# fnzhan/EMLight

Hardware: AMD Instinct MI355X
Metric: training images/sec (regression step: DenseNet-BC fwd + Sinkhorn loss + bwd + Adam) (higher is better)
Workload: dtype f32; 1 GPU; RegressionNetwork train step, BASELINE configs[1]; per_gpu_batch=64, global_batch=64, anchors=128, parallelism=single

## Files before the change

emlight_amd/RegressionNetwork/dense_engine.py:

```python

import os
import weakref

import numpy as np
import torch

from .. import _lib
from .._knobs import knob_int, knob_flag


def _r16(v):
    return (v + 15) // 16 * 16


def _capturing(x):
    return x.is_cuda and torch.cuda.is_current_stream_capturing()


def _row_floats(ctot):
    a = knob_int("EML_ROW_ALIGN", 32, 16, 64)
    if a not in (16, 32, 64):
        raise ValueError("EML_ROW_ALIGN must be 16, 32 or 64")
    return (ctot + a - 1) // a * a


class _Workspace:

    def __init__(self, enc, B, H, W, dev, keep_all):
        f32 = dict(dtype=torch.float32, device=dev)
        self.B, self.H, self.W = B, H, W
        self.blocks = []
        h, w = H, W
        for bi, (c0, nl) in enumerate(zip(enc.block_c0, enc.block_layers)):
            ctot = c0 + nl * enc.growth
            blk = {
                "H": h, "W": w, "P": B * h * w, "C0": c0, "Ctot": ctot, "ld": _row_floats(ctot),
                "X": torch.zeros(B * h * w, _row_floats(ctot), **f32),
                "Z": torch.empty(nl if keep_all else 1, B * h * w, enc.inter, **f32),
                "mean": torch.zeros(_r16(ctot), **f32), "var": torch.ones(_r16(ctot), **f32),
                "istd": torch.ones(_r16(ctot), **f32),
                "layers": [],
            }
            for l in range(nl):
                kp = _r16(c0 + l * enc.growth)
                blk["layers"].append({
                    "Cin": c0 + l * enc.growth, "Kp": kp,
                    "scale1": torch.zeros(kp, **f32), "shift1": torch.zeros(kp, **f32),
                    "scale2": torch.zeros(enc.inter, **f32), "shift2": torch.zeros(enc.inter, **f32),
                    "zmean": torch.zeros(enc.inter, **f32), "zvar": torch.ones(enc.inter, **f32),
                    "zistd": torch.ones(enc.inter, **f32),
                    "W1p": torch.empty(kp * 48, **f32), "W2p": torch.empty(9 * 3 * 4 * 16 * 4, **f32),
                    "W2t": torch.empty(7 * 3 * 64 * 4, **f32),
                    "mask": (torch.empty(((B * h * w + 255) // 256) * 16 * (kp // 16) * 4, dtype=torch.int64, device=dev)
                             if keep_all else None),
                })
            cout = enc.trans_cout[bi]
            kpt = _r16(ctot)
            blk["trans"] = {
                "Cout": cout, "Kp": kpt, "nchunks": (cout + 47) // 48,
                "scale": torch.zeros(kpt, **f32), "shift": torch.zeros(kpt, **f32),
                "Wp": torch.empty(((cout + 47) // 48) * kpt * 48, **f32),
                "Ko": _r16(cout),
                "T": torch.zeros(B * (h // 2) * (w // 2), _r16(cout), **f32),
                "A": torch.empty(B * (h // 2) * (w // 2), kpt, **f32),
                "mask16": (torch.empty(B * (h // 2) * (w // 2) * (kpt // 4), dtype=torch.int16, device=dev)
                           if keep_all else None),
                "one": torch.ones(kpt, **f32), "zero": torch.zeros(kpt, **f32),
                "tmean": torch.zeros(cout, **f32), "tvar": torch.ones(cout, **f32), "tistd": torch.ones(cout, **f32),
                "scaleL": torch.zeros(cout, **f32), "shiftL": torch.zeros(cout, **f32),
            }
            blk["tp"] = enc.tap_packed_plan(B, h, w, dev)
            self.blocks.append(blk)
            h, w = h // 2, w // 2
        self.hf, self.wf = h, w
        cf = enc.trans_cout[-1]
        self.F = torch.zeros(B * h * w, _r16(cf), **f32)
        self.Y0 = torch.empty(B * H * W, enc.c_init, **f32)
        self.mean0 = torch.zeros(enc.c_init, **f32)
        self.var0 = torch.ones(enc.c_init, **f32)
        self.istd0 = torch.ones(enc.c_init, **f32)
        self.scale0 = torch.zeros(enc.c_init, **f32)
        self.shift0 = torch.zeros(enc.c_init, **f32)
        self.partials = torch.zeros(enc.grid_max * max(96 * enc.chunks_max, 2 * enc.kp_max), dtype=torch.float64,
                                    device=dev)
        self.owner, self.done = None, True

    def in_use(self):
        return (not self.done) and self.owner is not None and self.owner() is not None


class _PermuteTable:
    _DT = np.dtype([("src", "<u8"), ("dst", "<u8"), ("kind", "<i4"), ("Cout", "<i4"), ("Cin", "<i4"), ("Kp", "<i4"),
                    ("Ko", "<i4"), ("reserved", "<i4")])

    def __init__(self):
        self.key, self.dev, self.n = None, None, 0

    def launch(self, L, st, items):
        key = tuple((w.data_ptr(), d.data_ptr(), cout, cin) for w, d, _, cout, cin, *_ in items)
        if key != self.key:
            host = np.zeros(len(items), dtype=self._DT)
            for i, (w, d, kind, cout, cin, kp, ko) in enumerate(items):
                host[i] = (w.data_ptr(), d.data_ptr(), kind, cout, cin, kp, ko, 0)
            self.dev = torch.from_numpy(host.view(np.uint8).copy()).to(items[0][1].device)
            self.key, self.n = key, len(items)
        _lib.check(L.eml_dense_permute_batch_f32(_lib.ptr(self.dev), self.n, st), "eml_dense_permute_batch_f32")


class _EncoderFn(torch.autograd.Function):

    @staticmethod
    def forward(ctx, enc, x, *params):
        ctx.enc = enc
        needs_grad = any(ctx.needs_input_grad[1:])
        ws, pooled = enc.run_forward(x, keep_all=needs_grad)
        ctx.ws = ws
        if needs_grad:
            ws.owner, ws.done = weakref.ref(ctx), False
        ctx.save_for_backward(x)
        return pooled

    @staticmethod
    def backward(ctx, gpooled):
        (x,) = ctx.saved_tensors
        ws = ctx.ws
        if ws.owner is None or ws.owner() is not ctx:
            raise RuntimeError("HIP DenseNet: the activations of this forward are gone -- backward() was already run on "
                               "this graph (the workspace is released after the first backward; retain_graph / double "
                               "backward are not supported)")
        need_x, need_params = ctx.needs_input_grad[1], ctx.needs_input_grad[2:]
        dx, grads = ctx.enc.run_backward(ws, x, gpooled.contiguous(), need_x, need_params)
        ws.done, ws.owner = True, None
        ctx.enc.trim_pool(ws)
        return (None, dx) + tuple(g if need else None for g, need in zip(grads, need_params))


class HipDenseEncoder:
    GRID_MAX = 1024

    @staticmethod
    def check_supported(model):
        f = model.features
        if model.bn_size * model.growth_rate != 48 or model.growth_rate != 12:
            raise NotImplementedError("the HIP engine is built for growth_rate=12, bn_size=4 (EMLight's DenseNet)")
        c = f.conv0.out_channels
        if c != 24:
            raise NotImplementedError("the HIP engine is built for num_init_features=24 (got %d)" % c)
        for bi, nl in enumerate(model.block_config):
            ctot = c + nl * model.growth_rate
            if nl < 1 or _r16(ctot) > 384:
                raise NotImplementedError("dense block %d would be %d channels wide; the HIP kernels hold per-channel "
                                          "vectors of at most 384 (EMLight: 216/300/342)" % (bi + 1, ctot))
            c = getattr(f, "transition%d" % (bi + 1)).conv.out_channels
            if _r16(c) == 48:
                raise NotImplementedError("transition %d has %d output channels: widths that pad to 48 collide with the "
                                          "dense layers' bottleneck in the 1x1 launchers (EMLight: 108/150/171)" % (bi + 1, c))
            if c % 2 and bi + 1 < len(model.block_config):
                raise NotImplementedError("transition %d feeds a dense block with an odd channel count (%d)" % (bi + 1, c))

    def __init__(self, model):
        f = model.features
        self.check_supported(model)
        self.model = model
        self.growth = model.growth_rate
        self.inter = model.bn_size * model.growth_rate
        self.c_init = f.conv0.out_channels
        self.block_layers = list(model.block_config)
        self.block_c0, self.trans_cout = [], []
        c = self.c_init
        for bi, nl in enumerate(self.block_layers):
            self.block_c0.append(c)
            c += nl * self.growth
            c = getattr(f, "transition%d" % (bi + 1)).conv.out_channels
            self.trans_cout.append(c)
        self.avgpool = model.avgpool_size
        self.grid_max = self.GRID_MAX
        self.kp_max = max(_r16(c0 + nl * self.growth) for c0, nl in zip(self.block_c0, self.block_layers))
        self.ko_max = max(_r16(c) for c in self.trans_cout)
        self.chunks_max = max((c + 47) // 48 for c in self.trans_cout)
        self._ws = {}
        self._cu = None
        self.last_dropout_key = None

    def param_list(self):
        f = self.model.features
        ps = [f.conv0.weight, f.norm0.weight, f.norm0.bias]
        for bi, nl in enumerate(self.block_layers):
            blk = getattr(f, "denseblock%d" % (bi + 1))
            for l in range(nl):
                L = getattr(blk, "denselayer%d" % (l + 1))
                ps += [L.norm1.weight, L.norm1.bias, L.conv1.weight, L.norm2.weight, L.norm2.bias, L.conv2.weight]
            T = getattr(f, "transition%d" % (bi + 1))
            ps += [T.norm.weight, T.norm.bias, T.conv.weight]
            LN = getattr(f, "last_norm%d" % (bi + 1))
            ps += [LN.weight, LN.bias]
        return ps

    def __call__(self, x):
        x = _lib.require_gpu_tensor(x, "x")
        B, C, H, W = x.shape
        if C != 3:
            raise ValueError("expected (B,3,H,W) input")
        div = 2 ** len(self.block_layers)
        if H % div or W % div or (H // div) < self.avgpool or (W // div) < self.avgpool:
            raise ValueError("crop %dx%d: each of the %d transitions halves the map and the HIP kernels need even maps "
                             "(H, W divisible by %d), then the head pools %dx%d.  Deviation from the reference: its "
                             "AvgPool2d(2) floors odd maps, so e.g. 100x132 trains there; crop to a multiple of %d "
                             "(EMLight's 192x256 and 240x320 are)." % (H, W, len(self.block_layers), div, self.avgpool,
                                                                       self.avgpool, div))
        return _EncoderFn.apply(self, x, *self.param_list())

    def _grid(self, dev):
        if self._cu is None:
            self._cu = torch.cuda.get_device_properties(dev).multi_processor_count
        return self._tuned("EML_GRID", 2 * self._cu)

    def _tuned(self, env, default):
        g = int(os.environ.get(env, 0))
        return min(self.grid_max, g if g > 0 else default)

    def overlap_wgrad(self, dev):
        return torch.device(dev).type == "cuda" and os.environ.get("EML_WGRAD_OVERLAP", "0") == "1"

    def _grid3(self, dev):
        self._grid(dev)
        return self._tuned("EML_GRID3", self._cu)

    def tap_packed_plan(self, B, H, W, dev):
        from .._knobs import knob_choice
        if knob_choice("EML_C3_TP", "auto", ("auto", "off")) == "off":
            return None
        if _lib.lib().eml_dense_conv3x3_fwd_tp_supported(B, H, W) != 4 or H < 8:
            return None
        self._grid(dev)
        bands = max(1, min(H // 4, -(-2 * self._cu // B)))
        band = -(-H // bands)
        return band, min(self.grid_max, B * (-(-H // band)))

    def workspace(self, B, H, W, dev, keep_all):
        key = (B, H, W, dev, keep_all)
        pool = self._ws.get(key)
        if pool is None:
            pool = []
            self._ws = {key: pool}
        for ws in pool:
            if not ws.in_use():
                return ws
        if pool:
            import warnings
            warnings.warn("HIP DenseNet: a %s grad-enabled forward of shape %s is alive before the previous one ran its "
                          "backward: allocating another full activation workspace (GBs at training sizes; idle extras are "
                          "freed after a backward)" % ("second" if len(pool) == 1 else "%d-th" % (len(pool) + 1),
                                                       (B, H, W)), stacklevel=3)
        ws = _Workspace(self, B, H, W, dev, keep_all)
        pool.append(ws)
        return ws

    POOL_KEEP = 2

    def trim_pool(self, ws):
        for key, pool in self._ws.items():
            if ws in pool:
                idle = [w for w in pool if not w.in_use()]
                for extra in idle[self.POOL_KEEP:]:
                    pool.remove(extra)
                return

    def _prepare(self, L, st, partials, G, pstride, n_new, c_new0, count, mean, var, istd, bn, C, Cpad, training,
                 scale, shift):
        p = _lib.ptr
        if bn is None:
            args = (None, None, None, None)
            eps, mom = 1e-5, 0.1
        else:
            args = (p(bn.weight), p(bn.bias), p(bn.running_mean), p(bn.running_var))
            eps, mom = bn.eps, (bn.momentum if bn.momentum is not None else 0.1)
        _lib.check(L.eml_dense_bn_prepare_f32(p(partials), G, pstride, n_new, c_new0, float(count), p(mean), p(var),
                                              p(istd), *args, C, Cpad, eps, mom, int(training), p(scale), p(shift),
                                              st), "eml_dense_bn_prepare_f32")

    def dropout_plan(self, x):
        from .DenseNet import check_drop_rate
        f = self.model.features
        plan, any_drop = [], False
        for bi, nl in enumerate(self.block_layers):
            mod = getattr(f, "denseblock%d" % (bi + 1))
            row = []
            for l in range(nl):
                Lm = getattr(mod, "denselayer%d" % (l + 1))
                q = check_drop_rate(Lm.drop_rate)
                row.append(q if (Lm.training and q > 0) else 0.0)
                any_drop = any_drop or row[-1] > 0
            plan.append(row)
        if not any_drop:
            return None, None
        if _capturing(x):
            raise RuntimeError("HIP DenseNet: drop_rate > 0 while the stream is being captured -- a captured graph would replay "
                               "one fixed dropout mask on every replay; capture with drop_rate = 0 or in eval mode")
        key = self.model.dropout_key
        if key is None:
            lo, hi = torch.randint(0, 2 ** 32, (2,), dtype=torch.int64).tolist()
            key = lo | (hi << 32)
        return key, plan

    def run_forward(self, x, keep_all):
        L, p, st = _lib.lib(), _lib.ptr, _lib.current_stream()
        m = self.model
        f = m.features
        B, _, H, W = x.shape
        dev = x.device
        drop_key, drop_plan = self.dropout_plan(x)
        ws = self.workspace(B, H, W, dev, keep_all)
        ws.drop_key, ws.drop_plan = drop_key, drop_plan
        self.last_dropout_key = drop_key
        G = self._grid(dev)
        G3 = self._grid3(dev)
        Gf = self._tuned("EML_GRID_FWD1", G)
        Gb = min(self.grid_max, 4 * (self._cu or 256))
        training = m.training
        part = ws.partials
        b0 = ws.blocks[0]
        if getattr(ws, "fwd_permutes", None) is None:
            ws.fwd_permutes = _PermuteTable()
        items = []
        for bi, blk in enumerate(ws.blocks):
            mod = getattr(f, "denseblock%d" % (bi + 1))
            for l, lay in enumerate(blk["layers"]):
                Lm = getattr(mod, "denselayer%d" % (l + 1))
                items.append((Lm.conv1.weight, lay["W1p"], 0, 48, lay["Cin"], lay["Kp"], 0))
                if blk["tp"] is None or not training:
                    items.append((Lm.conv2.weight, lay["W2p"], 1, 12, 48, 48, 0))
                else:
                    items.append((Lm.conv2.weight, lay["W2t"], 3, 12, 48, 48, 0))
            T, tr = getattr(f, "transition%d" % (bi + 1)), blk["trans"]
            items.append((T.conv.weight, tr["Wp"], 0, tr["Cout"], blk["Ctot"], tr["Kp"], 0))
        ws.fwd_permutes.launch(L, st, items)
        conv0 = ("eml_dense_conv0_fwd_mfma_f32" if knob_flag("EML_CONV0_MFMA", True) and 3 * B * H * W < 2 ** 31
                 else "eml_dense_conv0_fwd_f32")
        _lib.check(getattr(L, conv0)(p(x), p(f.conv0.weight), p(ws.Y0), self.c_init, B, H, W, self.c_init,
                                     p(part), G, st), conv0)
        self._prepare(L, st, part, G, 2 * self.c_init, self.c_init, 0, b0["P"], ws.mean0, ws.var0, ws.istd0, f.norm0,
                      self.c_init, self.c_init, training, ws.scale0, ws.shift0)
        _lib.check(L.eml_dense_bn_apply_f32(p(ws.Y0), self.c_init, p(b0["X"]), b0["ld"], self.c_init, b0["P"],
                                            p(ws.scale0), p(ws.shift0), 1, p(part), Gb, st), "eml_dense_bn_apply_f32")
        self._prepare(L, st, part, Gb, 2 * self.c_init, self.c_init, 0, b0["P"], b0["mean"], b0["var"], b0["istd"],
                      None, 0, 0, training, None, None)
        nb = len(ws.blocks)
        for bi, blk in enumerate(ws.blocks):
            mod = getattr(f, "denseblock%d" % (bi + 1))
            gl0 = sum(self.block_layers[:bi])
            P, Hb, Wb, ld = blk["P"], blk["H"], blk["W"], blk["ld"]
            pending = False
            Gc = G3
            for l, lay in enumerate(blk["layers"]):
                Lm = getattr(mod, "denselayer%d" % (l + 1))
                cin, kp = lay["Cin"], lay["Kp"]
                z = blk["Z"][l if keep_all else 0]
                self._prepare(L, st, part if pending else None, Gc, 32, 12, cin - 12, P, blk["mean"], blk["var"],
                              blk["istd"], Lm.norm1, cin, kp, training, lay["scale1"], lay["shift1"])
                _lib.check(L.eml_dense_conv1x1_fwd_f32(p(blk["X"]), ld, P, Hb, Wb, 0, kp, p(lay["scale1"]),
                                                       p(lay["shift1"]), p(lay["W1p"]), 48, p(z), 48, p(part), Gf,
                                                       p(lay["mask"]) if (keep_all and training) else None, st),
                           "eml_dense_conv1x1_fwd_f32")
                self._prepare(L, st, part, Gf, 96, 48, 0, P, lay["zmean"], lay["zvar"], lay["zistd"], Lm.norm2, 48, 48,
                              training, lay["scale2"], lay["shift2"])
                q = drop_plan[bi][l] if drop_plan is not None else 0.0
                drop = (drop_key, gl0 + l, q) if q > 0 else ()
                if blk["tp"] is None or not training:
                    Gc = G3
                    fn = "eml_dense_conv3x3_fwd_drop_f32" if drop else "eml_dense_conv3x3_fwd_f32"
                    _lib.check(getattr(L, fn)(p(z), p(lay["scale2"]), p(lay["shift2"]), p(lay["W2p"]), p(blk["X"]), ld, cin,
                                              B, Hb, Wb, p(part), G3, *drop, st), fn)
                else:
                    band, Gc = blk["tp"]
                    fn = "eml_dense_conv3x3_fwd_tp_drop_f32" if drop else "eml_dense_conv3x3_fwd_tp_f32"
                    _lib.check(getattr(L, fn)(p(z), p(lay["scale2"]), p(lay["shift2"]), p(lay["W2t"]), p(blk["X"]), ld, cin,
                                              B, Hb, Wb, band, p(part), Gc, *drop, st), fn)
                pending = True
            tr, T = blk["trans"], getattr(f, "transition%d" % (bi + 1))
            LN = getattr(f, "last_norm%d" % (bi + 1))
            ctot, cout, kpt = blk["Ctot"], tr["Cout"], tr["Kp"]
            self._prepare(L, st, part if pending else None, Gc, 32, 12, ctot - 12, P, blk["mean"], blk["var"],
                          blk["istd"], T.norm, ctot, kpt, training, tr["scale"], tr["shift"])
            Pn = B * (Hb // 2) * (Wb // 2)
            _lib.check(L.eml_dense_pool_act_f32(p(blk["X"]), ld, B, Hb, Wb, kpt, p(tr["scale"]), p(tr["shift"]),
                                                p(tr["A"]), kpt, p(tr["mask16"]) if (keep_all and training) else None,
                                                st), "eml_dense_pool_act_f32")
            _lib.check(L.eml_dense_conv1x1_fwd_f32(p(tr["A"]), kpt, Pn, Hb // 2, Wb // 2, 0, kpt, p(tr["one"]),
                                                   p(tr["zero"]), p(tr["Wp"]), cout, p(tr["T"]), tr["Ko"], p(part), G,
                                                   None, st), "eml_dense_conv1x1_fwd_f32(transition)")
            for ch in range(tr["nchunks"]):
                nv = min(48, cout - 48 * ch)
                last = ch == tr["nchunks"] - 1
                pv = part[ch * G * 96:]
                self._prepare(L, st, pv, G, 96, nv, 48 * ch, Pn, tr["tmean"], tr["tvar"], tr["tistd"],
                              LN if last else None, cout if last else 0, cout if last else 0, training,
                              tr["scaleL"] if last else None, tr["shiftL"] if last else None)
            if bi + 1 < nb:
                nxt = ws.blocks[bi + 1]
                dst, ldd = nxt["X"], nxt["ld"]
            else:
                dst, ldd = ws.F, ws.F.shape[1]
            _lib.check(L.eml_dense_bn_apply_f32(p(tr["T"]), tr["Ko"], p(dst), ldd, cout, Pn, p(tr["scaleL"]),
                                                p(tr["shiftL"]), 0, p(part), Gb, st), "eml_dense_bn_apply_f32")
            if bi + 1 < nb:
                self._prepare(L, st, part, Gb, 2 * cout, cout, 0, Pn, nxt["mean"], nxt["var"], nxt["istd"], None, 0, 0,
                              training, None, None)
        cf = self.trans_cout[-1]
        k = self.avgpool
        pooled = torch.empty(B, cf * (ws.hf // k) * (ws.wf // k), dtype=torch.float32, device=dev)
        _lib.check(L.eml_dense_head_pool_fwd_f32(p(ws.F), ws.F.shape[1], cf, B, ws.hf, ws.wf, k, p(pooled), st),
                   "eml_dense_head_pool_fwd_f32")
        if training:
            bns = [mm for mm in f.modules() if isinstance(mm, torch.nn.BatchNorm2d)]
            torch._foreach_add_([mm.num_batches_tracked for mm in bns], 1)
        return ws, pooled

    def run_backward(self, ws, x, gpooled, need_x=False, need_params=None):
        from .dense_engine_bwd import run_backward
        return run_backward(self, ws, x, gpooled, need_x, need_params)
```

emlight_amd/RegressionNetwork/dense_engine_bwd.py:

```python
import ctypes
import os

import torch

from .. import _lib
from .._knobs import knob_choice, knob_flag


def _r16(v):
    return (v + 15) // 16 * 16


class _BwdBuffers:
    def gf12(self, r):
        if self.GF12[r] is None:
            self.GF12[r] = self._gf12_new()
        return self.GF12[r]

    def __init__(self, enc, ws, dev):
        f32 = dict(dtype=torch.float32, device=dev)
        self.G = [torch.zeros(blk["P"], blk["ld"], **f32) for blk in ws.blocks]
        self.GF = torch.zeros(ws.F.shape[0], ws.F.shape[1], **f32)
        maxP = ws.blocks[0]["P"]
        self.DZ = torch.empty(2, maxP, 48, **f32)
        self.ring = max(1, int(os.environ.get("EML_WGRAD_RING", 4))) if enc.overlap_wgrad(dev) else 1
        self.GF12 = [None] * self.ring
        self._gf12_new = lambda: torch.empty(maxP, 12, **f32)
        self.N12 = torch.empty(maxP, 12, **f32)
        self.TOP = torch.empty(2 * maxP * 12, **f32)
        kp, ko, g = enc.kp_max, max(enc.ko_max, 48), enc.grid_max
        self.Wd = [[torch.empty(lay["Kp"] * 48, **f32) for lay in blk["layers"]] for blk in ws.blocks]
        self.WdT = [torch.empty(blk["trans"]["Kp"] * blk["trans"]["Ko"], **f32) for blk in ws.blocks]
        self.permutes = None
        self.coef = torch.zeros(8, max(kp, ko), **f32)
        self.part2 = torch.zeros(2, g * kp * 2, dtype=torch.float64, device=dev)
        self.partW = torch.empty(g * max(kp * 48, 2 * 27 * 256, 4 * 1024), **f32)
        i32 = dict(dtype=torch.int32, device=dev)
        self.cond = [[torch.zeros(lay["Kp"], **i32) for lay in blk["layers"]] for blk in ws.blocks]
        self.condT = [torch.zeros(blk["trans"]["Kp"], **i32) for blk in ws.blocks]
        self.any_ill = torch.zeros(1, **i32)
        self.dg_grid = 128
        self.dg_scratch = torch.empty(self.dg_grid * kp, dtype=torch.float64, device=dev)
        self.side = None
        if enc.overlap_wgrad(dev):
            self.side = torch.cuda.Stream(device=dev)
            self.partW3 = [torch.empty(g * 2 * 27 * 256, **f32) for _ in range(self.ring)]
            self.ev_ready = [torch.cuda.Event() for _ in range(self.ring)]
            self.ev_done = [None] * self.ring


def run_backward(enc, ws, x, gpooled, need_x=False, need_params=None):
    if getattr(ws, "bwd", None) is None:
        ws.bwd = _BwdBuffers(enc, ws, x.device)
    L, p, st = _lib.lib(), _lib.ptr, _lib.current_stream()
    m = enc.model
    f = m.features
    if not m.training:
        raise NotImplementedError("HIP DenseNet backward is implemented for train-mode BatchNorm "
                                  "(EMLight trains and tests in train mode, train.py:42 / test.py:36-37)")
    dev = x.device
    B, _, H, W = x.shape
    G = enc._grid(dev)
    G3 = enc._grid3(dev)
    G3d = enc._tuned("EML_GRID3_DGRAD", G3)
    Gw = enc._tuned("EML_GRID_WGRAD1", G)
    Gd = enc._tuned("EML_GRID_DGRAD", G)
    Gb = min(enc.grid_max, 4 * enc._cu)
    bw = ws.bwd
    part = ws.partials
    ring = [0]
    if bw.side is not None:
        main = torch.cuda.current_stream(dev)
        st_side = ctypes.c_void_p(bw.side.cuda_stream)
        G3s = enc._tuned("EML_GRID3_SIDE", G3)
        bw.side.wait_stream(main)
    if bw.permutes is None:
        from .dense_engine import _PermuteTable
        bw.permutes = _PermuteTable()
    items = []
    for bi_, blk_ in enumerate(ws.blocks):
        mod_ = getattr(f, "denseblock%d" % (bi_ + 1))
        for l_, lay_ in enumerate(blk_["layers"]):
            items.append((getattr(mod_, "denselayer%d" % (l_ + 1)).conv1.weight, bw.Wd[bi_][l_], 2, 48, lay_["Cin"],
                          lay_["Kp"], 48))
        tr_ = blk_["trans"]
        items.append((getattr(f, "transition%d" % (bi_ + 1)).conv.weight, bw.WdT[bi_], 2, tr_["Cout"], blk_["Ctot"],
                      tr_["Kp"], tr_["Ko"]))
    bw.permutes.launch(L, st, items)
    params = enc.param_list()
    if need_params is None:
        need_params = [True] * len(params)
    from .._dist import grad_slot
    grads = {}
    for q, need in zip(params, need_params):
        slot = grad_slot(q) if need else None
        grads[id(q)] = slot if slot is not None else torch.empty_like(q)
    gr = lambda q: p(grads[id(q)])
    coefs = [tuple(bw.coef[3 * k + i] for i in range(3)) for k in range(2)]
    cA, cB, cC = coefs[0]
    sB, sC = bw.coef[6], bw.coef[7]

    direct = knob_choice("EML_DGAMMA_DIRECT", "always", ("always", "never")) != "never"
    c3_fold = knob_flag("EML_C3_FOLD", True)
    c3_gf = knob_flag("EML_C3_GF", False)
    bw.any_ill.zero_()

    def dgamma_direct(blk, X_ld, Pin, Hin, Win, pool, DY, ld_dy, Zr, ld_z, co, Cout, conv, Cin, scale1, shift1, cond, bn):
        if not direct:
            return
        a, b, c = co if co is not None else (None, None, None)
        _lib.check(L.eml_dense_bn_dgamma_direct_f32(
            p(blk["X"]), X_ld, Pin, Hin, Win, pool, p(DY), ld_dy, p(Zr), ld_z, p(a), p(b), p(c), Cout, p(conv.weight), Cin,
            p(scale1), p(shift1), p(blk["mean"]), p(blk["istd"]), p(cond), p(bw.dg_scratch), gr(bn.weight), bw.dg_grid, st),
            "eml_dense_bn_dgamma_direct_f32")

    def finalize(R, pstride, count, bn, mean, istd, C, Cpad, coef=0, s_acc=None, src=None, c_lo=0, c_hi=None, conv=None,
                 cond=None):
        a, b, c = coefs[coef] if coef is not None else (None, None, None)
        wargs = (p(bn.bias), p(conv.weight), gr(conv.weight), conv.weight.shape[0]) if conv is not None else (None, None, None, 0)
        _lib.check(L.eml_dense_bn_bwd_finalize_f32(
            p(part if src is None else src), R, pstride, float(count), p(bn.weight), p(mean), p(istd), C, Cpad, 1,
            gr(bn.weight), gr(bn.bias), p(a), p(b), p(c),
            p(sB) if s_acc is not None else None, p(sC) if s_acc is not None else None, int(bool(s_acc)),
            c_lo, Cpad if c_hi is None else c_hi, *wargs, p(cond), p(bw.any_ill) if cond is not None else None, st),
            "eml_dense_bn_bwd_finalize_f32")

    def parr(tensors):
        return (ctypes.c_void_p * len(tensors))(*[t.data_ptr() for t in tensors])

    def materialize(Gbuf, blk, c0, n):
        _lib.check(L.eml_dense_grad_materialize_f32(p(Gbuf), blk["ld"], p(blk["X"]), blk["ld"], p(sB), p(sC), c0, n,
                                                    blk["P"], st), "eml_dense_grad_materialize_f32")

    cf, k = enc.trans_cout[-1], enc.avgpool
    ldF = ws.F.shape[1]
    _lib.check(L.eml_dense_head_pool_bwd_f32(p(gpooled), p(ws.F), ldF, cf, B, ws.hf, ws.wf, k, p(bw.GF), ldF, st),
               "eml_dense_head_pool_bwd_f32")
    dY, ld_dy = bw.GF, ldF
    nb = len(ws.blocks)
    for bi in reversed(range(nb)):
        blk, tr = ws.blocks[bi], ws.blocks[bi]["trans"]
        mod = getattr(f, "denseblock%d" % (bi + 1))
        T, LN = getattr(f, "transition%d" % (bi + 1)), getattr(f, "last_norm%d" % (bi + 1))
        P, Hb, Wb, ld, ctot = blk["P"], blk["H"], blk["W"], blk["ld"], blk["Ctot"]
        cout, Ko, kpt = tr["Cout"], tr["Ko"], tr["Kp"]
        Pn = B * (Hb // 2) * (Wb // 2)
        Gbuf = bw.G[bi]
        gl0 = sum(enc.block_layers[:bi])
        top2 = bw.TOP[:2 * P * 12].view(2, P, 12)
        _lib.check(L.eml_dense_bn_bwd_stats_f32(p(dY), ld_dy, p(tr["T"]), Ko, None, 0, 0, cout, Pn, p(tr["tmean"]),
                                                p(tr["tistd"]), p(part), Gb, st), "eml_dense_bn_bwd_stats_f32")
        finalize(Gb, 2 * cout, Pn, LN, tr["tmean"], tr["tistd"], cout, Ko, coef=0)
        _lib.check(L.eml_dense_conv1x1_bwd_weight_f32(
            p(tr["A"]), kpt, Pn, Hb // 2, Wb // 2, 0, kpt, ctot, p(tr["one"]), p(tr["zero"]), p(dY), ld_dy, p(tr["T"]),
            Ko, p(cA), p(cB), p(cC), cout, p(bw.partW), gr(T.conv.weight), G, None, None, 0, None, 0, None, None, st),
            "eml_dense_conv1x1_bwd_weight_f32")
        _lib.check(L.eml_dense_conv1x1_bwd_data_f32(
            p(dY), ld_dy, p(tr["T"]), Ko, p(cA), p(cB), p(cC), Ko, p(bw.WdT[bi]), None, ld, p(tr["scale"]),
            p(tr["shift"]), None, None, Pn, Hb, Wb, 1, kpt, p(Gbuf), ld, 0, p(part), G, p(tr["mask16"]), st),
            "eml_dense_conv1x1_bwd_data_f32")
        finalize(G, 2 * kpt, P, T.norm, blk["mean"], blk["istd"], ctot, kpt, coef=None, s_acc=False, conv=T.conv,
                 cond=bw.condT[bi])
        dgamma_direct(blk, ld, P, Hb, Wb, 1, dY, ld_dy, tr["T"], Ko, coefs[0], cout, T.conv, ctot, tr["scale"], tr["shift"],
                      bw.condT[bi], T.norm)
        def conv2_backward(l, slot, n12=False, narrow_lo=None, top=False):
            lay = blk["layers"][l]
            Lm = getattr(mod, "denselayer%d" % (l + 1))
            cin, kp, z, dz = lay["Cin"], lay["Kp"], blk["Z"][l], bw.DZ[slot]
            gsrc = (p(bw.N12), 12, 0) if n12 else (p(top2[1]), 12, 0) if top else (p(Gbuf), ld, cin)
            r = ring[0] = (ring[0] + 1) % bw.ring
            if bw.side is not None and bw.ev_done[r] is not None:
                main.wait_event(bw.ev_done[r])
            fold = (bw.side is None and c3_fold
                    and L.eml_dense_conv3x3_bwd_fused_supported(gsrc[1], gsrc[2], ld, cin) == 1)
            q = ws.drop_plan[bi][l] if ws.drop_plan is not None else 0.0
            drop = (ws.drop_key, gl0 + l, q) if q > 0 else ()
            if fold:
                fn = "eml_dense_conv3x3_bwd_fused_drop_f32" if drop else "eml_dense_conv3x3_bwd_fused_f32"
                _lib.check(getattr(L, fn)(*gsrc, p(Lm.conv2.weight), p(z), p(lay["zmean"]), p(lay["zistd"]), p(dz), B, Hb, Wb,
                                          p(part), G3d, p(blk["X"]), ld, cin, p(sB), p(sC), p(bw.gf12(r)) if c3_gf else None,
                                          p(lay["scale2"]), p(lay["shift2"]), p(bw.partW), gr(Lm.conv2.weight), *drop, st), fn)
            else:
                fn = "eml_dense_conv3x3_bwd_data_drop_f32" if drop else "eml_dense_conv3x3_bwd_data_f32"
                _lib.check(getattr(L, fn)(*gsrc, p(Lm.conv2.weight), p(z), p(lay["zmean"]), p(lay["zistd"]), p(dz), B, Hb, Wb,
                                          p(part), G3d, p(blk["X"]), ld, cin, p(sB), p(sC), p(bw.gf12(r)), *drop, st), fn)
            if fold:
                pass
            elif bw.side is None:
                _lib.check(L.eml_dense_conv3x3_bwd_weight_f32(p(bw.gf12(r)), 12, 0, p(z), p(lay["scale2"]),
                                                              p(lay["shift2"]), B, Hb, Wb, p(bw.partW),
                                                              gr(Lm.conv2.weight), G3, st),
                           "eml_dense_conv3x3_bwd_weight_f32")
            else:
                bw.ev_ready[r].record(main)
                bw.side.wait_event(bw.ev_ready[r])
                _lib.check(L.eml_dense_conv3x3_bwd_weight_f32(p(bw.gf12(r)), 12, 0, p(z), p(lay["scale2"]),
                                                              p(lay["shift2"]), B, Hb, Wb, p(bw.partW3[r]),
                                                              gr(Lm.conv2.weight), G3s, st_side),
                           "eml_dense_conv3x3_bwd_weight_f32")
                if bw.ev_done[r] is None:
                    bw.ev_done[r] = torch.cuda.Event()
                bw.ev_done[r].record(bw.side)
            finalize(G3d, 96, P, Lm.norm2, lay["zmean"], lay["zistd"], 48, 48, coef=slot)
            a, b, c = coefs[slot]
            _lib.check(L.eml_dense_conv1x1_bwd_weight_f32(
                p(blk["X"]), ld, P, Hb, Wb, 0, kp, cin, p(lay["scale1"]), p(lay["shift1"]), p(dz), 48, p(z), 48,
                p(a), p(b), p(c), 48, p(bw.partW), gr(Lm.conv1.weight), Gw, p(dz),
                *((p(Lm.conv1.weight), narrow_lo, *((p(top2[0]), 12) if top else (p(Gbuf), ld)), p(bw.N12),
                   p(bw.part2[slot])) if narrow_lo is not None
                  else (None, 0, None, 0, None, None)), st), "eml_dense_conv1x1_bwd_weight_f32")
            return Lm

        def dgrad(layers, slots, k_lo, k_hi, top=False):
            lays = [blk["layers"][l] for l in layers]
            if top:
                _lib.check(L.eml_dense_conv1x1_bwd_data_multi_top_f32(
                    parr([bw.DZ[s_] for s_ in slots]), parr([bw.Wd[bi][l_] for l_ in layers]),
                    parr([y["scale1"] for y in lays]), parr([y["shift1"] for y in lays]),
                    parr([bw.part2[s_] for s_ in slots]), (ctypes.c_int * len(layers))(*[y["Kp"] for y in lays]),
                    P, k_hi, p(Gbuf), ld, Gd, parr([y["mask"] for y in lays]), p(top2), st),
                    "eml_dense_conv1x1_bwd_data_multi_top_f32")
                return
            _lib.check(L.eml_dense_conv1x1_bwd_data_multi_f32(
                len(layers), parr([bw.DZ[s_] for s_ in slots]), None, None, None, None,
                parr([bw.Wd[bi][l_] for l_ in layers]),
                parr([y["scale1"] for y in lays]), parr([y["shift1"] for y in lays]),
                parr([bw.part2[s_] for s_ in slots]), (ctypes.c_int * len(layers))(*[y["Kp"] for y in lays]),
                None, ld, None, None, P, k_lo, k_hi, p(Gbuf), ld, Gd,
                parr([y["mask"] for y in lays]), st),
                "eml_dense_conv1x1_bwd_data_multi_f32")

        def bn1_finalize(l, Lm, slot, c_lo, c_hi, rows=None):
            lay = blk["layers"][l]
            finalize(Gd if rows is None else rows, 2 * lay["Kp"], P, Lm.norm1, blk["mean"], blk["istd"], lay["Cin"], lay["Kp"], coef=None,
                     s_acc=True, src=bw.part2[slot], c_lo=c_lo, c_hi=c_hi, conv=Lm.conv1, cond=bw.cond[bi][l])

        def bn1_direct(l, Lm, slot):
            lay = blk["layers"][l]
            dgamma_direct(blk, ld, P, Hb, Wb, 0, bw.DZ[slot], 48, None, 0, None, 48, Lm.conv1, lay["Cin"], lay["scale1"],
                          lay["shift1"], bw.cond[bi][l], Lm.norm1)

        l = len(blk["layers"]) - 1
        have_top = False
        while l >= 0:
            if l >= 1:
                la, lb = l, l - 1
                cin_a, cin_b = blk["layers"][la]["Cin"], blk["layers"][lb]["Cin"]
                Lma = conv2_backward(la, 0, narrow_lo=cin_b, top=have_top)
                bn1_finalize(la, Lma, 0, cin_b, cin_a, rows=Gw)
                Lmb = conv2_backward(lb, 1, n12=True)
                to_top = (lb >= 2 and blk["layers"][la]["mask"] is not None and bw.side is None
                          and cin_b >= 24 and cin_b % 4 == 0)
                dgrad([la, lb], [0, 1], 0, cin_b, top=to_top)
                have_top = to_top
                bn1_finalize(la, Lma, 0, 0, cin_b)
                bn1_finalize(lb, Lmb, 1, 0, blk["layers"][lb]["Kp"])
                bn1_direct(la, Lma, 0)
                bn1_direct(lb, Lmb, 1)
                l -= 2
            else:
                Lm0 = conv2_backward(l, 0)
                dgrad([l], [0], 0, blk["layers"][l]["Cin"])
                bn1_finalize(l, Lm0, 0, 0, blk["layers"][l]["Kp"])
                bn1_direct(l, Lm0, 0)
                l -= 1
        c0b = blk["C0"]
        norm0_fused = bi == 0 and knob_flag("EML_NORM0_FUSED", True) and c0b % 4 == 0 and c0b <= 32
        if not norm0_fused:
            materialize(Gbuf, blk, 0, c0b)
        dY, ld_dy = Gbuf, ld
    b0 = ws.blocks[0]
    c0 = enc.c_init
    if norm0_fused:
        _lib.check(L.eml_dense_norm0_bwd_stats_f32(p(dY), ld_dy, p(ws.Y0), c0, p(ws.scale0), p(ws.shift0), p(sB), p(sC), c0,
                                                   b0["P"], p(ws.mean0), p(ws.istd0), p(part), Gb, st),
                   "eml_dense_norm0_bwd_stats_f32")
    else:
        _lib.check(L.eml_dense_bn_bwd_stats_f32(p(dY), ld_dy, p(ws.Y0), c0, p(b0["X"]), b0["ld"], 1, c0, b0["P"],
                                                p(ws.mean0), p(ws.istd0), p(part), Gb, st), "eml_dense_bn_bwd_stats_f32")
    finalize(Gb, 2 * c0, b0["P"], f.norm0, ws.mean0, ws.istd0, c0, _r16(c0), coef=0)
    if norm0_fused:
        _lib.check(L.eml_dense_conv0_bwd_weight_fused_f32(p(x), p(dY), ld_dy, p(ws.Y0), c0, p(ws.scale0), p(ws.shift0), p(sB),
                                                          p(sC), p(cA), p(cB), p(cC), B, H, W, p(bw.partW),
                                                          gr(f.conv0.weight), G, st), "eml_dense_conv0_bwd_weight_fused_f32")
    else:
        _lib.check(L.eml_dense_conv0_bwd_weight_f32(p(x), p(dY), ld_dy, p(b0["X"]), b0["ld"], p(ws.Y0), c0, p(cA), p(cB),
                                                    p(cC), B, H, W, p(bw.partW), gr(f.conv0.weight), G, st),
                   "eml_dense_conv0_bwd_weight_f32")
    dx = None
    if need_x:
        dx = torch.empty(B, 3, H, W, dtype=torch.float32, device=dev)
        X1 = (None, 0) if norm0_fused else (p(b0["X"]), b0["ld"])
        _lib.check(L.eml_dense_conv0_bwd_data_f32(p(dY), ld_dy, *X1, p(ws.Y0), c0, p(ws.scale0), p(ws.shift0), p(sB), p(sC),
                                                  p(cA), p(cB), p(cC), p(f.conv0.weight), B, H, W, p(dx), st),
                   "eml_dense_conv0_bwd_data_f32")
    if bw.side is not None:
        main.wait_stream(bw.side)
    return dx, [grads[id(q)] for q in params]
```

emlight_amd/_lib.py:

```python
import ctypes
import os
import threading

_HERE = os.path.dirname(os.path.abspath(__file__))
LIB_PATH = os.environ.get("EML_LIB_PATH") or os.path.join(_HERE, "libemlight_hip.so")

_f32p = ctypes.c_void_p
_i32p = ctypes.c_void_p
_f64p = ctypes.c_void_p
_stream = ctypes.c_void_p
_int = ctypes.c_int
_u64 = ctypes.c_ulonglong

ABI_VERSION = 31

SIGNATURES = {
    "eml_abi_version": (_int, []),
    "eml_last_error": (ctypes.c_char_p, []),
    "eml_sg_rasterise_f32": (_int, [_f32p, _f32p, _f32p, _f32p, _int, _int, _int, _int, _stream]),
    "eml_sg_rasterise_ex_f32": (_int, [_f32p, _f32p, _f32p, _f32p, _int, _int, _int, _int, _int, ctypes.c_void_p, _stream]),
    "eml_sg_rasterise_bwd_colors_f32": (_int, [_f32p, _f32p, _f32p, _f32p, _int, _int, _int, _int, _stream]),
    "eml_emd_anchor_cost_f32": (_int, [_f32p, _f32p, _int, _stream]),
    "eml_sinkhorn_schedule_f32": (_int, [_f32p, _f32p, ctypes.c_long, ctypes.c_double, ctypes.c_double, _int,
                                         ctypes.c_double, _f32p, _f32p, _i32p, _f32p, _stream]),
    "eml_sinkhorn_work_floats": (ctypes.c_size_t, [_int, _int]),
    "eml_sinkhorn_fwd_f32": (_int, [_f32p, _f32p, _f32p, _f32p, _f32p, _f32p, ctypes.c_double, ctypes.c_double, _int,
                                    ctypes.c_double, _f32p, _f32p, _i32p, _f32p, _f32p, _f32p, _f32p, _f32p, _int, _int,
                                    _stream]),
    "eml_sinkhorn_fwd_ex_f32": (_int, [_f32p, _f32p, _f32p, _f32p, _f32p, _f32p, ctypes.c_double, ctypes.c_double, _int,
                                       ctypes.c_double, _f32p, _f32p, _i32p, _f32p, _f32p, _f32p, _f32p, _f32p, _int, _int,
                                       _int, _stream]),
    "eml_sinkhorn_fwd_rho_f32": (_int, [_f32p, _f32p, _f32p, _f32p, _f32p, _f32p, ctypes.c_double, ctypes.c_double, _int,
                                        ctypes.c_double, _f32p, _f32p, _i32p, _f32p, _f32p, _f32p, _f32p, _f32p, _int, _int,
                                        _int, ctypes.c_double, _f32p, _stream]),
    "eml_sinkhorn_bwd_f32": (_int, [_f32p, _f32p, _f32p, _int, _int, _stream]),
    "eml_sinkhorn_dim_work_floats": (ctypes.c_size_t, [_int, _int, _int]),
    "eml_sinkhorn_fwd_dim_f32": (_int, [_f32p, _f32p, _f32p, _f32p, _f32p, _f32p, ctypes.c_double, ctypes.c_double, _int,
                                        ctypes.c_double, _f32p, _f32p, _i32p, _f32p, _f32p, _f32p, _f32p, _f32p, _int, _int,
                                        _int, _int, ctypes.c_double, _f32p, _stream]),
    "eml_sinkhorn_schedule_dim_f32": (_int, [_f32p, _f32p, ctypes.c_long, _int, ctypes.c_double, ctypes.c_double, _int,
                                             ctypes.c_double, _f32p, _f32p, _i32p, _f32p, _stream]),
    "eml_sinkhorn_bwd_weights_f32": (_int, [_f32p, _f32p, _f32p, _f32p, _int, _int, _stream]),
    "eml_l1_pairs_partial_doubles": (ctypes.c_size_t, [_int]),
    "eml_l1_pairs_fwd_f32": (_int, [_int, ctypes.c_void_p, ctypes.c_void_p, ctypes.c_void_p, ctypes.c_void_p, ctypes.c_void_p,
                                    ctypes.c_void_p, _f64p, _f32p, _stream]),
    "eml_l1_pairs_bwd_f32": (_int, [_int, ctypes.c_void_p, ctypes.c_void_p, ctypes.c_void_p, ctypes.c_void_p, ctypes.c_void_p,
                                    ctypes.c_void_p, _f32p, ctypes.c_void_p, ctypes.c_void_p, ctypes.c_void_p, _stream]),
    "eml_colsum_partial_doubles": (ctypes.c_size_t, [_int]),
    "eml_colsum_f32": (_int, [_f32p, ctypes.c_long, _int, _f64p, _f32p, _stream]),
    "eml_gt_anchor_index_i32": (_int, [_f32p, _int, _int, _int, _i32p, _stream]),
    "eml_gt_parametrise_f64": (_int, [_f32p, _i32p, _i32p, _int, _int, _int, _int, _f32p, _f32p, _f32p, _stream]),
    "eml_pano_crop_f32": (_int, [ctypes.c_void_p, _int, _int, _int, _int, _int, _int, ctypes.c_double, ctypes.c_double, _f64p,
                                 ctypes.c_double, _f64p, _f32p, _stream]),
    "eml_pano_resize_area_f32": (_int, [_f32p, _int, _int, _int, _int, _int, ctypes.c_double, _f64p, _f32p, _stream]),
    "eml_tonemap_work_floats": (ctypes.c_size_t, [_int]),
    "eml_tonemap_f32": (_int, [_f32p, _int, ctypes.c_long, _int, ctypes.c_double, ctypes.c_double, ctypes.c_double, _f32p,
                               _int, _f32p, _f32p, _i32p, _f32p, ctypes.c_void_p, _stream]),
    "eml_projector_targets_work_floats": (ctypes.c_size_t, [_int, _int, _int]),
    "eml_projector_targets_f32": (_int, [_f32p, _f32p, _int, _int, _int, _f32p, _f32p, _f32p, _stream]),
    "eml_resize_bilinear_f32": (_int, [_f32p, _f32p, _int, _int, _int, _int, _int, _int, _int, _f32p, _stream]),
    "eml_sphere_render_work_floats": (ctypes.c_size_t, [_int, _int, _int, _int]),
    "eml_sphere_render_f32": (_int, [_f32p, _int, _int, _int, _int, ctypes.c_double, _int, ctypes.c_double, _f32p, _f32p,
                                     _stream]),
    "eml_sphere_render_metrics_f64": (_int, [_f32p, _f32p, _int, _int, _int, _f64p, _stream]),
    "eml_needlet_basis_f32": (_int, [_f32p, _int, _f32p, _f32p, _int, _f32p, _stream]),
    "eml_needlet_work_floats": (ctypes.c_size_t, [_int, _int, _int]),
    "eml_needlet_analysis_f32": (_int, [_f32p, _f32p, _f32p, _int, _int, _f32p, _f32p, _int, _f32p, _f32p, _stream]),
    "eml_needlet_synthesis_f32": (_int, [_f32p, _f32p, _f32p, _int, _int, _f32p, _f32p, _int, _f32p, _stream]),
    "eml_needlet_sparsify_f32": (_int, [_f32p, _int, _int, _int, ctypes.c_double, _f32p, _i32p, _stream]),
    "eml_sh_basis_f32": (_int, [_f32p, _int, _f32p, _int, _f32p, _stream]),
    "eml_sh_work_floats": (ctypes.c_size_t, [_int, _int, _int, _int]),
    "eml_sh_analysis_f32": (_int, [_f32p, _f32p, _f32p, _f32p, _f32p, _int, _int, _int, _int, _f32p, _f32p, _stream]),
    "eml_sh_synthesis_f32": (_int, [_f32p, _f32p, _f32p, _f32p, _f32p, _int, _int, _int, _int, _f32p, _stream]),
    "eml_sphere_tap_table_f32": (_int, [_f32p, _int, _int, _int, _int, _i32p, _f32p, _stream]),
    "eml_sphere_im2col_f32": (_int, [_f32p, _i32p, _f32p, _f32p, _int, _int, _int, _int, _stream]),
    "eml_sphere_col2im_f32": (_int, [_f32p, _i32p, _i32p, _f32p, _f32p, _int, _int, _int, _int, _stream]),
    "eml_sphere_conv_fwd_fused_f32": (_int, [_f32p, _i32p, _f32p, _f32p, _f32p, _f32p, _int, _int, _int, _int, _int, _int,
                                             _stream]),
    "eml_sphere_conv_fwd_fused_ex_f32": (_int, [_f32p, _i32p, _f32p, _f32p, _f32p, _f32p, _int, _int, _int, _int, _int, _int,
                                                _f32p, ctypes.c_float, _int, _stream]),
    "eml_sphere_conv_small_supported": (_int, [_int, _int]),
    "eml_sphere_conv_small_fwd_f32": (_int, [_f32p, _i32p, _f32p, _f32p, _f32p, _f32p, _int, _int, _int, _int, _int,
                                             ctypes.c_float, _stream]),
    "eml_sphere_conv_small_wgrad_partial_floats": (ctypes.c_size_t, [_int, _int, _int, _int]),
    "eml_sphere_conv_small_wgrad_f32": (_int, [_f32p, _i32p, _f32p, _f32p, _f32p, ctypes.c_float, _f32p, _f32p, _f32p, _int,
                                               _int, _int, _int, _int, _stream]),
    "eml_sphere_conv_small_da9_f32": (_int, [_f32p, _f32p, ctypes.c_float, _f32p, _f32p, ctypes.c_long, _int, _int, _stream]),
    "eml_spade_norm_modulate_up2_fwd_f32": (_int, [_f32p, _f32p, _f32p, _int, _int, _int, _int, ctypes.c_float, _f32p, _f32p,
                                                   _stream]),
    "eml_spade_norm_modulate_bwd_cols_f32": (_int, [_f32p, _f32p, _f32p, _f32p, _f32p, _int, _int, _int, _int, _int,
                                                    ctypes.c_float, _f32p, _f32p, _f32p, _int, _stream]),
    "eml_sg_rasterise_bwd_work_floats": (ctypes.c_size_t, [_int, _int, _int, _int]),
    "eml_sg_rasterise_bwd_colors_ex_f32": (_int, [_f32p, _f32p, _f32p, _f32p, _f32p, _int, _int, _int, _int, _int, _stream]),
    "eml_sg_rasterise_bwd_full_work_floats": (ctypes.c_size_t, [_int, _int, _int, _int]),
    "eml_sg_rasterise_bwd_f32": (_int, [_f32p, _f32p, _f32p, _f32p, _f32p, _f32p, _f32p, _f32p, _int, _int, _int, _int, _int,
                                        _stream]),
    "eml_sphere_conv_narrow_supported": (_int, [_int, _int]),
    "eml_sphere_conv_narrow_fwd_f32": (_int, [_f32p, _i32p, _f32p, _f32p, _f32p, _f32p, _int, _int, _int, _int, _int, _stream]),
    "eml_sphere_conv_narrow_dgrad_f32": (_int, [_f32p, _i32p, _f32p, _int, _f32p, _f32p, _int, _int, _int, _int, _int, _stream]),
    "eml_sphere_conv_narrow_wgrad_partial_floats": (ctypes.c_size_t, [_int, _int, _int, _int]),
    "eml_sphere_conv_narrow_wgrad_f32": (_int, [_f32p, _i32p, _f32p, _f32p, _f32p, _f32p, _int, _int, _int, _int, _int, _stream]),
    "eml_sphere_conv_narrow_scratch_floats": (ctypes.c_size_t, [_int, _int]),
    "eml_sphere_conv_narrow_fwd2_f32": (_int, [_f32p, _i32p, _f32p, _f32p, _f32p, _f32p, _f32p, _int, _int, _int, _int, _int, _stream]),
    "eml_sphere_conv_narrow_wgrad2_partial_floats": (ctypes.c_size_t, [_int, _int, _int]),
    "eml_sphere_conv_narrow_dgrad2_f32": (_int, [_f32p, _i32p, _f32p, _int, ctypes.c_void_p, _f32p, _f32p, _f32p, _int, _int, _int,
                                                 _int, _int, _int, _stream]),
    "eml_sphere_conv_narrow_wgrad2_f32": (_int, [_f32p, _i32p, _f32p, _int, ctypes.c_void_p, _f32p, _f32p, _f32p, _f32p, _int, _int,
                                                 _int, _int, _int, _stream]),
    "eml_sphere_conv_spade_supported": (_int, [_int, _int, ctypes.c_long]),
    "eml_sphere_conv_spade_fwd_f32": (_int, [_f32p, _i32p, _f32p, _f32p, _f32p, _f32p, _f32p, _f32p, _f32p, _f32p, _int, _int,
                                             _int, _int, _int, _int, ctypes.c_float, _int, _stream]),
    "eml_spade_norm_modulate_bwd_y_f32": (_int, [_f32p, _f32p, _f32p, _f32p, _f32p, _f32p, _int, _int, _int, _int, _int,
                                                 ctypes.c_float, _f32p, _f32p, _f32p, _int, _stream]),
    "eml_bn_bwd_apply_up2_f32": (_int, [_f32p, _f32p, _int, _int, _int, _int, _f32p, _f32p, _f32p, _f32p, _stream]),
    "eml_spectral_norm_scratch_floats": (ctypes.c_size_t, [_int, _int]),
    "eml_spectral_norm_w2_f32": (_int, [_f32p, _f32p, _f32p, _int, ctypes.c_float, _f32p, _f32p, _f32p, _f32p, _int, _int,
                                        _stream]),
    "eml_spectral_norm_w2_bwd_f32": (_int, [_f32p, _f32p, _f32p, _f32p, _f32p, _f32p, _f32p, _int, _int, _stream]),
    "eml_spectral_norm_w2_batch_f32": (_int, [_int, ctypes.c_void_p, ctypes.c_void_p, ctypes.c_void_p, _int, ctypes.c_float,
                                              ctypes.c_void_p, ctypes.c_void_p, ctypes.c_void_p, ctypes.c_void_p, ctypes.c_void_p,
                                              ctypes.c_void_p, _stream]),
    "eml_spade_heads_w2_f32": (_int, [_f32p, _f32p, _f32p, _f32p, _f32p, _f32p, _int, _int, _int, _stream]),
    "eml_instance_norm_act_fwd_f32": (_int, [_f32p, _f32p, _f32p, _int, _int, _int, _int, ctypes.c_float, ctypes.c_float,
                                             _stream]),
    "eml_instance_norm_act_bwd_f32": (_int, [_f32p, _f32p, _f32p, _f32p, _int, _int, _int, _int, ctypes.c_float, _stream]),
    "eml_sphere_conv_dgrad_fused_f32": (_int, [_f32p, _i32p, _f32p, _i32p, _int, _f32p, _f32p, _int, _int, _int, _int, _int,
                                               _int, _stream]),
    "eml_sphere_conv_lowres_variant": (_int, [_int, _int, _int, _int]),
    "eml_sphere_conv_lowres_table_i32": (_int, [_i32p, _i32p, _i32p, _int, _int, _stream]),
    "eml_sphere_conv_lowres_partial_floats": (ctypes.c_size_t, [ctypes.c_long, _int, _int]),
    "eml_sphere_conv_lowres_f32": (_int, [_f32p, _i32p, _f32p, _i32p, _int, _i32p, _int, _f32p, _f32p, _f32p, _f32p, _int, _int,
                                          _int, _int, _int, _int, _f32p, ctypes.c_float, _stream]),
    "eml_sphere_conv_wgrad_partial_floats": (ctypes.c_size_t, [_int, _int, _int]),
    "eml_sphere_conv_wgrad_fused_f32": (_int, [_f32p, _i32p, _f32p, _f32p, _f32p, _f32p, _int, _int, _int, _int, _int, _int,
                                               _stream]),
    "eml_spade_modulate_fwd_f32": (_int, [_f32p, _int, _f32p, _int, _f32p, _int, ctypes.c_long, _int, ctypes.c_float,
                                          _stream]),
    "eml_spade_modulate_bwd_f32": (_int, [_f32p, _int, _f32p, _int, _f32p, _int, _f32p, _int, _f32p, _int, ctypes.c_long,
                                          _int, ctypes.c_float, _stream]),
    "eml_bn_stats_f32": (_int, [_f32p, _int, ctypes.c_long, _int, _f32p, _int, _stream]),
    "eml_bn_fold_f64": (_int, [_f32p, _int, _int, _f32p, _stream]),
    "eml_bn_finalize_f32": (_int, [_f32p, _int, ctypes.c_float, ctypes.c_float, _f32p, _f32p, _f32p, _f32p, _stream]),
    "eml_spade_norm_modulate_fwd_f32": (_int, [_f32p, _int, _f32p, _int, _f32p, _int, ctypes.c_long, _int, ctypes.c_float,
                                               _f32p, _f32p, _stream]),
    "eml_bn_bwd_apply_f32": (_int, [_f32p, _int, _f32p, _int, ctypes.c_long, _int, _f32p, _f32p, _f32p, _f32p, _int,
                                    _stream]),
    "eml_dense_conv0_fwd_f32": (_int, [_f32p, _f32p, _f32p, _int, _int, _int, _int, _int, _f32p, _int, _stream]),
    "eml_dense_conv0_fwd_mfma_f32": (_int, [_f32p, _f32p, _f32p, _int, _int, _int, _int, _int, _f32p, _int, _stream]),
    "eml_dense_bn_apply_f32": (_int, [_f32p, _int, _f32p, _int, _int, ctypes.c_long, _f32p, _f32p, _int, _f32p,
                                      _int, _stream]),
    "eml_dense_bn_prepare_f32": (_int, [_f32p, _int, _int, _int, _int, ctypes.c_double, _f32p, _f32p, _f32p, _f32p,
                                        _f32p, _f32p, _f32p, _int, _int, ctypes.c_float, ctypes.c_float, _int,
                                        _f32p, _f32p, _stream]),
    "eml_dense_permute_w1_f32": (_int, [_f32p, _int, _int, _int, _f32p, _stream]),
    "eml_dense_permute_w2_f32": (_int, [_f32p, _int, _f32p, _stream]),
    "eml_dense_permute_batch_f32": (_int, [ctypes.c_void_p, _int, _stream]),
    "eml_dense_conv1x1_fwd_f32": (_int, [_f32p, _int, ctypes.c_long, _int, _int, _int, _int, _f32p, _f32p, _f32p,
                                         _int, _f32p, _int, _f32p, _int, ctypes.c_void_p, _stream]),
    "eml_dense_conv3x3_fwd_f32": (_int, [_f32p, _f32p, _f32p, _f32p, _f32p, _int, _int, _int, _int, _int, _f32p,
                                         _int, _stream]),
    "eml_dense_permute_w2_tp_f32": (_int, [_f32p, _f32p, _stream]),
    "eml_dense_conv3x3_fwd_tp_supported": (_int, [_int, _int, _int]),
    "eml_dense_conv3x3_fwd_tp_f32": (_int, [_f32p, _f32p, _f32p, _f32p, _f32p, _int, _int, _int, _int, _int, _int, _f32p,
                                            _int, _stream]),
    "eml_dense_conv3x3_fwd_drop_f32": (_int, [_f32p, _f32p, _f32p, _f32p, _f32p, _int, _int, _int, _int, _int, _f32p,
                                              _int, _u64, _int, ctypes.c_double, _stream]),
    "eml_dense_conv3x3_fwd_tp_drop_f32": (_int, [_f32p, _f32p, _f32p, _f32p, _f32p, _int, _int, _int, _int, _int, _int, _f32p,
                                                 _int, _u64, _int, ctypes.c_double, _stream]),
    "eml_dense_dropout_mask_u16": (_int, [_u64, _int, ctypes.c_double, ctypes.c_long, ctypes.c_void_p, _stream]),
    "eml_dense_pool_act_f32": (_int, [_f32p, _int, _int, _int, _int, _int, _f32p, _f32p, _f32p, _int, ctypes.c_void_p,
                                      _stream]),
    "eml_dense_head_pool_fwd_f32": (_int, [_f32p, _int, _int, _int, _int, _int, _int, _f32p, _stream]),
    "eml_dense_conv3x3_bwd_data_f32": (_int, [_f32p, _int, _int, _f32p, _f32p, _f32p, _f32p, _f32p, _int, _int, _int,
                                              _f32p, _int, _f32p, _int, _int, _f32p, _f32p, _f32p, _stream]),
    "eml_dense_conv3x3_bwd_fused_supported": (_int, [_int, _int, _int, _int]),
    "eml_dense_conv3x3_bwd_fused_f32": (_int, [_f32p, _int, _int, _f32p, _f32p, _f32p, _f32p, _f32p, _int, _int, _int, _f64p, _int,
                                               _f32p, _int, _int, _f32p, _f32p, _f32p, _f32p, _f32p, _f32p, _f32p, _stream]),
    "eml_dense_conv3x3_bwd_data_drop_f32": (_int, [_f32p, _int, _int, _f32p, _f32p, _f32p, _f32p, _f32p, _int, _int, _int,
                                                   _f32p, _int, _f32p, _int, _int, _f32p, _f32p, _f32p, _u64, _int,
                                                   ctypes.c_double, _stream]),
    "eml_dense_conv3x3_bwd_fused_drop_f32": (_int, [_f32p, _int, _int, _f32p, _f32p, _f32p, _f32p, _f32p, _int, _int, _int,
                                                    _f64p, _int, _f32p, _int, _int, _f32p, _f32p, _f32p, _f32p, _f32p, _f32p,
                                                    _f32p, _u64, _int, ctypes.c_double, _stream]),
    "eml_dense_conv3x3_bwd_weight_f32": (_int, [_f32p, _int, _int, _f32p, _f32p, _f32p, _int, _int, _int, _f32p,
                                                _f32p, _int, _stream]),
    "eml_dense_bn_bwd_finalize_f32": (_int, [_f32p, _int, _int, ctypes.c_double, _f32p, _f32p, _f32p, _int, _int,
                                             _int, _f32p, _f32p, _f32p, _f32p, _f32p, _f32p, _f32p, _int, _int, _int,
                                             _f32p, _f32p, _f32p, _int, _i32p, _i32p, _stream]),
    "eml_dense_bn_dgamma_direct_f32": (_int, [_f32p, _int, ctypes.c_long, _int, _int, _int, _f32p, _int, _f32p, _int,
                                              _f32p, _f32p, _f32p, _int, _f32p, _int, _f32p, _f32p, _f32p, _f32p, _i32p,
                                              _f32p, _f32p, _int, _stream]),
    "eml_dense_conv1x1_bwd_weight_f32": (_int, [_f32p, _int, ctypes.c_long, _int, _int, _int, _int, _int, _f32p,
                                                _f32p, _f32p, _int, _f32p, _int, _f32p, _f32p, _f32p, _int, _f32p,
                                                _f32p, _int, _f32p, _f32p, _int, _f32p, _int, _f32p, _f32p, _stream]),
    "eml_dense_conv1x1_bwd_narrow_f32": (_int, [_f32p, _f32p, _int, _int, _f32p, _int, _f32p, _f32p, _f32p, _f32p,
                                                ctypes.c_long, _f32p, _int, _f32p, _f32p, _int, _int, _stream]),
    "eml_dense_permute_w1_bwd_f32": (_int, [_f32p, _int, _int, _int, _int, _f32p, _stream]),
    "eml_dense_conv1x1_bwd_data_f32": (_int, [_f32p, _int, _f32p, _int, _f32p, _f32p, _f32p, _int, _f32p, _f32p,
                                              _int, _f32p, _f32p, _f32p, _f32p, ctypes.c_long, _int, _int, _int,
                                              _int, _f32p, _int, _int, _f32p, _int, ctypes.c_void_p, _stream]),
    "eml_dense_conv1x1_bwd_data_multi_f32": (_int, [_int] + [ctypes.c_void_p] * 10 + [_f32p, _int, _f32p, _f32p,
                                                    ctypes.c_long, _int, _int, _f32p, _int, _int, ctypes.c_void_p,
                                                    _stream]),
    "eml_dense_conv1x1_bwd_data_multi_top_f32": (_int, [ctypes.c_void_p] * 6 + [ctypes.c_long, _int, _f32p, _int, _int,
                                                        ctypes.c_void_p, _f32p, _stream]),
    "eml_dense_grad_materialize_f32": (_int, [_f32p, _int, _f32p, _int, _f32p, _f32p, _int, _int, ctypes.c_long,
                                              _stream]),
    "eml_dense_bn_bwd_stats_f32": (_int, [_f32p, _int, _f32p, _int, _f32p, _int, _int, _int, ctypes.c_long, _f32p,
                                          _f32p, _f32p, _int, _stream]),
    "eml_dense_norm0_bwd_stats_f32": (_int, [_f32p, _int, _f32p, _int, _f32p, _f32p, _f32p, _f32p, _int, ctypes.c_long, _f32p, _f32p,
                                             ctypes.c_void_p, _int, _stream]),
    "eml_dense_conv0_bwd_weight_fused_f32": (_int, [_f32p, _f32p, _int, _f32p, _int, _f32p, _f32p, _f32p, _f32p, _f32p, _f32p, _f32p,
                                                    _int, _int, _int, _f32p, _f32p, _int, _stream]),
    "eml_dense_conv0_bwd_weight_f32": (_int, [_f32p, _f32p, _int, _f32p, _int, _f32p, _int, _f32p, _f32p, _f32p,
                                              _int, _int, _int, _f32p, _f32p, _int, _stream]),
    "eml_dense_conv0_bwd_data_f32": (_int, [_f32p, _int, _f32p, _int, _f32p, _int, _f32p, _f32p, _f32p, _f32p, _f32p, _f32p,
                                            _f32p, _f32p, _int, _int, _int, _f32p, _stream]),
    "eml_dense_head_pool_bwd_f32": (_int, [_f32p, _f32p, _int, _int, _int, _int, _int, _int, _f32p, _int, _stream]),
}

EXT_SIGNATURES = {
    "eml_pano_warp_f32": (_int, [_f32p, _int, _int, _int, _int, _int, ctypes.c_double, ctypes.c_double, ctypes.c_double, _f64p,
                                 _f32p, _f64p, _stream]),
    "eml_pano_warp_bwd_work_floats": (ctypes.c_size_t, [_int, _int, _int, _int, _int, _int, _int]),
    "eml_pano_warp_bwd_f32": (_int, [_f32p, _f32p, _int, _int, _int, _int, _int, ctypes.c_double, ctypes.c_double,
                                     ctypes.c_double, _f64p, _f32p, _f64p, _f32p, _stream]),
    "eml_sphere_render_bwd_work_floats": (ctypes.c_size_t, [_int, _int, _int, _int]),
    "eml_sphere_render_bwd_f32": (_int, [_f32p, _int, _int, _int, _int, ctypes.c_double, _int, ctypes.c_double, _i32p, _i32p,
                                         _f32p, _f32p, _f32p, _stream]),
    "eml_sphere_mirror_taps_f32": (_int, [_int, _int, _int, ctypes.c_double, _i32p, _f32p, _stream]),
    "eml_gm_anchor_cost_f32": (_int, [ctypes.c_void_p, _int, _int, _int, _f32p, _f32p, _stream]),
    "eml_sinkhorn_fwd_cost_f32": (_int, [_f32p, _f32p, _f32p, _f32p, _f32p, _f32p, ctypes.c_double, ctypes.c_double, _int,
                                         ctypes.c_double, _f32p, _f32p, _i32p, _f32p, _f32p, _f32p, _f32p, _f32p, _int, _int,
                                         _int, _int, ctypes.c_double, _f32p, ctypes.c_long, _stream]),
    "eml_sphere_max_pool_fwd_f32": (_int, [_f32p, _i32p, _f32p, _f32p, ctypes.c_void_p, _int, _int, _int, _int, _stream]),
    "eml_sphere_max_pool_bwd_f32": (_int, [_f32p, ctypes.c_void_p, _i32p, _i32p, _f32p, _f32p, _int, _int, _int, _int, _stream]),
    "eml_sphere_conv_small_dbias_f32": (_int, [_f32p, _f32p, ctypes.c_float, _f32p, _f32p, _int, _int, _int, _int, _stream]),
    "eml_env_prefilter_work_floats": (ctypes.c_size_t, [_int, _int, _int, _int, _int]),
    "eml_env_prefilter_f32": (_int, [_f32p, _int, _int, _int, _int, _int, ctypes.c_void_p, _f32p, _f32p, _stream]),
    "eml_gbuffer_shade_f32": (_int, [_f32p, _int, _f32p, _int, ctypes.c_long, _f32p, _int, ctypes.c_long, _f32p, _f32p, _f32p,
                                     _f32p, _f32p, _int, _int, _int, ctypes.c_double, ctypes.c_double, _f32p, _f32p, _f32p,
                                     ctypes.c_double, _f32p, _stream]),
    "eml_env_prefilter_bwd_work_floats": (ctypes.c_size_t, [_int, _int, _int, _int, _int]),
    "eml_env_prefilter_bwd_f32": (_int, [_f32p, _int, _int, _int, _int, _int, ctypes.c_void_p, _f32p, _f32p, _stream]),
    "eml_gbuffer_shade_bwd_work_floats": (ctypes.c_size_t, [_int, _int, _int, _int, _int, _int, _int, _int, _int]),
    "eml_gbuffer_shade_bwd_f32": (_int, [_f32p, _f32p, _int, _f32p, _int, ctypes.c_long, _f32p, _int, ctypes.c_long, _f32p,
                                         _f32p, _f32p, _f32p, _f32p, _int, _int, _int, ctypes.c_double, ctypes.c_double,
                                         _f32p, _f32p, ctypes.c_double, _f32p, _f32p, _f32p, _f32p, _f32p, _f32p, _f32p,
                                         _f32p, _stream]),
    "eml_pano_warp_depth_work_floats": (ctypes.c_size_t, [_int, _int, _int]),
    "eml_pano_warp_depth_f32": (_int, [_f32p, _f32p, _int, _int, _int, _int, _int, ctypes.c_double, ctypes.c_double,
                                       ctypes.c_double, _f64p, _int, _int, _f32p, _f32p, _f64p, _f32p, _stream]),
    "eml_gt_anchor_depth_f64": (_int, [_f32p, _i32p, _i32p, _int, _int, _int, _int, _f64p, _stream]),
    "eml_ground_shadow_work_floats": (ctypes.c_size_t, [_int, _int, _int, _int, _int]),
    "eml_ground_shadow_f32": (_int, [_f32p, _int, _int, _int, _f32p, _int, _f32p, _int, _int, _int, ctypes.c_double,
                                     ctypes.c_double, _f32p, _f32p, _f32p, _f32p, _stream]),
}

_lock = threading.Lock()
_lib = None


class EmlightHipError(RuntimeError):
    pass


def lib():
    global _lib
    if _lib is not None:
        return _lib
    with _lock:
        if _lib is not None:
            return _lib
        if not os.path.exists(LIB_PATH):
            raise EmlightHipError(
                "libemlight_hip.so not found at %s -- build it with "
                "`python -c 'import __graft_entry__ as g; g.build()'` or `make -C emlight_amd/csrc`. "
                "There is no CPU fallback." % LIB_PATH)
        handle = ctypes.CDLL(LIB_PATH)
        for name, (res, args) in list(SIGNATURES.items()) + list(EXT_SIGNATURES.items()):
            try:
                fn = getattr(handle, name)
            except AttributeError as e:
                raise EmlightHipError("libemlight_hip.so lacks symbol %s" % name) from e
            fn.restype, fn.argtypes = res, args
        got = handle.eml_abi_version()
        if got != ABI_VERSION:
            raise EmlightHipError("libemlight_hip.so has ABI version %d, this binding expects %d -- rebuild it "
                                  "(make -C emlight_amd/csrc)" % (got, ABI_VERSION))
        _lib = handle
    from . import _gemm_selection
    _gemm_selection.ensure_if_requested()
    return _lib


_DEBUG_SYNC = bool(os.environ.get("EML_DEBUG_SYNC"))


def check(rc, what):
    if rc != 0:
        msg = lib().eml_last_error()
        raise EmlightHipError("%s failed (rc=%d): %s" % (what, rc, msg.decode() if msg else "?"))
    if _DEBUG_SYNC:
        import sys
        import torch
        sys.stderr.write("[eml] %s ... " % what)
        sys.stderr.flush()
        torch.cuda.synchronize()
        sys.stderr.write("ok\n")


def ptr(t):
    if t is None:
        return None
    return ctypes.c_void_p(t.data_ptr())


def current_stream():
    import torch
    return ctypes.c_void_p(torch.cuda.current_stream().cuda_stream)


def require_gpu_tensor(t, name, dtype=None):
    import torch
    if not isinstance(t, torch.Tensor) or not t.is_cuda:
        raise EmlightHipError("%s must be a tensor on the MI355X (got %s); there is no CPU path"
                              % (name, getattr(t, "device", type(t))))
    if t.dtype != (dtype or torch.float32):
        raise EmlightHipError("%s must be %s (got %s)" % (name, dtype or torch.float32, t.dtype))
    return t.contiguous()
```

emlight_amd/csrc/dense_bwd.hip:

```cpp
#include "eml_common.h"
#include "eml_dropout.h"

#include <cstdint>
#include <cstdlib>
#include <type_traits>

namespace {

using eml::f32x4;
using eml::f4c;
using eml::mfma16;
using eml::shfl_xor_d;

constexpr int kTH = 8, kTW = 32, kHH = kTH + 2, kHW = kTW + 2;

constexpr int kPSG = 14;
constexpr int kBD = 512;
constexpr int kGRows = 2;
constexpr int kGPass = kHH / kGRows;

template <bool FUSE, bool WIDE, bool DROP = false>
__global__ __launch_bounds__(kBD, 2) void conv3x3_bwd_data_kernel(
    const float* __restrict__ G, int ldg, int c0, const float* __restrict__ W2, const float* __restrict__ Z,
    const float* __restrict__ zmean, const float* __restrict__ zistd, float* __restrict__ DZ, int B, int H, int W,
// ... 444 lines not shown

  for (int e = tid; e < 27 * 3 * 64; e += 512) {
    const int l = e & 63, g3 = e >> 6, n = g3 % 3, ts = g3 / 3, s3 = ts % 3, tap = ts / 3;
    w_l[e] = W2[((size_t)(4 * s3 + (l >> 4)) * 48 + 16 * n + (l & 15)) * 9 + tap];
  }
  if (tid < 24) coef_l[tid] = tid < 12 ? sB[cx + tid] : sC[cx + tid - 12];

  const int role = __builtin_amdgcn_readfirstlane(wave >> 2), pairj = wave & 3;
  f32x4 accw[4][3];
  int goff[4];
#pragma unroll
  for (int i = 0; i < 4; ++i) {
#pragma unroll
    for (int n = 0; n < 3; ++n) accw[i][n] = f32x4{0.f, 0.f, 0.f, 0.f};
    const int t = min(3 * role + i, 6);
    const int row = min(16 * t + r, 107), tap = row / 12, o = row - 12 * tap;
    goff[i] = (-(tap / 3 - 1) * kHW - (tap % 3 - 1)) * kPSG + o;
  }
  float scb[3], shb[3];
#pragma unroll
  for (int n = 0; n < 3; ++n) {
    scb[n] = scale2[16 * n + r];
    shb[n] = shift2[16 * n + r];
  }
  const int tx_n = (W + kTW - 1) / kTW, ty_n = (H + kTH - 1) / kTH;
  const int ntiles = B * ty_n * tx_n;
  for (int e = tid; e < 8 * 48 * 2; e += 512) red[e] = 0.0;

  constexpr int kWideItems = kHH * kHW * 3;
  int w_hy[2], w_hx[2], w_q[2], w_pix[2];
  bool w_ok[2], w_own[2];
#pragma unroll
  for (int it = 0; it < 2; ++it) {
    const int t = min(tid + 512 * it, kWideItems - 1), hp = t / 3;
    w_q[it] = t - 3 * hp;
    w_hy[it] = hp / kHW;
    w_hx[it] = hp - w_hy[it] * kHW;
  }
  f32x4 gt4[2], xt4[2];
  constexpr int kZI = kTH * kTW * 12 / 512;
  int z_pq[kZI];
#pragma unroll
  for (int it = 0; it < kZI; ++it) {
    const int t = tid + 512 * it;
    z_pq[it] = ((t / 12) << 4) | (t % 12);
  }
  auto stage_begin = [&](int tile) {
    const int b = tile / (ty_n * tx_n), rem = tile - b * (ty_n * tx_n);
    const int ty = rem / tx_n, tx = rem - ty * tx_n;
#pragma unroll
    for (int it = 0; it < 2; ++it) {
      const int gy = ty * kTH - 1 + w_hy[it], gx = tx * kTW - 1 + w_hx[it];
      w_ok[it] = gy >= 0 && gy < H && gx >= 0 && gx < W;
      w_pix[it] = (b * H + min(max(gy, 0), H - 1)) * W + min(max(gx, 0), W - 1);
      if constexpr (STORE_GF) w_own[it] = w_ok[it] && w_hy[it] >= 1 && w_hy[it] <= kTH && w_hx[it] >= 1 && w_hx[it] <= kTW;
    }
  };
  auto g_load = [&](int it) {
    const float* gp = G + (size_t)w_pix[it] * ldg + c0 + 4 * w_q[it];
    const float* xp = Xb + (size_t)w_pix[it] * ldx + cx + 4 * w_q[it];
    if constexpr (A16) {
      asm volatile("global_load_dwordx4 %0, %1, off" : "=&v"(gt4[it]) : "v"(gp) : "memory");
      asm volatile("global_load_dwordx4 %0, %1, off" : "=&v"(xt4[it]) : "v"(xp) : "memory");
    } else {
      const float2 g0 = *reinterpret_cast<const float2*>(gp), g1 = *reinterpret_cast<const float2*>(gp + 2);
      const float2 x0 = *reinterpret_cast<const float2*>(xp), x1 = *reinterpret_cast<const float2*>(xp + 2);
      gt4[it] = f32x4{g0.x, g0.y, g1.x, g1.y};
      xt4[it] = f32x4{x0.x, x0.y, x1.x, x1.y};
    }
  };
  auto g_wait = [&]() {
    if constexpr (A16)
      asm volatile("s_waitcnt vmcnt(0)" : "+v"(gt4[0]), "+v"(xt4[0]), "+v"(gt4[1]), "+v"(xt4[1]) :: "memory");
  };
  auto g_commit = [&](int it, float* dst) {
    const float4 fb4 = *reinterpret_cast<const float4*>(coef_l + 4 * w_q[it]);
    const float4 fc4 = *reinterpret_cast<const float4*>(coef_l + 12 + 4 * w_q[it]);
    float4 v;
    v.x = fmaf(fb4.x, xt4[it][0], gt4[it][0]) + fc4.x;
    v.y = fmaf(fb4.y, xt4[it][1], gt4[it][1]) + fc4.y;
    v.z = fmaf(fb4.z, xt4[it][2], gt4[it][2]) + fc4.z;
    v.w = fmaf(fb4.w, xt4[it][3], gt4[it][3]) + fc4.w;
    if constexpr (DROP) v = eml::drop4(dk, (unsigned)w_pix[it], (unsigned)w_q[it], v);
    if (!w_ok[it]) v = make_float4(0.f, 0.f, 0.f, 0.f);
    float* d = dst + (w_hy[it] * kHW + w_hx[it]) * kPSG + 4 * w_q[it];
    *reinterpret_cast<float2*>(d) = make_float2(v.x, v.y);
    *reinterpret_cast<float2*>(d + 2) = make_float2(v.z, v.w);
    if constexpr (STORE_GF) gt4[it] = f32x4{v.x, v.y, v.z, v.w};
  };
  auto g_store = [&](int it) {
    if constexpr (!STORE_GF) return;
    if (w_own[it]) *reinterpret_cast<float4*>(GF + ((unsigned)w_pix[it] * 12u + 4u * (unsigned)w_q[it])) = make_float4(gt4[it][0], gt4[it][1], gt4[it][2], gt4[it][3]);
  };
  auto z_dma = [&](int it, int b, int y0, int x0, int buf) {
    const int pix = z_pq[it] >> 4, q = z_pq[it] & 15;
    const int gy = min(y0 + (pix >> 5), H - 1), gx = min(x0 + (pix & 31), W - 1);
    const float* src = Z + ((size_t)(b * H + gy) * W + gx) * 48 + 4 * q;
    unsigned keep;
    const unsigned dst = __builtin_amdgcn_readfirstlane(
        (unsigned)(size_t)(const __attribute__((address_space(3))) char*)(z_l + buf * (kTH * kTW * kZS) + 4 * (64 * wave + 512 * it)));
    asm volatile("s_mov_b32 %0, m0\n\ts_mov_b32 m0, %2\n\ts_nop 0\n\tglobal_load_lds_dwordx4 %1, off\n\ts_mov_b32 m0, %0"
                 : "=&s"(keep) : "v"(src), "s"(dst) : "memory");
  };

  int tile = blockIdx.x, cur = 0;
  __syncthreads();
  if (tile < ntiles) {
    stage_begin(tile);
    g_load(0);
    g_load(1);
    {
      const int b = tile / (ty_n * tx_n), rem = tile - b * (ty_n * tx_n);
#pragma unroll
      for (int it = 0; it < kZI; ++it) z_dma(it, b, (rem / tx_n) * kTH, (rem % tx_n) * kTW, 0);
    }
    g_wait();
    g_commit(0, g_l);
    g_commit(1, g_l);
    g_store(0);
    g_store(1);
  }
  __syncthreads();
#ifdef EML_STAMPS
  unsigned long long st_acc[5] = {0, 0, 0, 0, 0}, st_last = __builtin_readcyclecounter();
#endif
  for (; tile < ntiles; tile += gridDim.x) {
    const int nxt = tile + gridDim.x;
    const float* gc = g_l + cur * kGT;
    float* gn = g_l + (cur ^ 1) * kGT;
    const int b = tile / (ty_n * tx_n), rem = tile - b * (ty_n * tx_n);
    const int ty = rem / tx_n, tx = rem - ty * tx_n;
    const int gy = ty * kTH + wave;
    size_t prow[2];
    bool pv[2];
#pragma unroll
    for (int m = 0; m < 2; ++m) {
      const int gx = tx * kTW + 16 * m + r;
      pv[m] = gy < H && gx < W;
      prow[m] = ((size_t)(b * H + min(gy, H - 1)) * W + min(gx, W - 1)) * 48;
    }
    stage_begin(nxt < ntiles ? nxt : tile);
    f32x4 acc[2][3];
#pragma unroll
    for (int m = 0; m < 2; ++m)
#pragma unroll
      for (int n = 0; n < 3; ++n) acc[m][n] = f32x4{0.f, 0.f, 0.f, 0.f};
    float aq[2][2], wq[2][3];
#pragma unroll
    for (int n = 0; n < 3; ++n) wq[0][n] = w_l[n * 64 + lane];
#pragma unroll
    for (int m = 0; m < 2; ++m) aq[0][m] = gc[((wave + 2) * kHW + 16 * m + r + 2) * kPSG + kk];
#pragma unroll
    for (int tap = 0; tap < 9; ++tap) {
#pragma unroll
      for (int s3 = 0; s3 < 3; ++s3) {
        const int gi = tap * 3 + s3;
        if (gi < 2) {
          g_load(gi);
          asm volatile("" ::: "memory");
          __builtin_amdgcn_sched_barrier(0);
        }
        if (gi + 1 < 27) {
          const int tn = (gi + 1) / 3, sn = (gi + 1) - 3 * tn, dyn = tn / 3, dxn = tn - 3 * dyn;
#pragma unroll
          for (int n = 0; n < 3; ++n) wq[(gi + 1) & 1][n] = w_l[((gi + 1) * 3 + n) * 64 + lane];
#pragma unroll
          for (int m = 0; m < 2; ++m)
            aq[(gi + 1) & 1][m] = gc[((wave + 2 - dyn) * kHW + 16 * m + r + 2 - dxn) * kPSG + 4 * sn + kk];
        }
        __builtin_amdgcn_sched_barrier(0);
#pragma unroll
        for (int m = 0; m < 2; ++m)
#pragma unroll
          for (int n = 0; n < 3; ++n) acc[m][n] = mfma16(wq[gi & 1][n], aq[gi & 1][m], acc[m][n]);
        if (gi >= 25) {
          __builtin_amdgcn_sched_barrier(0);
          if (gi == 25) g_wait();
          g_commit(gi - 25, gn);
        }
      }
    }
    g_store(0);
    g_store(1);
    EML_C3_STAMP(0);
    asm volatile("s_waitcnt vmcnt(0)" ::: "memory");
    eml::lds_barrier();
    EML_C3_STAMP(1);
    const float* ga = gc + ((2 * pairj + 1) * kHW + kk + 1) * kPSG;
    const float* zc = z_l + cur * (kTH * kTW * kZS);
    const float* zb = zc + (kTW * 2 * pairj + kk) * kZS + r;
    const int xl0 = ty * kTH + 2 * pairj < H ? W - tx * kTW - kk : 0, xl1 = ty * kTH + 2 * pairj + 1 < H ? W - tx * kTW - kk : 0;
    auto phase_b = [&](auto nt_tag) {
      constexpr int NT = decltype(nt_tag)::value;
      float av[2][NT], bz[2][3];
#pragma unroll
      for (int i = 0; i < NT; ++i) av[0][i] = ga[goff[i]];
#pragma unroll
      for (int n = 0; n < 3; ++n) bz[0][n] = zb[16 * n];
#pragma unroll
      for (int ks = 0; ks < 16; ++ks) {
        if (ks + 1 < 16) {
          const int k1 = ks + 1, go = ((k1 >> 3) * kHW + 4 * (k1 & 7)) * kPSG, zo = ((k1 >> 3) * kTW + 4 * (k1 & 7)) * kZS;
#pragma unroll
          for (int i = 0; i < NT; ++i) av[k1 & 1][i] = ga[go + goff[i]];
#pragma unroll
          for (int n = 0; n < 3; ++n) bz[k1 & 1][n] = zb[zo + 16 * n];
        }
        __builtin_amdgcn_sched_barrier(0);
        if (ks == 1) {
          const int t2 = nxt < ntiles ? nxt : tile;
          const int b2 = t2 / (ty_n * tx_n), rem2 = t2 - b2 * (ty_n * tx_n);
#pragma unroll
          for (int it = 0; it < kZI; ++it) z_dma(it, b2, (rem2 / tx_n) * kTH, (rem2 % tx_n) * kTW, cur ^ 1);
          __builtin_amdgcn_sched_barrier(0);
        }
        const bool pin = 4 * (ks & 7) < (ks < 8 ? xl0 : xl1);
        float bv[3];
#pragma unroll
        for (int n = 0; n < 3; ++n) bv[n] = pin ? fmaf(bz[ks & 1][n], scb[n], shb[n]) : 0.f;
#pragma unroll
        for (int i = 0; i < NT; ++i) {
          const float a = (i < 3 || r < 12) ? av[ks & 1][i] : 0.f;
#pragma unroll
          for (int n = 0; n < 3; ++n) accw[i][n] = mfma16(a, bv[n], accw[i][n]);
        }
        if (ks == 2 || ks == 4 || ks == 6) {
          const int n = (ks - 2) >> 1;
          float l1[4] = {0.f, 0.f, 0.f, 0.f}, l2[4] = {0.f, 0.f, 0.f, 0.f};
#pragma unroll
          for (int m = 0; m < 2; ++m) {
            const float4 z = *reinterpret_cast<const float4*>(zc + (kTW * wave + 16 * m + r) * kZS + 16 * n + 4 * kk);
#pragma unroll
            for (int g = 0; g < 4; ++g) {
              const float v = pv[m] ? acc[m][n][g] : 0.f;
              l1[g] += v;
              l2[g] = fmaf(v, f4c(z, g), l2[g]);
            }
          }
#pragma unroll
          for (int g = 0; g < 4; ++g) {
            const float t1 = eml::row16_sum(l1[g]), t2 = eml::row16_sum(l2[g]);
            if (r == 0) {
              double* d = red + (wave * 48 + 16 * n + 4 * kk + g) * 2;
              d[0] += (double)t1;
              d[1] += (double)t2;
            }
          }
        } else if (ks >= 8 && ks < 14) {
          const int si = ks - 8, m = si / 3, n = si - 3 * m;
          if (pv[m])
            *reinterpret_cast<float4*>(DZ + prow[m] + 16 * n + 4 * kk) =
                make_float4(acc[m][n][0], acc[m][n][1], acc[m][n][2], acc[m][n][3]);
        }
        __builtin_amdgcn_sched_barrier(0);
      }
    };
    if (role == 0) phase_b(std::integral_constant<int, 3>{});
    else phase_b(std::integral_constant<int, 4>{});
    EML_C3_STAMP(2);
    eml::lds_barrier();
    EML_C3_STAMP(3);
#ifdef EML_STAMPS
    st_acc[4] += 1;
#endif
    cur ^= 1;
  }
#ifdef EML_STAMPS
  if (tid == 0)
    for (int i = 0; i < 5; ++i) atomicAdd(&eml_c3_stamps[i], st_acc[i]);
#endif
  asm volatile("s_waitcnt vmcnt(0)" ::: "memory");
  __syncthreads();
  float* wsum = smem;
  for (int w8 = 0; w8 < 8; ++w8) {
    if (wave == w8) {
#pragma unroll
      for (int i = 0; i < 4; ++i)
        if (i < 3 + role) {
#pragma unroll
          for (int n = 0; n < 3; ++n)
#pragma unroll
            for (int g = 0; g < 4; ++g) {
              float* q = wsum + ((((3 * role + i) * 3 + n) * 16 + 4 * kk + g) * 16 + r);
              *q = ((w8 & 3) == 0 ? 0.f : *q) + accw[i][n][g];
            }
        }
    }
    __syncthreads();
  }
  for (int e = tid; e < 21 * 256; e += 512) partialW[(size_t)blockIdx.x * (21 * 256) + e] = wsum[e];
  if (tid < 48) {
    double t1 = 0.0, t2 = 0.0;
#pragma unroll
    for (int w8 = 0; w8 < 8; ++w8) {
      t1 += red[(w8 * 48 + tid) * 2 + 0];
      t2 += red[(w8 * 48 + tid) * 2 + 1];
    }
    partials[(size_t)blockIdx.x * 96 + 2 * tid + 0] = t1;
    partials[(size_t)blockIdx.x * 96 + 2 * tid + 1] = (double)zistd[tid] * (t2 - (double)zmean[tid] * t1);
  }
}


__global__ __launch_bounds__(256) void bn_bwd_finalize_kernel(
    const double* __restrict__ partials, int R, int pstride, double count, const float* __restrict__ gamma,
    const float* __restrict__ mean, const float* __restrict__ istd, int C, int Cpad, int training,
    float* __restrict__ dgamma, float* __restrict__ dbeta, float* __restrict__ cA, float* __restrict__ cB,
    float* __restrict__ cC, float* __restrict__ sB, float* __restrict__ sC, int s_accumulate, int c_lo, int c_hi,
    const float* __restrict__ beta, const float* __restrict__ Wc, const float* __restrict__ dWc, int w_rows,
    int* __restrict__ cond , int* __restrict__ any_cond ) {
  const int lane = threadIdx.x & 63, wave = threadIdx.x >> 6;
  const int c = c_lo + blockIdx.x * 4 + wave;
  if (c >= Cpad || c >= c_hi) return;
  float a = 0.f, b = 0.f, d = 0.f;
  if (c < C) {
    double S1 = 0.0, S2 = 0.0;
    for (int g = lane; g < R; g += 64) {
      S1 += partials[(size_t)g * pstride + 2 * c];
      S2 += partials[(size_t)g * pstride + 2 * c + 1];
    }
    double Q = 0.0;
    if (Wc)
      for (int o = lane; o < w_rows; o += 64) Q += (double)Wc[(size_t)o * C + c] * (double)dWc[(size_t)o * C + c];
#pragma unroll
    for (int o = 32; o > 0; o >>= 1) {
      S1 += __shfl_xor(S1, o, 64);
      S2 += __shfl_xor(S2, o, 64);
      Q += __shfl_xor(Q, o, 64);
    }
    if (Wc) {
      const double ga0 = gamma[c], bs = (double)beta[c] * S1, num = Q - bs;
      S2 = fabs(ga0) >= 1e-12 ? num / ga0 : 0.0;
      if (cond && lane == 0) {
        const int ill = fabs(ga0) < 1e-3 * fabs((double)beta[c]) || ga0 == 0.0;
        cond[c] = ill;
        if (ill && any_cond) *any_cond = 1;
      }
    }
    if (lane == 0) {
      dgamma[c] = (float)S2;
      dbeta[c] = (float)S1;
    }
    const double ga = gamma[c], is = istd[c], mu = mean[c];
    a = (float)(ga * is);
    if (training) {
      b = (float)(-ga * is * is * S2 / count);
      d = (float)(-ga * is * S1 / count + ga * is * is * S2 / count * mu);
    }
  }
  if (lane != 0) return;
  if (cA) {
    cA[c] = a;
    cB[c] = b;
    cC[c] = d;
  }
  if (sB) {
    sB[c] = (s_accumulate ? sB[c] : 0.f) + b;
    sC[c] = (s_accumulate ? sC[c] : 0.f) + d;
  }
}

__global__ __launch_bounds__(256) void reduce_rows_kernel(const float* __restrict__ partial, int R, size_t row_stride,
                                                          int mode, int dim0, int dim1, int n0,
                                                          float* __restrict__ out) {
  __shared__ double red[4][64];
  const int tid = threadIdx.x, e = blockIdx.x * 64 + (tid & 63), slice = tid >> 6;
  size_t src = 0, dst = 0;
  bool valid = false;
  if (mode == 0) {
    const int k = e / 48, o = e - 48 * k;
    valid = k < dim0 && o < dim1;
    src = (size_t)e;
    dst = (size_t)(n0 + o) * dim0 + k;
  } else if (mode == 1) {
    const int o = e & 15, ci = (e >> 4) & 15, pair = e >> 8, tap = pair / 3, mc = pair - 3 * tap;
    valid = pair < 27 && o < 12;
    src = (size_t)e;
    dst = (size_t)(o * 48 + 16 * mc + ci) * 9 + tap;
  } else if (mode == 3) {
    const int j = e & 15, i = (e >> 4) & 15, tn = e >> 8, t = tn / 3, n = tn - 3 * t, row = 16 * t + i;
    valid = tn < 21 && row < 108;
    src = (size_t)e;
    dst = (size_t)((row % 12) * 48 + 16 * n + j) * 9 + row / 12;
  } else {
    const int t = e >> 5, o = e & 31;
    valid = t < 27 && o < dim1;
    src = (size_t)e;
    dst = (size_t)o * 27 + t;
  }
  double s = 0.0;
  if (valid) {
#pragma unroll 8
    for (int r = slice; r < R; r += 4) s += (double)partial[(size_t)r * row_stride + src];
  }
  red[slice][tid & 63] = s;
  __syncthreads();
  if (slice == 0 && valid) out[dst] = (float)((red[0][tid] + red[1][tid]) + (red[2][tid] + red[3][tid]));
}

struct NarrowArgs {
  const float* W1;
  const float* G;
  float* N12;
  double* partials;
  int Cin, k_lo, ldg;
};
template <bool POOL, bool NARROW = false>
__global__ __launch_bounds__(256, NARROW ? 2 : 1) void conv1x1_bwd_weight_kernel(
    const float* __restrict__ X, int ldx, int P, int Hin, int Win, int Kp, const float* __restrict__ scale1,
    const float* __restrict__ shift1, const float* __restrict__ DY, int ld_dy, const float* __restrict__ Zr,
    int ld_z, const float* __restrict__ cA, const float* __restrict__ cB, const float* __restrict__ cC, int n_valid,
    int n_load ,
    float* __restrict__ partial ,
    float* __restrict__ dz_out ,
    NarrowArgs na) {
  __shared__ __attribute__((aligned(16))) float dz_l[2][64 * 48];
  const int tid = threadIdx.x, lane = tid & 63, wave = tid >> 6;
  const int r = lane & 15, kk = lane >> 4;
  constexpr int GW = 32;
  constexpr int MAXG = 3;
  const int ngroups = (Kp + GW - 1) / GW;
  float nsk[4] = {0.f, 0.f, 0.f, 0.f}, ntk[4] = {0.f, 0.f, 0.f, 0.f};
  double ns1[4] = {0.0, 0.0, 0.0, 0.0};
  const int kq = min(kk, 2);
  if constexpr (NARROW) {
#pragma unroll
    for (int g = 0; g < 4; ++g) {
      nsk[g] = kk < 3 ? scale1[na.k_lo + 4 * kq + g] : 0.f;
      ntk[g] = kk < 3 ? shift1[na.k_lo + 4 * kq + g] : 0.f;
    }
  }

  float sv[MAXG][2], tv[MAXG][2];
  int coff[MAXG];
  bool gv[MAXG];
#pragma unroll
  for (int i = 0; i < MAXG; ++i) {
    const int cg = wave + 4 * i;
    const int ch = GW * cg + 2 * r;
    gv[i] = cg < ngroups && ch < Kp;
    coff[i] = gv[i] ? ch : 0;
#pragma unroll
    for (int t = 0; t < 2; ++t) {
      sv[i][t] = gv[i] ? scale1[ch + t] : 0.f;
      tv[i][t] = gv[i] ? shift1[ch + t] : 0.f;
    }
  }
  const int spix = tid >> 2, sq = tid & 3;
  __shared__ __attribute__((aligned(16))) float co_l[3 * 48];
  __shared__ float wn_l[NARROW ? 12 * 64 : 1];
  float4 sa_r[NARROW ? 1 : 3], sb_r[NARROW ? 1 : 3], sc_r[NARROW ? 1 : 3];
  if constexpr (NARROW) {
    if (tid < 48) {
      const bool v = tid < n_valid;
      co_l[tid] = v ? cA[tid] : 0.f;
      co_l[48 + tid] = v ? cB[tid] : 0.f;
      co_l[96 + tid] = v ? cC[tid] : 0.f;
    }
  } else {
#pragma unroll
    for (int j = 0; j < 3; ++j) {
      const int col = 4 * (sq + 4 * j);
      float a[4], b[4], c[4];
#pragma unroll
      for (int e = 0; e < 4; ++e) {
        const bool v = col + e < n_valid;
        a[e] = v ? cA[col + e] : 0.f;
        b[e] = v ? cB[col + e] : 0.f;
        c[e] = v ? cC[col + e] : 0.f;
      }
      sa_r[j] = make_float4(a[0], a[1], a[2], a[3]);
      sb_r[j] = make_float4(b[0], b[1], b[2], b[3]);
      sc_r[j] = make_float4(c[0], c[1], c[2], c[3]);
    }
  }
  if constexpr (NARROW) {
    for (int e = tid; e < 12 * 64; e += 256) {
      const int st = e >> 6, l = e & 63, rr = l & 15, k4 = l >> 4;
      wn_l[e] = rr < 12 ? na.W1[(size_t)(4 * st + k4) * na.Cin + na.k_lo + rr] : 0.f;
    }
  }
  __syncthreads();
  f32x4 acc[MAXG][2][3];
#pragma unroll
  for (int i = 0; i < MAXG; ++i)
#pragma unroll
    for (int t = 0; t < 2; ++t)
#pragma unroll
      for (int n = 0; n < 3; ++n) acc[i][t][n] = f32x4{0.f, 0.f, 0.f, 0.f};

  const int Wo = Win >> 1, Ho = Hin >> 1;
  const int nchunks = (P + 63) >> 6;
  const int ngw = (ngroups > wave) ? (ngroups - wave + 3) >> 2 : 0;

  float4 rdy[3], rzr[3];
  bool rpv = false;
  int rp = 0;
  auto stage_load = [&](int chunk) {
    const int p = chunk * 64 + spix;
    rpv = chunk < nchunks && p < P;
    const size_t pc = rpv ? p : 0;
    rp = (int)pc;
#pragma unroll
    for (int j = 0; j < 3; ++j) {
      const int col = 4 * (sq + 4 * j);
      const bool cv = col < n_load;
      rdy[j] = cv ? *reinterpret_cast<const float4*>(DY + pc * ld_dy + col) : make_float4(0.f, 0.f, 0.f, 0.f);
      rzr[j] = cv ? *reinterpret_cast<const float4*>(Zr + pc * ld_z + col) : make_float4(0.f, 0.f, 0.f, 0.f);
    }
  };
  auto stage_write = [&](float* dzb) {
#pragma unroll
    for (int j = 0; j < 3; ++j) {
      const int col = 4 * (sq + 4 * j);
      float4 sa, sb, sc;
      if constexpr (NARROW) {
        sa = *reinterpret_cast<const float4*>(co_l + col);
        sb = *reinterpret_cast<const float4*>(co_l + 48 + col);
        sc = *reinterpret_cast<const float4*>(co_l + 96 + col);
      } else {
        sa = sa_r[j];
        sb = sb_r[j];
        sc = sc_r[j];
      }
      float4 v;
      v.x = rpv ? fmaf(sa.x, rdy[j].x, fmaf(sb.x, rzr[j].x, sc.x)) : 0.f;
      v.y = rpv ? fmaf(sa.y, rdy[j].y, fmaf(sb.y, rzr[j].y, sc.y)) : 0.f;
      v.z = rpv ? fmaf(sa.z, rdy[j].z, fmaf(sb.z, rzr[j].z, sc.z)) : 0.f;
      v.w = rpv ? fmaf(sa.w, rdy[j].w, fmaf(sb.w, rzr[j].w, sc.w)) : 0.f;
      *reinterpret_cast<float4*>(dzb + spix * 48 + col) = v;
      if (dz_out && rpv) *reinterpret_cast<float4*>(dz_out + (size_t)rp * 48 + col) = v;
    }
  };
  auto chunk_loop = [&](auto ngw_c) {
    constexpr int NGW = decltype(ngw_c)::value;
    constexpr int UQ = POOL ? 1 : 4;
    constexpr int NBUF = 2;
    constexpr int NS = POOL ? 4 : 1;
    constexpr int NB = 16 / UQ;
    constexpr int AHEAD = NBUF - 1;
    float2 xr[NBUF][UQ][NGW > 0 ? NGW : 1][NS];
    auto load_batch = [&](int chunk, int q0, float2 (&dst)[UQ][NGW > 0 ? NGW : 1][NS]) {
#pragma unroll
      for (int u = 0; u < UQ; ++u) {
        const int pc = min(chunk * 64 + 4 * (q0 + u) + kk, P - 1);
        const float* xp;
        if constexpr (POOL) {
          const int b = pc / (Ho * Wo), rem = pc - b * (Ho * Wo);
          const int oy = rem / Wo, ox = rem - oy * Wo;
          xp = X + ((size_t)(b * Hin + 2 * oy) * Win + 2 * ox) * ldx;
        } else {
          xp = X + (size_t)pc * ldx;
        }
#pragma unroll
        for (int i = 0; i < NGW; ++i)
#pragma unroll
          for (int sub = 0; sub < NS; ++sub)
            dst[u][i][sub] = *reinterpret_cast<const float2*>(xp + ((sub >> 1) * (size_t)Win + (sub & 1)) * ldx + coff[i]);
      }
    };
    stage_load(blockIdx.x);
    stage_write(dz_l[0]);
    if constexpr (NGW > 0) {
#pragma unroll
      for (int a = 0; a < AHEAD; ++a) load_batch(min((int)blockIdx.x, nchunks - 1), a * UQ, xr[a]);
    }
    __syncthreads();
    int it = 0;
    for (int chunk = blockIdx.x; chunk < nchunks; chunk += gridDim.x, ++it) {
      const float* dzb = dz_l[it & 1];
      stage_load(chunk + gridDim.x);
      float2 nx[2], ng[2];
      const int pn = chunk * 64 + 16 * wave + r;
      if constexpr (NARROW) {
        const size_t pc = (size_t)min(pn, P - 1);
        const float* xs = X + pc * ldx + na.k_lo + 4 * kq;
        const float* gs = na.G + pc * na.ldg + (na.ldg == 12 ? 0 : na.k_lo) + 4 * kq;
        nx[0] = *reinterpret_cast<const float2*>(xs);
        nx[1] = *reinterpret_cast<const float2*>(xs + 2);
        ng[0] = *reinterpret_cast<const float2*>(gs);
        ng[1] = *reinterpret_cast<const float2*>(gs + 2);
      }
      if constexpr (NGW > 0) {
        float bzq[2][3];
#pragma unroll
        for (int n = 0; n < 3; ++n) bzq[0][n] = dzb[kk * 48 + 16 * n + r];
#pragma unroll
        for (int bi = 0; bi < NB; ++bi) {
          const int q0 = bi * UQ;
          if (bi + AHEAD < NB)
            load_batch(chunk, q0 + AHEAD * UQ, xr[(bi + AHEAD) % NBUF]);
          else
            load_batch(min(chunk + (int)gridDim.x, nchunks - 1), (bi + AHEAD - NB) * UQ, xr[(bi + AHEAD) % NBUF]);
          __builtin_amdgcn_sched_barrier(0);
#pragma unroll
          for (int u = 0; u < UQ; ++u) {
            const int pl = 4 * (q0 + u) + kk;
            const bool pvu = chunk * 64 + pl < P;
            float bz[3];
#pragma unroll
            for (int n = 0; n < 3; ++n) bz[n] = bzq[(q0 + u) & 1][n];
            if (q0 + u + 1 < 16) {
#pragma unroll
              for (int n = 0; n < 3; ++n) bzq[(q0 + u + 1) & 1][n] = dzb[(pl + 4) * 48 + 16 * n + r];
            }
#pragma unroll
            for (int i = 0; i < NGW; ++i) {
              float av[2];
#pragma unroll
              for (int t = 0; t < 2; ++t) av[t] = 0.f;
#pragma unroll
              for (int sub = 0; sub < NS; ++sub) {
                const float2 xv = xr[bi % NBUF][u][i][sub];
                av[0] += fmaxf(fmaf(xv.x, sv[i][0], tv[i][0]), 0.f);
                av[1] += fmaxf(fmaf(xv.y, sv[i][1], tv[i][1]), 0.f);
              }
#pragma unroll
              for (int t = 0; t < 2; ++t) {
                if constexpr (POOL) av[t] *= 0.25f;
                if (!pvu) av[t] = 0.f;
              }
#pragma unroll
              for (int n = 0; n < 3; ++n)
#pragma unroll
                for (int t = 0; t < 2; ++t) acc[i][t][n] = mfma16(av[t], bz[n], acc[i][t][n]);
            }
          }
          __builtin_amdgcn_sched_barrier(0);
        }
      }
      if constexpr (NARROW) {
        asm volatile("" ::"v"(ng[0].x), "v"(ng[0].y), "v"(ng[1].x), "v"(ng[1].y), "v"(nx[0].x), "v"(nx[0].y), "v"(nx[1].x), "v"(nx[1].y));
        f32x4 an = f32x4{0.f, 0.f, 0.f, 0.f};
#pragma unroll
        for (int st = 0; st < 12; ++st) an = mfma16(wn_l[st * 64 + lane], dzb[(16 * wave + r) * 48 + 4 * st + kk], an);
        const bool nv = pn < P && kk < 3;
        const float xg[4] = {nx[0].x, nx[0].y, nx[1].x, nx[1].y}, gg[4] = {ng[0].x, ng[0].y, ng[1].x, ng[1].y};
        float o4[4];
#pragma unroll
        for (int g = 0; g < 4; ++g) {
          const float dam = (nv && fmaf(xg[g], nsk[g], ntk[g]) > 0.f) ? an[g] : 0.f;
          o4[g] = fmaf(nsk[g], dam, gg[g]);
          ns1[g] += (double)dam;
        }
        if (nv) *reinterpret_cast<float4*>(na.N12 + ((unsigned)pn * 12u + 4u * (unsigned)kk)) = make_float4(o4[0], o4[1], o4[2], o4[3]);
      }
      stage_write(dz_l[(it + 1) & 1]);
      eml::lds_barrier();
    }
  };
  switch (ngw) {
    case 0: chunk_loop(std::integral_constant<int, 0>{}); break;
    case 1: chunk_loop(std::integral_constant<int, 1>{}); break;
    case 2: chunk_loop(std::integral_constant<int, 2>{}); break;
    default: chunk_loop(std::integral_constant<int, MAXG>{}); break;
  }
  float* out = partial + (size_t)blockIdx.x * Kp * 48;
#pragma unroll
  for (int i = 0; i < MAXG; ++i) {
    const int cg = wave + 4 * i;
#pragma unroll
    for (int t = 0; t < 2; ++t)
#pragma unroll
      for (int g = 0; g < 4; ++g) {
        const int ch = GW * cg + 2 * (4 * kk + g) + t;
        if (cg < ngroups && ch < Kp) {
#pragma unroll
          for (int n = 0; n < 3; ++n) out[(size_t)ch * 48 + 16 * n + r] = acc[i][t][n][g];
        }
      }
  }
  if constexpr (NARROW) {
    __syncthreads();
    double* red = reinterpret_cast<double*>(&dz_l[0][0]);
#pragma unroll
    for (int g = 0; g < 4; ++g) {
#pragma unroll
      for (int o = 1; o < 16; o <<= 1) ns1[g] += shfl_xor_d(ns1[g], o);
      if (r == 0 && kk < 3) red[wave * 12 + 4 * kk + g] = ns1[g];
    }
    __syncthreads();
    if (tid < 12) {
      double* dst = na.partials + ((size_t)blockIdx.x * Kp + na.k_lo + tid) * 2;
      dst[0] = (red[tid] + red[12 + tid]) + (red[24 + tid] + red[36 + tid]);
      dst[1] = 0.0;
    }
  }
}

template <bool POOL, bool RES , int NCH = 4>
__global__ __launch_bounds__(256) void conv1x1_bwd_data_kernel(
    const float* __restrict__ DY, int ld_dy, const float* __restrict__ Zr, int ld_z, const float* __restrict__ cA,
    const float* __restrict__ cB, const float* __restrict__ cC, int Ko, const float* __restrict__ Wd,
    const float* __restrict__ X, int ldx, const float* __restrict__ scale1, const float* __restrict__ shift1,
    const float* __restrict__ mean, const float* __restrict__ istd, int P, int Hin, int Win, int Kp,
    float* __restrict__ Gd, int ldg, int accumulate, double* __restrict__ partials ) {
  extern __shared__ __attribute__((aligned(16))) float smem[];
  double* sacc = reinterpret_cast<double*>(smem);
  const int tid = threadIdx.x, lane = tid & 63, wave = tid >> 6;
  const int r = lane & 15, kk = lane >> 4;
// ... 846 lines not shown
    for (int u = 0; u < kUN; ++u) {
      const bool ok = live && p0 + (size_t)u * PW + slot < P;
      const float d[4] = {(ok && ou[u].x > 0.f) ? dy[u].x : 0.f, (ok && ou[u].y > 0.f) ? dy[u].y : 0.f,
                          (ok && ou[u].z > 0.f) ? dy[u].z : 0.f, (ok && ou[u].w > 0.f) ? dy[u].w : 0.f};
      const float xh[4] = {(rw[u].x - mu.x) * is.x, (rw[u].y - mu.y) * is.y, (rw[u].z - mu.z) * is.z, (rw[u].w - mu.w) * is.w};
#pragma unroll
      for (int g = 0; g < 4; ++g) {
        a1[g] += (double)d[g];
        a2[g] += (double)(d[g] * xh[g]);
      }
    }
  }
#pragma unroll
  for (int g = 0; g < 4; ++g) {
    red[wave][lane][2 * g] = live ? a1[g] : 0.0;
    red[wave][lane][2 * g + 1] = live ? a2[g] : 0.0;
  }
  __syncthreads();
  for (int e = tid; e < C * 2; e += 256) {
    const int c = e >> 1, k = e & 1, q = c >> 2, g = c & 3;
    double t = 0.0;
    for (int w = 0; w < 4; ++w)
      for (int sl = 0; sl < PW; ++sl) t += red[w][sl * CQ + q][2 * g + k];
    partials[(size_t)blockIdx.x * C * 2 + e] = t;
  }
}

__global__ __launch_bounds__(256) void norm0_bwd_stats_kernel(const float* __restrict__ Gd, int ldg, const float* __restrict__ Y0,
                                                              int ld_y0, const float* __restrict__ scale0,
                                                              const float* __restrict__ shift0, const float* __restrict__ sB,
                                                              const float* __restrict__ sC, int C, size_t P,
                                                              const float* __restrict__ mean, const float* __restrict__ istd,
                                                              double* __restrict__ partials ) {
  __shared__ double red[4][64][8];
  const int tid = threadIdx.x, lane = tid & 63, wave = tid >> 6;
  const int CQ = C >> 2, PW = 64 / CQ;
  const int slot = lane / CQ, quad = lane - slot * CQ;
  const bool live = slot < PW;
  auto ld4 = [&](const float* q) { return *reinterpret_cast<const float4*>(q + 4 * quad); };
  const float4 mu = ld4(mean), is = ld4(istd), s0 = ld4(scale0), t0 = ld4(shift0), b4 = ld4(sB), c4 = ld4(sC);
  double a1[4] = {0.0, 0.0, 0.0, 0.0}, a2[4] = {0.0, 0.0, 0.0, 0.0};
  constexpr int kUN = 4;
  const size_t step = (size_t)gridDim.x * 4 * kUN * PW;
  for (size_t p0 = ((size_t)blockIdx.x * 4 + wave) * kUN * PW; p0 < P; p0 += step) {
    float4 gv[kUN], yv[kUN];
#pragma unroll
    for (int u = 0; u < kUN; ++u) {
      const size_t p = p0 + (size_t)u * PW + slot;
      const size_t pc = p < P ? p : P - 1;
      gv[u] = *reinterpret_cast<const float4*>(Gd + pc * ldg + 4 * quad);
      yv[u] = *reinterpret_cast<const float4*>(Y0 + pc * ld_y0 + 4 * quad);
    }
#pragma unroll
    for (int u = 0; u < kUN; ++u) {
      const bool ok = live && p0 + (size_t)u * PW + slot < P;
      const float y[4] = {yv[u].x, yv[u].y, yv[u].z, yv[u].w}, g[4] = {gv[u].x, gv[u].y, gv[u].z, gv[u].w};
      const float sc[4] = {s0.x, s0.y, s0.z, s0.w}, sh[4] = {t0.x, t0.y, t0.z, t0.w};
      const float bb[4] = {b4.x, b4.y, b4.z, b4.w}, cc[4] = {c4.x, c4.y, c4.z, c4.w};
      const float mm[4] = {mu.x, mu.y, mu.z, mu.w}, ii[4] = {is.x, is.y, is.z, is.w};
#pragma unroll
      for (int e = 0; e < 4; ++e) {
        const float x = fmaxf(fmaf(y[e], sc[e], sh[e]), 0.f);
        const float dy = g[e] + fmaf(bb[e], x, cc[e]);
        const float d = (ok && x > 0.f) ? dy : 0.f;
        a1[e] += (double)d;
        a2[e] += (double)(d * ((y[e] - mm[e]) * ii[e]));
      }
    }
  }
#pragma unroll
  for (int g = 0; g < 4; ++g) {
    red[wave][lane][2 * g] = live ? a1[g] : 0.0;
    red[wave][lane][2 * g + 1] = live ? a2[g] : 0.0;
  }
  __syncthreads();
  for (int e = tid; e < C * 2; e += 256) {
    const int c = e >> 1, k = e & 1, q = c >> 2, g = c & 3;
    double t = 0.0;
    for (int w = 0; w < 4; ++w)
      for (int sl = 0; sl < PW; ++sl) t += red[w][sl * CQ + q][2 * g + k];
    partials[(size_t)blockIdx.x * C * 2 + e] = t;
  }
}

template <bool FUSED>
__global__ __launch_bounds__(256) void conv0_bwd_weight_kernel(
    const float* __restrict__ x, const float* __restrict__ Gd, int ldg, const float* __restrict__ X1, int ldx,
    const float* __restrict__ Y0, int C0, const float* __restrict__ cA, const float* __restrict__ cB,
    const float* __restrict__ cC, int B, int H, int W, float* __restrict__ partial ,
    const float* __restrict__ scale0, const float* __restrict__ shift0, const float* __restrict__ sB,
    const float* __restrict__ sC) {
  const int tid = threadIdx.x, lane = tid & 63, wave = tid >> 6;
  const int r = lane & 15, kk = lane >> 4;
  f32x4 acc[2][2];
#pragma unroll
  for (int i = 0; i < 2; ++i)
#pragma unroll
    for (int n = 0; n < 2; ++n) acc[i][n] = f32x4{0.f, 0.f, 0.f, 0.f};
  float ca[2], cb[2], cc[2], fs0[2] = {0.f, 0.f}, ft0[2] = {0.f, 0.f}, fb[2] = {0.f, 0.f}, fc[2] = {0.f, 0.f};
  bool ov[2];
#pragma unroll
  for (int n = 0; n < 2; ++n) {
    ov[n] = 16 * n + r < C0;
    ca[n] = ov[n] ? cA[16 * n + r] : 0.f;
    cb[n] = ov[n] ? cB[16 * n + r] : 0.f;
    cc[n] = ov[n] ? cC[16 * n + r] : 0.f;
    if constexpr (FUSED) {
      fs0[n] = ov[n] ? scale0[16 * n + r] : 0.f;
      ft0[n] = ov[n] ? shift0[16 * n + r] : 0.f;
      fb[n] = ov[n] ? sB[16 * n + r] : 0.f;
      fc[n] = ov[n] ? sC[16 * n + r] : 0.f;
    }
  }
  int ci[2], dyi[2], dxi[2];
  bool iv[2];
#pragma unroll
  for (int i = 0; i < 2; ++i) {
    const int t = 16 * i + r;
    iv[i] = t < 27;
    ci[i] = iv[i] ? t / 9 : 0;
    dyi[i] = iv[i] ? (t % 9) / 3 - 1 : 0;
    dxi[i] = iv[i] ? (t % 3) - 1 : 0;
  }
  const size_t P = (size_t)B * H * W, plane = (size_t)H * W;
  const size_t nq = (P + 3) >> 2;
  constexpr int kU = 4;
  for (size_t q0 = ((size_t)blockIdx.x * 4 + wave) * kU; q0 < nq; q0 += (size_t)gridDim.x * 4 * kU) {
    float av[kU][2], gv[kU][2], xv[kU][2], yv[kU][2];
    bool pvu[kU], inb[kU][2];
#pragma unroll
    for (int u = 0; u < kU; ++u) {
      const size_t p = 4 * (q0 + u) + kk;
      pvu[u] = p < P;
      const size_t pc = pvu[u] ? p : P - 1;
      const int b = (int)(pc / plane), rem = (int)(pc - (size_t)b * plane);
      const int yy = rem / W, xx = rem - yy * W;
#pragma unroll
      for (int i = 0; i < 2; ++i) {
        const int gy = yy + dyi[i], gx = xx + dxi[i];
        inb[u][i] = pvu[u] && iv[i] && gy >= 0 && gy < H && gx >= 0 && gx < W;
        const int gyc = min(max(gy, 0), H - 1), gxc = min(max(gx, 0), W - 1);
        av[u][i] = x[((size_t)(b * 3 + ci[i]) * H + gyc) * W + gxc];
      }
#pragma unroll
      for (int n = 0; n < 2; ++n) {
        const int o = ov[n] ? 16 * n + r : 0;
        gv[u][n] = Gd[pc * ldg + o];
        if constexpr (!FUSED) xv[u][n] = X1[pc * ldx + o];
        yv[u][n] = Y0[pc * C0 + o];
      }
    }
#pragma unroll
    for (int u = 0; u < kU; ++u) {
      float a[2], d[2];
#pragma unroll
      for (int i = 0; i < 2; ++i) a[i] = inb[u][i] ? av[u][i] : 0.f;
#pragma unroll
      for (int n = 0; n < 2; ++n) {
        float g;
        if constexpr (FUSED) {
          const float xx = fmaxf(fmaf(yv[u][n], fs0[n], ft0[n]), 0.f);
          g = xx > 0.f ? gv[u][n] + fmaf(fb[n], xx, fc[n]) : 0.f;
        } else {
          g = xv[u][n] > 0.f ? gv[u][n] : 0.f;
        }
        const float v = fmaf(ca[n], g, fmaf(cb[n], yv[u][n], cc[n]));
        d[n] = (pvu[u] && ov[n]) ? v : 0.f;
      }
#pragma unroll
      for (int i = 0; i < 2; ++i)
#pragma unroll
        for (int n = 0; n < 2; ++n) acc[i][n] = mfma16(a[i], d[n], acc[i][n]);
    }
  }
  float* out = partial + ((size_t)blockIdx.x * 4 + wave) * 1024;
#pragma unroll
  for (int i = 0; i < 2; ++i)
#pragma unroll
    for (int n = 0; n < 2; ++n)
#pragma unroll
      for (int g = 0; g < 4; ++g) out[(16 * i + 4 * kk + g) * 32 + 16 * n + r] = acc[i][n][g];
}

constexpr int kC0dTH = 8, kC0dTW = 32, kC0dC = 24;
constexpr int kC0dHW = kC0dTW + 2, kC0dNP = (kC0dTH + 2) * kC0dHW;
constexpr int kC0dLd = 28;
constexpr int kC0dPP = 256 / (kC0dC / 4);
constexpr int kC0dPasses = (kC0dNP + kC0dPP - 1) / kC0dPP;

template <bool FUSED>
__global__ __launch_bounds__(256) void conv0_bwd_data_kernel(
    const float* __restrict__ Gd, int ldg, const float* __restrict__ X1, int ldx, const float* __restrict__ Y0,
    const float* __restrict__ scale0, const float* __restrict__ shift0, const float* __restrict__ sB,
    const float* __restrict__ sC, const float* __restrict__ cA, const float* __restrict__ cB, const float* __restrict__ cC,
    const float* __restrict__ W0, int B, int H, int W, float* __restrict__ dX) {
  __shared__ __attribute__((aligned(16))) float dz[kC0dNP * kC0dLd];
  __shared__ __attribute__((aligned(16))) float wl[9 * 3 * kC0dC];
  const int tid = threadIdx.x;
  for (int e = tid; e < kC0dC * 27; e += 256) wl[((e % 9) * 3 + (e % 27) / 9) * kC0dC + e / 27] = W0[e];
  const int q = tid % (kC0dC / 4), s0 = tid / (kC0dC / 4);
  const bool stager = s0 < kC0dPP;
  const int o4 = 4 * q;
  const float4 ca = *reinterpret_cast<const float4*>(cA + o4), cb = *reinterpret_cast<const float4*>(cB + o4),
               cc = *reinterpret_cast<const float4*>(cC + o4);
  float4 fs0 = {0.f, 0.f, 0.f, 0.f}, ft0 = fs0, fb = fs0, fc = fs0;
  if constexpr (FUSED) {
    fs0 = *reinterpret_cast<const float4*>(scale0 + o4);
    ft0 = *reinterpret_cast<const float4*>(shift0 + o4);
    fb = *reinterpret_cast<const float4*>(sB + o4);
    fc = *reinterpret_cast<const float4*>(sC + o4);
  }
  const float cav[4] = {ca.x, ca.y, ca.z, ca.w}, cbv[4] = {cb.x, cb.y, cb.z, cb.w}, ccv[4] = {cc.x, cc.y, cc.z, cc.w};
  const float fsv[4] = {fs0.x, fs0.y, fs0.z, fs0.w}, ftv[4] = {ft0.x, ft0.y, ft0.z, ft0.w};
  const float fbv[4] = {fb.x, fb.y, fb.z, fb.w}, fcv[4] = {fc.x, fc.y, fc.z, fc.w};
  const int ty = tid / kC0dTW, tx = tid % kC0dTW;
  const int tiles_x = (W + kC0dTW - 1) / kC0dTW, tiles_y = (H + kC0dTH - 1) / kC0dTH;
  const size_t plane = (size_t)H * W;
  {
    const int b = (int)(blockIdx.x / (tiles_y * tiles_x));
    const int r = (int)(blockIdx.x - b * tiles_y * tiles_x);
    const int h0 = (r / tiles_x) * kC0dTH, w0 = (r % tiles_x) * kC0dTW;
    float4 gv[kC0dPasses], yv[kC0dPasses], xv[kC0dPasses];
    bool in[kC0dPasses];
#pragma unroll
    for (int k = 0; k < kC0dPasses; ++k) {
      const int s = s0 + k * kC0dPP;
      const int hy = h0 - 1 + s / kC0dHW, hx = w0 - 1 + s % kC0dHW;
      in[k] = stager && s < kC0dNP && hy >= 0 && hy < H && hx >= 0 && hx < W;
      const size_t p = (size_t)b * plane + (size_t)(in[k] ? hy : 0) * W + (in[k] ? hx : 0);
      gv[k] = in[k] ? *reinterpret_cast<const float4*>(Gd + p * ldg + o4) : float4{0.f, 0.f, 0.f, 0.f};
      yv[k] = in[k] ? *reinterpret_cast<const float4*>(Y0 + p * kC0dC + o4) : float4{0.f, 0.f, 0.f, 0.f};
      if constexpr (!FUSED) xv[k] = in[k] ? *reinterpret_cast<const float4*>(X1 + p * ldx + o4) : float4{0.f, 0.f, 0.f, 0.f};
    }
#pragma unroll
    for (int k = 0; k < kC0dPasses; ++k) {
      const int s = s0 + k * kC0dPP;
      if (!stager || s >= kC0dNP) continue;
      const float g4[4] = {gv[k].x, gv[k].y, gv[k].z, gv[k].w}, y4[4] = {yv[k].x, yv[k].y, yv[k].z, yv[k].w};
      float d[4];
#pragma unroll
      for (int e = 0; e < 4; ++e) {
        float g;
        if constexpr (FUSED) {
          const float xx = fmaxf(fmaf(y4[e], fsv[e], ftv[e]), 0.f);
          g = xx > 0.f ? g4[e] + fmaf(fbv[e], xx, fcv[e]) : 0.f;
        } else {
          const float x4[4] = {xv[k].x, xv[k].y, xv[k].z, xv[k].w};
          g = x4[e] > 0.f ? g4[e] : 0.f;
        }
        d[e] = in[k] ? fmaf(cav[e], g, fmaf(cbv[e], y4[e], ccv[e])) : 0.f;
      }
      *reinterpret_cast<float4*>(&dz[s * kC0dLd + o4]) = float4{d[0], d[1], d[2], d[3]};
    }
    __syncthreads();
    float acc[3] = {0.f, 0.f, 0.f};
#pragma unroll
    for (int ky = 0; ky < 3; ++ky)
#pragma unroll
      for (int kx = 0; kx < 3; ++kx) {
        const float* src = &dz[((ty + 2 - ky) * kC0dHW + (tx + 2 - kx)) * kC0dLd];
        const float* wt = &wl[(ky * 3 + kx) * 3 * kC0dC];
#pragma unroll
        for (int o4i = 0; o4i < kC0dC / 4; ++o4i) {
          const float4 v = *reinterpret_cast<const float4*>(src + 4 * o4i);
          const float vv[4] = {v.x, v.y, v.z, v.w};
#pragma unroll
          for (int c = 0; c < 3; ++c) {
            const float4 wq = *reinterpret_cast<const float4*>(wt + c * kC0dC + 4 * o4i);
            const float ww[4] = {wq.x, wq.y, wq.z, wq.w};
#pragma unroll
            for (int e = 0; e < 4; ++e) acc[c] = fmaf(ww[e], vv[e], acc[c]);
          }
        }
      }
    const int h = h0 + ty, w = w0 + tx;
    if (h < H && w < W) {
#pragma unroll
      for (int c = 0; c < 3; ++c) dX[((size_t)b * 3 + c) * plane + (size_t)h * W + w] = acc[c];
    }
  }
}

__global__ __launch_bounds__(256) void head_pool_bwd_kernel(const float* __restrict__ gp, const float* __restrict__ F,
                                                            int ldf, int C, int B, int H, int W, int k,
                                                            float* __restrict__ dF, int ldd) {
  const int Ho = H / k, Wo = W / k;
  const size_t total = (size_t)B * H * W * C;
  const float inv = 1.0f / (float)(k * k);
  for (size_t e = (size_t)blockIdx.x * 256 + threadIdx.x; e < total; e += (size_t)gridDim.x * 256) {
    const int c = (int)(e % C);
    const size_t p = e / C;
    const int xx = (int)(p % W);
    const size_t rest = p / W;
    const int yy = (int)(rest % H), b = (int)(rest / H);
    const int oy = yy / k, ox = xx / k;
    float v = 0.f;
    if (oy < Ho && ox < Wo && F[p * ldf + c] > 0.f) v = gp[(((size_t)b * C + c) * Ho + oy) * Wo + ox] * inv;
    dF[p * ldd + c] = v;
  }
}

}

__global__ __launch_bounds__(256) void bn_dgamma_direct_partial_kernel(
    const float* __restrict__ X, int ldx, long P, int Hin, int Win, int pool, const float* __restrict__ DY, int ld_dy,
    const float* __restrict__ Zr, int ld_z, const float* __restrict__ cA, const float* __restrict__ cB,
    const float* __restrict__ cC, int Cout, const float* __restrict__ W, int Cin, const float* __restrict__ scale1,
    const float* __restrict__ shift1, const float* __restrict__ mean, const float* __restrict__ istd,
    const int* __restrict__ cond, double* __restrict__ partial) {
  __shared__ int list[384];
  __shared__ int cnt;
  __shared__ float wcol[192], co[3][192];
  __shared__ double red[4];
  const int tid = threadIdx.x;
  if (tid == 0) cnt = 0;
  __syncthreads();
  for (int c = tid; c < Cin; c += 256)
    if (cond[c]) list[atomicAdd(&cnt, 1)] = c;
  __syncthreads();
  const int n = cnt;
  if (n == 0) return;
  for (int o = tid; o < Cout; o += 256) {
    co[0][o] = Zr ? cA[o] : 1.f;
    co[1][o] = Zr ? cB[o] : 0.f;
    co[2][o] = Zr ? cC[o] : 0.f;
  }
  const long per = (P + gridDim.x - 1) / gridDim.x, p_lo = (long)blockIdx.x * per, p_hi = min(P, p_lo + per);
  const int Ho = Hin >> 1, Wo = Win >> 1;
  for (int li = 0; li < n; ++li) {
    const int c = list[li];
    __syncthreads();
    for (int o = tid; o < Cout; o += 256) wcol[o] = W[(size_t)o * Cin + c];
    __syncthreads();
    const float s1 = scale1[c], t1 = shift1[c];
    const double mu = mean[c], is = istd[c];
    double acc = 0.0;
    for (long p = p_lo + tid; p < p_hi; p += 256) {
      const float x = X[(size_t)p * ldx + c];
      if (fmaf(x, s1, t1) > 0.f) {
        long pp = p;
        if (pool) {
          const long b = p / ((long)Hin * Win), rem = p - b * (long)Hin * Win;
          const int y = (int)(rem / Win), xx = (int)(rem - (long)y * Win);
          pp = (b * Ho + (y >> 1)) * Wo + (xx >> 1);
        }
        const float* dy = DY + (size_t)pp * ld_dy;
        const float* zr = Zr ? Zr + (size_t)pp * ld_z : dy;
        double d = 0.0;
        for (int o = 0; o < Cout; ++o) d += (double)wcol[o] * (double)fmaf(co[0][o], dy[o], fmaf(co[1][o], zr[o], co[2][o]));
        if (pool) d *= 0.25;
        acc += d * (((double)x - mu) * is);
      }
    }
#pragma unroll
    for (int o = 32; o > 0; o >>= 1) acc += shfl_xor_d(acc, o);
    if ((tid & 63) == 0) red[tid >> 6] = acc;
    __syncthreads();
    if (tid == 0) partial[(size_t)blockIdx.x * Cin + c] = (red[0] + red[1]) + (red[2] + red[3]);
  }
}

__global__ __launch_bounds__(256) void bn_dgamma_direct_reduce_kernel(const double* __restrict__ partial, int R, int Cin,
                                                                      const int* __restrict__ cond,
                                                                      float* __restrict__ dgamma) {
  const int c = blockIdx.x * 256 + threadIdx.x;
  if (c >= Cin || !cond[c]) return;
  double s = 0.0;
  for (int g = 0; g < R; ++g) s += partial[(size_t)g * Cin + c];
  dgamma[c] = (float)s;
}

template <bool DROP>
static int conv3x3_bwd_data_launch(const char* name, const float* G, int ldg, int c0, const float* W2, const float* Z,
                                   const float* zmean, const float* zistd, float* DZ, int B, int H, int W, double* partials,
                                   int grid, const float* X, int ldx, int cx, const float* sB, const float* sC, float* GF,
                                   unsigned long long seed, int layer, double p, eml_stream_t stream) {
  if (!G || !W2 || !Z || !zmean || !zistd || !DZ || !partials || B < 1 || H < 1 || W < 1 || grid < 1 || (c0 & 1) ||
      (ldg & 1))
    return eml::fail(EML_EINVAL, "%s: bad arguments", name);
  if (DROP || X) {
    if (!X || !sB || !sC || !GF || (ldx & 1)) return eml::fail(EML_EINVAL, "%s: fused affine needs X, sB, sC, GF", name);
    if (cx < 0 || (cx & 1)) return eml::fail(EML_EINVAL, "%s: cx must be even", name);
  }
  eml::DropKey dk{};
  if constexpr (DROP) {
    if (!(p >= 0.0 && p <= 1.0) || layer < 0)
      return eml::fail(EML_EINVAL, "%s: p must be in [0, 1] and layer >= 0 (p = %g, layer = %d)", name, p, layer);
    if ((long long)B * H * W > 0x7FFFFFFFll) return eml::fail(EML_EINVAL, "%s: B*H*W must fit the 32-bit pixel counter", name);
    dk = eml_drop_key(seed, layer, p);
  }
  const auto al16 = [](const void* q) { return (reinterpret_cast<uintptr_t>(q) & 15) == 0; };
  const bool wide = (ldg & 3) == 0 && (c0 & 3) == 0 && al16(G) &&
                    (!X || ((ldx & 3) == 0 && (cx & 3) == 0 && al16(X) && al16(sB) && al16(sC) && al16(GF)));
#define EML_LAUNCH_D3(FUSEV, WIDEV)                                                                                      \
  hipLaunchKernelGGL((conv3x3_bwd_data_kernel<FUSEV, WIDEV, DROP>), dim3(grid), dim3(kBD), 0, (hipStream_t)stream, G, ldg, c0, \
                     W2, Z, zmean, zistd, DZ, B, H, W, partials, X, ldx, cx, sB, sC, GF, dk)
  if (DROP || X) {
    if (wide) EML_LAUNCH_D3(true, true); else EML_LAUNCH_D3(true, false);
  } else if constexpr (!DROP) {
    if (wide) EML_LAUNCH_D3(false, true); else EML_LAUNCH_D3(false, false);
  }
#undef EML_LAUNCH_D3
  return eml::check_launch(name);
}

extern "C" int eml_dense_conv3x3_bwd_data_f32(const float* G, int ldg, int c0, const float* W2, const float* Z,
                                              const float* zmean, const float* zistd, float* DZ, int B, int H, int W,
                                              double* partials, int grid, const float* X, int ldx, int cx,
                                              const float* sB, const float* sC, float* GF, eml_stream_t stream) {
  return conv3x3_bwd_data_launch<false>("eml_dense_conv3x3_bwd_data_f32", G, ldg, c0, W2, Z, zmean, zistd, DZ, B, H, W, partials,
                                        grid, X, ldx, cx, sB, sC, GF, 0, 0, 0.0, stream);
}

extern "C" int eml_dense_conv3x3_bwd_data_drop_f32(const float* G, int ldg, int c0, const float* W2, const float* Z,
                                                   const float* zmean, const float* zistd, float* DZ, int B, int H, int W,
                                                   double* partials, int grid, const float* X, int ldx, int cx,
                                                   const float* sB, const float* sC, float* GF, unsigned long long seed,
                                                   int layer, double p, eml_stream_t stream) {
  return conv3x3_bwd_data_launch<true>("eml_dense_conv3x3_bwd_data_drop_f32", G, ldg, c0, W2, Z, zmean, zistd, DZ, B, H, W,
                                       partials, grid, X, ldx, cx, sB, sC, GF, seed, layer, p, stream);
}

extern "C" int eml_dense_conv3x3_bwd_weight_f32(const float* G, int ldg, int c0, const float* Z, const float* scale2,
                                                const float* shift2, int B, int H, int W, float* partial, float* dW2,
                                                int grid, eml_stream_t stream) {
  if (!G || !Z || !scale2 || !shift2 || !partial || !dW2 || B < 1 || H < 1 || W < 1 || grid < 1)
    return eml::fail(EML_EINVAL, "eml_dense_conv3x3_bwd_weight_f32: bad arguments");
  if ((ldg & 3) == 0 && (c0 & 3) == 0 && (reinterpret_cast<uintptr_t>(G) & 15) == 0) {
    const size_t lds = (size_t)(2 * kHH * kHW * kPSW + 2 * kGL) * sizeof(float);
    EML_ENSURE_LDS((&conv3x3_bwd_weight_kernel<true>), lds);
    hipLaunchKernelGGL(conv3x3_bwd_weight_kernel<true>, dim3(grid), dim3(kBW), lds, (hipStream_t)stream, G, ldg, c0, Z,
                       scale2, shift2, B, H, W, partial);
  } else {
    const size_t lds = (size_t)(2 * kHH * kHW * kPSW) * sizeof(float);
    EML_ENSURE_LDS((&conv3x3_bwd_weight_kernel<false>), lds);
    hipLaunchKernelGGL(conv3x3_bwd_weight_kernel<false>, dim3(grid), dim3(kBW), lds, (hipStream_t)stream, G, ldg, c0, Z,
                       scale2, shift2, B, H, W, partial);
  }
  int rc = eml::check_launch("eml_dense_conv3x3_bwd_weight_f32");
  if (rc) return rc;
  hipLaunchKernelGGL(reduce_rows_kernel, dim3(27 * 256 / 64), dim3(256), 0, (hipStream_t)stream, partial, 2 * grid,
                     (size_t)27 * 256, 1, 0, 0, 0, dW2);
  return eml::check_launch("eml_dense_conv3x3_bwd_weight_f32(reduce)");
}

#ifdef EML_STAMPS
extern "C" int eml_c3_read_stamps(unsigned long long* out, int reset) {
  if (hipMemcpyFromSymbol(out, HIP_SYMBOL(eml_c3_stamps), 8 * sizeof(unsigned long long)) != hipSuccess) return -1;
  if (reset) {
    const unsigned long long z[8] = {0};
    if (hipMemcpyToSymbol(HIP_SYMBOL(eml_c3_stamps), z, sizeof(z)) != hipSuccess) return -1;
  }
  return 0;
}
#endif
extern "C" int eml_dense_conv3x3_bwd_fused_supported(int ldg, int c0, int ldx, int cx) {
  return ((ldg & 1) == 0 && (c0 & 1) == 0 && (ldx & 1) == 0 && (cx & 1) == 0) ? 1 : 0;
}
template <bool DROP>
static int conv3x3_bwd_fused_launch(const char* name, const float* G, int ldg, int c0, const float* W2, const float* Z,
                                    const float* zmean, const float* zistd, float* DZ, int B, int H, int W, double* partials,
                                    int grid, const float* X, int ldx, int cx, const float* sB, const float* sC, float* GF,
                                    const float* scale2, const float* shift2, float* partialW, float* dW2, eml::DropKey dk,
                                    eml_stream_t stream) {
  if (!G || !W2 || !Z || !zmean || !zistd || !DZ || !partials || !X || !sB || !sC || !scale2 || !shift2 || !partialW ||
      !dW2 || B < 1 || H < 1 || W < 1 || grid < 1 || cx < 0)
    return eml::fail(EML_EINVAL, "%s: bad arguments", name);
  const auto al16 = [](const void* q) { return (reinterpret_cast<uintptr_t>(q) & 15) == 0; };
  if (!eml_dense_conv3x3_bwd_fused_supported(ldg, c0, ldx, cx) || !al16(G) || !al16(X) || !al16(GF) || !al16(Z) || !al16(scale2) ||
      !al16(shift2))
    return eml::fail(EML_EINVAL, "%s: needs even ldg, c0, ldx, cx and 16-byte aligned buffers", name);
  const bool a16 = (ldg & 3) == 0 && (c0 & 3) == 0 && (ldx & 3) == 0 && (cx & 3) == 0;
  const size_t lds = (size_t)(2 * kHH * kHW * kPSG + 2 * kTH * kTW * 48 + 27 * 3 * 64 + 32) * sizeof(float) + 8 * 48 * 2 * sizeof(double);
  const auto launch = [&](auto a16_c, auto gf_c) {
    const auto kernel = &conv3x3_bwd_fused_tp_kernel<decltype(a16_c)::value, DROP, decltype(gf_c)::value>;
    EML_ENSURE_LDS(kernel, lds);
    hipLaunchKernelGGL(kernel, dim3(grid), dim3(512), lds, (hipStream_t)stream, G, ldg, c0, W2, Z, zmean, zistd, DZ, B, H, W,
                       partials, X, ldx, cx, sB, sC, GF, scale2, shift2, partialW, dk);
  };
  if (a16) { if (GF) launch(std::true_type{}, std::true_type{}); else launch(std::true_type{}, std::false_type{}); }
  else     { if (GF) launch(std::false_type{}, std::true_type{}); else launch(std::false_type{}, std::false_type{}); }
  int rc = eml::check_launch(name);
  if (rc) return rc;
  hipLaunchKernelGGL(reduce_rows_kernel, dim3(21 * 256 / 64), dim3(256), 0, (hipStream_t)stream, partialW, grid,
                     (size_t)21 * 256, 3, 0, 0, 0, dW2);
  return eml::check_launch(DROP ? "eml_dense_conv3x3_bwd_fused_drop_f32(reduce)" : "eml_dense_conv3x3_bwd_fused_f32(reduce)");
}

extern "C" int eml_dense_conv3x3_bwd_fused_f32(const float* G, int ldg, int c0, const float* W2, const float* Z,
                                               const float* zmean, const float* zistd, float* DZ, int B, int H, int W,
                                               double* partials, int grid, const float* X, int ldx, int cx,
                                               const float* sB, const float* sC, float* GF, const float* scale2,
                                               const float* shift2, float* partialW, float* dW2, eml_stream_t stream) {
  return conv3x3_bwd_fused_launch<false>("eml_dense_conv3x3_bwd_fused_f32", G, ldg, c0, W2, Z, zmean, zistd, DZ, B, H, W, partials,
                                         grid, X, ldx, cx, sB, sC, GF, scale2, shift2, partialW, dW2, eml::DropKey{}, stream);
}

extern "C" int eml_dense_conv3x3_bwd_fused_drop_f32(const float* G, int ldg, int c0, const float* W2, const float* Z,
                                                    const float* zmean, const float* zistd, float* DZ, int B, int H, int W,
                                                    double* partials, int grid, const float* X, int ldx, int cx,
                                                    const float* sB, const float* sC, float* GF, const float* scale2,
                                                    const float* shift2, float* partialW, float* dW2, unsigned long long seed,
                                                    int layer, double p, eml_stream_t stream) {
  if (!(p >= 0.0 && p <= 1.0) || layer < 0)
    return eml::fail(EML_EINVAL, "eml_dense_conv3x3_bwd_fused_drop_f32: p must be in [0, 1] and layer >= 0 (p = %g, layer = %d)", p,
                     layer);
  if ((long long)B * H * W > 0x7FFFFFFFll)
    return eml::fail(EML_EINVAL, "eml_dense_conv3x3_bwd_fused_drop_f32: B*H*W must fit the 32-bit pixel counter");
  return conv3x3_bwd_fused_launch<true>("eml_dense_conv3x3_bwd_fused_drop_f32", G, ldg, c0, W2, Z, zmean, zistd, DZ, B, H, W,
                                        partials, grid, X, ldx, cx, sB, sC, GF, scale2, shift2, partialW, dW2,
                                        eml_drop_key(seed, layer, p), stream);
}

namespace {
__global__ __launch_bounds__(256) void dropout_mask_kernel(eml::DropKey dk, unsigned P, unsigned short* __restrict__ out) {
  for (unsigned q = blockIdx.x * 256u + threadIdx.x; q < P; q += gridDim.x * 256u) {
    unsigned m = 0;
#pragma unroll
    for (unsigned grp = 0; grp < 3; ++grp) {
      const uint4 d = eml::drop_draws(dk, q, grp);
#pragma unroll
      for (int w = 0; w < 4; ++w)
        if ((unsigned long long)eml::draw_word(d, w) >= dk.thr) m |= 1u << (4 * grp + w);
    }
    out[q] = (unsigned short)m;
  }
}
}

extern "C" int eml_dense_dropout_mask_u16(unsigned long long seed, int layer, double p, long P, unsigned short* mask,
                                          eml_stream_t stream) {
  if (!mask || P < 1 || P > 0x7FFFFFFFl || layer < 0 || !(p >= 0.0 && p <= 1.0))
    return eml::fail(EML_EINVAL, "eml_dense_dropout_mask_u16: bad arguments (mask null, P outside [1, 2^31), layer < 0 or p "
                                 "outside [0, 1])");
  const unsigned grid = (unsigned)std::min<long>((P + 255) / 256, 4096);
  hipLaunchKernelGGL(dropout_mask_kernel, dim3(grid), dim3(256), 0, (hipStream_t)stream, eml_drop_key(seed, layer, p), (unsigned)P,
                     mask);
  return eml::check_launch("eml_dense_dropout_mask_u16");
}

extern "C" int eml_dense_bn_bwd_finalize_f32(const double* partials, int R, int pstride, double count,
                                             const float* gamma, const float* mean, const float* istd, int C, int Cpad,
                                             int training, float* dgamma, float* dbeta, float* cA, float* cB,
                                             float* cC, float* sB, float* sC, int s_accumulate, int c_lo,
                                             int c_hi, const float* beta, const float* W, const float* dW, int w_rows,
                                             int* cond, int* any_cond, eml_stream_t stream) {
  if (!partials || !gamma || !mean || !istd || !dgamma || !dbeta || C < 1 || Cpad < C || R < 1 ||
      (cA && (!cB || !cC)) || (sB && !sC) || c_lo < 0 || c_hi <= c_lo)
    return eml::fail(EML_EINVAL, "eml_dense_bn_bwd_finalize_f32: bad arguments");
  if (W && (!dW || !beta || w_rows < 1))
    return eml::fail(EML_EINVAL, "eml_dense_bn_bwd_finalize_f32: W given without dW / beta / w_rows");
  if (c_hi > Cpad) c_hi = Cpad;
  hipLaunchKernelGGL(bn_bwd_finalize_kernel, dim3((c_hi - c_lo + 3) / 4), dim3(256), 0, (hipStream_t)stream, partials,
                     R, pstride, count, gamma, mean, istd, C, Cpad, training, dgamma, dbeta, cA, cB, cC, sB, sC,
                     s_accumulate, c_lo, c_hi, beta, W, dW, w_rows, W ? cond : nullptr, W ? any_cond : nullptr);
  return eml::check_launch("eml_dense_bn_bwd_finalize_f32");
}

extern "C" int eml_dense_bn_dgamma_direct_f32(const float* X, int ldx, long P, int Hin, int Win, int pool, const float* DY,
                                              int ld_dy, const float* Zr, int ld_z, const float* cA, const float* cB,
                                              const float* cC, int Cout, const float* W, int Cin, const float* scale1,
                                              const float* shift1, const float* mean, const float* istd, const int* cond,
                                              double* scratch, float* dgamma, int grid, eml_stream_t stream) {
  if (!X || !DY || !W || !scale1 || !shift1 || !mean || !istd || !cond || !scratch || !dgamma || P < 1 || grid < 1 ||
      Cin < 1 || Cin > 384 || Cout < 1 || Cout > 192 || Cin > ldx || Cout > ld_dy || (Zr && (!cA || !cB || !cC || Cout > ld_z)) ||
      (pool && ((Hin | Win) & 1)))
    return eml::fail(EML_EINVAL, "eml_dense_bn_dgamma_direct_f32: bad arguments (Cin <= 384, Cout <= 192, even maps when pooled)");
  hipLaunchKernelGGL(bn_dgamma_direct_partial_kernel, dim3(grid), dim3(256), 0, (hipStream_t)stream, X, ldx, P, Hin, Win,
                     pool, DY, ld_dy, Zr, ld_z, cA, cB, cC, Cout, W, Cin, scale1, shift1, mean, istd, cond, scratch);
  int rc = eml::check_launch("eml_dense_bn_dgamma_direct_f32(partial)");
  if (rc) return rc;
  hipLaunchKernelGGL(bn_dgamma_direct_reduce_kernel, dim3((Cin + 255) / 256), dim3(256), 0, (hipStream_t)stream, scratch,
                     grid, Cin, cond, dgamma);
  return eml::check_launch("eml_dense_bn_dgamma_direct_f32(reduce)");
}

extern "C" int eml_dense_conv1x1_bwd_weight_f32(const float* X, int ldx, long P, int Hin, int Win, int pool, int Kp,
                                                int Cin, const float* scale1, const float* shift1, const float* DY,
                                                int ld_dy, const float* Zr, int ld_z, const float* cA, const float* cB,
                                                const float* cC, int Cout, float* partial, float* dW, int grid,
                                                float* dz_out, const float* W1, int k_lo, const float* G, int ldg,
                                                float* N12, double* partials_n, eml_stream_t stream) {
  if (dz_out && (Cout != 48 || pool))
    return eml::fail(EML_EINVAL, "eml_dense_conv1x1_bwd_weight_f32: dz_out is for dense layers (Cout == 48, no pool)");
  if (N12 && (Cout != 48 || pool || !W1 || !G || !partials_n || k_lo < 0 || (k_lo & 1) || k_lo + 12 > Cin || (ldg & 1) ||
              (ldg != 12 && k_lo + 12 > ldg)))
    return eml::fail(EML_EINVAL, "eml_dense_conv1x1_bwd_weight_f32: fused narrow pass needs a dense layer, W1, G, partials_n "
                                 "and an even k_lo with k_lo + 12 <= Cin (k_lo=%d, Cin=%d)", k_lo, Cin);
  if (!X || !scale1 || !shift1 || !DY || !Zr || !cA || !cB || !cC || !partial || !dW || P < 1 || grid < 1 || Kp < 32 ||
      (Kp & 15) || Cin > Kp || Cout < 1)
    return eml::fail(EML_EINVAL, "eml_dense_conv1x1_bwd_weight_f32: bad arguments");
  const int nchunks = (Cout + 47) / 48;
  for (int ch = 0; ch < nchunks; ++ch) {
    const int n0 = ch * 48, nv = (Cout - n0 < 48) ? Cout - n0 : 48;
    int n_load = ((ld_dy < ld_z ? ld_dy : ld_z) - n0) & ~3;
    if (n_load > 48) n_load = 48;
    if (n_load < nv) return eml::fail(EML_EINVAL, "eml_dense_conv1x1_bwd_weight_f32: DY/Zr rows narrower than Cout");
    const NarrowArgs na{W1, G, N12, partials_n, Cin, k_lo, ldg};
    if (pool)
      hipLaunchKernelGGL((conv1x1_bwd_weight_kernel<true, false>), dim3(grid), dim3(256), 0, (hipStream_t)stream, X, ldx,
                         (int)P, Hin, Win, Kp, scale1, shift1, DY + n0, ld_dy, Zr + n0, ld_z, cA + n0, cB + n0, cC + n0,
                         nv, n_load, partial, nullptr, na);
    else if (N12)
      hipLaunchKernelGGL((conv1x1_bwd_weight_kernel<false, true>), dim3(grid), dim3(256), 0, (hipStream_t)stream, X, ldx,
                         (int)P, Hin, Win, Kp, scale1, shift1, DY + n0, ld_dy, Zr + n0, ld_z, cA + n0, cB + n0, cC + n0,
                         nv, n_load, partial, dz_out, na);
    else
      hipLaunchKernelGGL((conv1x1_bwd_weight_kernel<false, false>), dim3(grid), dim3(256), 0, (hipStream_t)stream, X, ldx,
                         (int)P, Hin, Win, Kp, scale1, shift1, DY + n0, ld_dy, Zr + n0, ld_z, cA + n0, cB + n0, cC + n0,
                         nv, n_load, partial, dz_out, na);
    int rc = eml::check_launch("eml_dense_conv1x1_bwd_weight_f32");
    if (rc) return rc;
    hipLaunchKernelGGL(reduce_rows_kernel, dim3((Cin * 48 + 63) / 64), dim3(256), 0, (hipStream_t)stream, partial,
                       grid, (size_t)Kp * 48, 0, Cin, nv, n0, dW);
    rc = eml::check_launch("eml_dense_conv1x1_bwd_weight_f32(reduce)");
    if (rc) return rc;
  }
  return EML_OK;
}

extern "C" int eml_dense_permute_w1_bwd_f32(const float* W, int Cout, int Cin, int Kp, int Ko, float* Wd,
                                            eml_stream_t stream) {
  if (!W || !Wd || Cout < 1 || Cin < 1 || Kp < Cin || (Kp & 15) || Ko < Cout || (Ko & 15))
    return eml::fail(EML_EINVAL, "eml_dense_permute_w1_bwd_f32: bad arguments");
  hipLaunchKernelGGL(permute_w1_bwd_kernel, dim3(64), dim3(256), 0, (hipStream_t)stream, W, Cout, Cin, Kp, Ko, Wd);
  return eml::check_launch("eml_dense_permute_w1_bwd_f32");
}

extern "C" int eml_dense_conv1x1_bwd_data_f32(const float* DY, int ld_dy, const float* Zr, int ld_z, const float* cA,
                                              const float* cB, const float* cC, int Ko, const float* Wd,
                                              const float* X, int ldx, const float* scale1, const float* shift1,
                                              const float* mean, const float* istd, long P, int Hin, int Win, int pool,
                                              int Kp, float* G, int ldg, int accumulate, double* partials, int grid,
                                              const unsigned short* relu_mask16, eml_stream_t stream) {
  if (!DY || !Zr || !cA || !cB || !cC || !Wd || (!relu_mask16 && (!X || !mean || !istd)) || !scale1 || !shift1 || !G ||
      !partials || P < 1 || grid < 1 || (Kp & 15) || (Ko & 15) || Ko > ld_dy || Ko > ld_z || (ld_dy & 3) || (ld_z & 3) ||
      (ldx & 3) || (ldg & 3) || (!relu_mask16 && Kp > ldx) || Kp > ldg)
    return eml::fail(EML_EINVAL, "eml_dense_conv1x1_bwd_data_f32: bad arguments");
  if (relu_mask16 && !(pool && Ko != 48))
    return eml::fail(EML_EINVAL, "eml_dense_conv1x1_bwd_data_f32: relu_mask16 is for the transition form (pool, Ko != 48)");
  const size_t lds = (size_t)4 * Kp * 2 * sizeof(double);
#define EML_LAUNCH_BWD_DATA(POOLV, RESV, NCHV)                                                                        \
  hipLaunchKernelGGL((conv1x1_bwd_data_kernel<POOLV, RESV, NCHV>), dim3(grid), dim3(256), lds, (hipStream_t)stream, DY, \
                     ld_dy, Zr, ld_z, cA, cB, cC, Ko, Wd, X, ldx, scale1, shift1, mean, istd, (int)P, Hin, Win, Kp, G, \
                     ldg, accumulate, partials)
  if (pool) {
    if (Ko == 48) {
      EML_LAUNCH_BWD_DATA(true, true, 4);
    } else {
      const size_t lds_t = lds + (size_t)(4 * Kp + 3 * Ko + 4 * 16 * 36) * sizeof(float);
#define EML_LAUNCH_TRANSITION(ACCV, MSKV)                                                                              \
  do {                                                                                                                \
    EML_ENSURE_LDS((&transition_bwd_data_kernel<2, 2, ACCV, MSKV>), lds_t);                                 \
    hipLaunchKernelGGL((transition_bwd_data_kernel<2, 2, ACCV, MSKV>), dim3(grid), dim3(256), lds_t,                   \
                       (hipStream_t)stream, DY, ld_dy, Zr, ld_z, cA, cB, cC, Ko, Wd, X, ldx, scale1, shift1, mean, istd, \
                       (int)P, Hin, Win, Kp, G, ldg, partials, relu_mask16);                                           \
  } while (0)
#define EML_LAUNCH_TRANSITION_RES(NJOV)                                                                                \
  do {                                                                                                                \
    EML_ENSURE_LDS((&transition_bwd_data_kernel<2, 2, false, true, NJOV>), lds_t);                                     \
    hipLaunchKernelGGL((transition_bwd_data_kernel<2, 2, false, true, NJOV>), dim3(grid), dim3(256), lds_t,            \
                       (hipStream_t)stream, DY, ld_dy, Zr, ld_z, cA, cB, cC, Ko, Wd, X, ldx, scale1, shift1, mean, istd, \
                       (int)P, Hin, Win, Kp, G, ldg, partials, relu_mask16);                                           \
  } while (0)
      if (relu_mask16 && !accumulate && Ko == 112) EML_LAUNCH_TRANSITION_RES(7);
      else if (relu_mask16 && !accumulate && Ko == 160) EML_LAUNCH_TRANSITION_RES(10);
      else if (relu_mask16 && !accumulate && Ko == 176) EML_LAUNCH_TRANSITION_RES(11);
      else if (relu_mask16) {
        if (accumulate) EML_LAUNCH_TRANSITION(true, true); else EML_LAUNCH_TRANSITION(false, true);
      } else {
        if (accumulate) EML_LAUNCH_TRANSITION(true, false); else EML_LAUNCH_TRANSITION(false, false);
      }
#undef EML_LAUNCH_TRANSITION
#undef EML_LAUNCH_TRANSITION_RES
    }
  } else {
    if (Ko == 48) EML_LAUNCH_BWD_DATA(false, true, 2); else EML_LAUNCH_BWD_DATA(false, false, 4);
  }
#undef EML_LAUNCH_BWD_DATA
  return eml::check_launch("eml_dense_conv1x1_bwd_data_f32");
}

namespace {
int launch_bwd_data_multi(int n_layers, const float* const* DZ, const float* const* Zr, const float* const* cA,
                          const float* const* cB, const float* const* cC, const float* const* Wd,
                          const float* const* scale1, const float* const* shift1, double* const* partials, const int* Kp,
                          const float* X, int ldx, const float* mean, const float* istd, long P, int k_lo, int k_hi,
                          float* G, int ldg, int grid, const unsigned long long* const* relu_masks, float* top,
                          eml_stream_t stream) {
  if (top && (n_layers != 2 || !relu_masks || Zr || k_lo != 0 || k_hi < 24 || (k_hi & 3) || P * 12 > 2147483647L))
    return eml::fail(EML_EINVAL, "eml_dense_conv1x1_bwd_data_multi_top_f32: the compact top-24 output needs two layers, "
                                 "relu_masks, materialised dz, k_lo == 0 and k_hi >= 24, a multiple of 4 (k_hi=%d)", k_hi);
  if (n_layers < 1 || n_layers > 2 || !DZ || !Wd || !scale1 || !shift1 || !partials ||
      !Kp || (!relu_masks && (!X || !mean || !istd)) || !G || P < 1 || grid < 1 || k_lo < 0 || k_hi <= k_lo ||
      (ldx & 3) || (ldg & 3))
    return eml::fail(EML_EINVAL, "eml_dense_conv1x1_bwd_data_multi_f32: bad arguments");
  const bool raw = Zr == nullptr;
  if (!raw && (!cA || !cB || !cC))
    return eml::fail(EML_EINVAL, "eml_dense_conv1x1_bwd_data_multi_f32: Zr given without cA/cB/cC");
  if (relu_masks && !raw)
    return eml::fail(EML_EINVAL, "eml_dense_conv1x1_bwd_data_multi_f32: relu_masks needs the materialised dz (Zr == NULL)");
  BwdLayer L[2];
  const unsigned long long* Mk[2] = {nullptr, nullptr};
  int kmax = 0;
  for (int j = 0; j < 2; ++j) {
    const int s = j < n_layers ? j : 0;
    const unsigned long long* mk = relu_masks ? relu_masks[s] : nullptr;
    Mk[j] = mk;
    L[j] = raw ? BwdLayer{DZ[s], nullptr, nullptr, nullptr, nullptr, Wd[s], scale1[s], shift1[s], partials[s], Kp[s]}
               : BwdLayer{DZ[s], Zr[s], cA[s], cB[s], cC[s], Wd[s], scale1[s], shift1[s], partials[s], Kp[s]};
    if (!DZ[s] || (!raw && !Zr[s]) || !Wd[s] || !partials[s] || (relu_masks && !mk) || (Kp[s] & 15) ||
        (!relu_masks && Kp[s] > ldx) || Kp[s] > ldg)
      return eml::fail(EML_EINVAL, "eml_dense_conv1x1_bwd_data_multi_f32: bad layer %d", s);
    if (Kp[s] > kmax) kmax = Kp[s];
  }
  if (((k_hi + 15) & ~15) > kmax) return eml::fail(EML_EINVAL, "eml_dense_conv1x1_bwd_data_multi_f32: range beyond Kp");
  const size_t lds = (size_t)n_layers * 4 * kmax * 2 * sizeof(double) + (size_t)(2 + 2 * n_layers) * kmax * sizeof(float);
  if (lds > 80 * 1024) return eml::fail(EML_EINVAL, "eml_dense_conv1x1_bwd_data_multi_f32: Kp=%d does not fit LDS", kmax);
#define EML_LAUNCH_MULTI(NLV, MTV, RAWV, MSKV)                                                                       \
  do {                                                                                                              \
    EML_ENSURE_LDS((&conv1x1_bwd_data_multi_kernel<NLV, MTV, RAWV, MSKV>), lds);                                 \
    hipLaunchKernelGGL((conv1x1_bwd_data_multi_kernel<NLV, MTV, RAWV, MSKV>), dim3(grid), dim3(256), lds,            \
                       (hipStream_t)stream, L[0], L[1], X, ldx, mean, istd, (int)P, k_lo, k_hi, G, ldg, kmax,        \
                       Mk[0], Mk[1], (float*)nullptr);                                                              \
  } while (0)
  if (n_layers == 1) {
    if (relu_masks) EML_LAUNCH_MULTI(1, 4, true, true);
    else if (raw) EML_LAUNCH_MULTI(1, 4, true, false);
    else EML_LAUNCH_MULTI(1, 4, false, false);
  } else if (top) {
    EML_ENSURE_LDS((&conv1x1_bwd_data_multi_kernel<2, 2, true, true, true>), lds);
    hipLaunchKernelGGL((conv1x1_bwd_data_multi_kernel<2, 2, true, true, true>), dim3(grid), dim3(256), lds,
                       (hipStream_t)stream, L[0], L[1], X, ldx, mean, istd, (int)P, k_lo, k_hi, G, ldg, kmax, Mk[0], Mk[1],
                       top);
  } else {
    if (relu_masks) EML_LAUNCH_MULTI(2, 2, true, true);
    else if (raw) EML_LAUNCH_MULTI(2, 2, true, false);
    else EML_LAUNCH_MULTI(2, 2, false, false);
  }
#undef EML_LAUNCH_MULTI
  return eml::check_launch("eml_dense_conv1x1_bwd_data_multi_f32");
}
}

extern "C" int eml_dense_conv1x1_bwd_data_multi_f32(int n_layers, const float* const* DZ, const float* const* Zr,
                                                    const float* const* cA, const float* const* cB,
                                                    const float* const* cC, const float* const* Wd,
                                                    const float* const* scale1, const float* const* shift1,
                                                    double* const* partials, const int* Kp, const float* X, int ldx,
                                                    const float* mean, const float* istd, long P, int k_lo, int k_hi,
                                                    float* G, int ldg, int grid,
                                                    const unsigned long long* const* relu_masks, eml_stream_t stream) {
  return launch_bwd_data_multi(n_layers, DZ, Zr, cA, cB, cC, Wd, scale1, shift1, partials, Kp, X, ldx, mean, istd, P, k_lo,
                               k_hi, G, ldg, grid, relu_masks, nullptr, stream);
}

extern "C" int eml_dense_conv1x1_bwd_data_multi_top_f32(const float* const* DZ, const float* const* Wd,
                                                        const float* const* scale1, const float* const* shift1,
                                                        double* const* partials, const int* Kp, long P, int k_hi,
                                                        float* G, int ldg, int grid,
                                                        const unsigned long long* const* relu_masks, float* top,
                                                        eml_stream_t stream) {
  if (!top) return eml::fail(EML_EINVAL, "eml_dense_conv1x1_bwd_data_multi_top_f32: top is NULL");
  return launch_bwd_data_multi(2, DZ, nullptr, nullptr, nullptr, nullptr, Wd, scale1, shift1, partials, Kp, nullptr, 0,
                               nullptr, nullptr, P, 0, k_hi, G, ldg, grid, relu_masks, top, stream);
}

extern "C" int eml_dense_conv1x1_bwd_narrow_f32(const float* DZ, const float* W1, int Cin, int k_lo, const float* X,
                                                int ldx, const float* scale1, const float* shift1, const float* mean,
                                                const float* istd, long P, const float* G, int ldg, float* N12,
                                                double* partials, int Kp, int grid, eml_stream_t stream) {
  if (!DZ || !W1 || !X || !scale1 || !shift1 || !mean || !istd || !G || !N12 || !partials || P < 1 || grid < 1 ||
      k_lo < 0 || (k_lo & 1) || k_lo + 12 > Cin || Cin > Kp || (ldx & 1) || (ldg & 1) || Kp > ldx || Kp > ldg)
    return eml::fail(EML_EINVAL, "eml_dense_conv1x1_bwd_narrow_f32: bad arguments");
  hipLaunchKernelGGL((conv1x1_bwd_narrow_kernel<4>), dim3(grid), dim3(256), 0, (hipStream_t)stream, DZ, W1, Cin, k_lo, X,
                     ldx, scale1, shift1, mean, istd, (int)P, G, ldg, N12, partials, Kp);
  return eml::check_launch("eml_dense_conv1x1_bwd_narrow_f32");
}

extern "C" int eml_dense_grad_materialize_f32(float* G, int ldg, const float* X, int ldx, const float* sB,
                                              const float* sC, int c0, int n, long P, eml_stream_t stream) {
  if (!G || !X || !sB || !sC || P < 1 || n < 2 || (n & 1) || (c0 & 1) || (ldg & 1) || (ldx & 1))
    return eml::fail(EML_EINVAL, "eml_dense_grad_materialize_f32: bad arguments");
  const size_t total = (size_t)P * (n >> 1);
  const int grid = (int)((total + 255) / 256 < 8192 ? (total + 255) / 256 : 8192);
  hipLaunchKernelGGL(grad_materialize_kernel, dim3(grid), dim3(256), 0, (hipStream_t)stream, G, ldg, X, ldx, sB, sC, c0,
                     n, (size_t)P);
  return eml::check_launch("eml_dense_grad_materialize_f32");
}

extern "C" int eml_dense_bn_bwd_stats_f32(const float* DY, int ld_dy, const float* raw, int ld_raw, const float* out,
                                          int ld_out, int relu, int C, long P, const float* mean, const float* istd,
                                          double* partials, int grid, eml_stream_t stream) {
  if (!DY || !raw || !mean || !istd || !partials || (relu && !out) || C < 1 || C > 384 || P < 1 || grid < 1)
    return eml::fail(EML_EINVAL, "eml_dense_bn_bwd_stats_f32: bad arguments");
  auto a16 = [](const void* q) { return (reinterpret_cast<size_t>(q) & 15) == 0; };
  if (C <= 32 && (C & 3) == 0 && ((ld_dy | ld_raw | (relu ? ld_out : 0)) & 3) == 0 && a16(DY) && a16(raw) && (!relu || a16(out)) &&
      a16(mean) && a16(istd)) {
    hipLaunchKernelGGL(bn_bwd_stats_small_kernel, dim3(grid), dim3(256), 0, (hipStream_t)stream, DY, ld_dy, raw, ld_raw, out, ld_out,
                       relu, C, (size_t)P, mean, istd, partials);
    return eml::check_launch("eml_dense_bn_bwd_stats_f32");
  }
  const size_t lds = (size_t)4 * ((C + 63) / 64) * 64 * 2 * sizeof(double);
  hipLaunchKernelGGL(bn_bwd_stats_kernel, dim3(grid), dim3(256), lds, (hipStream_t)stream, DY, ld_dy, raw, ld_raw, out,
                     ld_out, relu, C, (size_t)P, mean, istd, partials);
  return eml::check_launch("eml_dense_bn_bwd_stats_f32");
}

extern "C" int eml_dense_conv0_bwd_weight_f32(const float* x, const float* G, int ldg, const float* X1, int ldx,
                                              const float* Y0, int C0, const float* cA, const float* cB,
                                              const float* cC, int B, int H, int W, float* partial, float* dW0,
                                              int grid, eml_stream_t stream) {
  if (!x || !G || !X1 || !Y0 || !cA || !cB || !cC || !partial || !dW0 || C0 < 1 || C0 > 32 || B < 1 || grid < 1)
    return eml::fail(EML_EINVAL, "eml_dense_conv0_bwd_weight_f32: bad arguments");
  hipLaunchKernelGGL(conv0_bwd_weight_kernel<false>, dim3(grid), dim3(256), 0, (hipStream_t)stream, x, G, ldg, X1, ldx, Y0, C0,
                     cA, cB, cC, B, H, W, partial, nullptr, nullptr, nullptr, nullptr);
  int rc = eml::check_launch("eml_dense_conv0_bwd_weight_f32");
  if (rc) return rc;
  hipLaunchKernelGGL(reduce_rows_kernel, dim3(27 * 32 / 64 + 1), dim3(256), 0, (hipStream_t)stream, partial, grid * 4,
                     (size_t)1024, 2, 0, C0, 0, dW0);
  return eml::check_launch("eml_dense_conv0_bwd_weight_f32(reduce)");
}

extern "C" int eml_dense_head_pool_bwd_f32(const float* gpooled, const float* F, int ldf, int C, int B, int H, int W,
                                           int k, float* dF, int ldd, eml_stream_t stream) {
  if (!gpooled || !F || !dF || C < 1 || B < 1 || k < 1) return eml::fail(EML_EINVAL, "eml_dense_head_pool_bwd_f32: bad arguments");
  const size_t total = (size_t)B * H * W * C;
  const int grid = (int)((total + 255) / 256 < 4096 ? (total + 255) / 256 : 4096);
  hipLaunchKernelGGL(head_pool_bwd_kernel, dim3(grid), dim3(256), 0, (hipStream_t)stream, gpooled, F, ldf, C, B, H, W, k,
                     dF, ldd);
  return eml::check_launch("eml_dense_head_pool_bwd_f32");
}

extern "C" int eml_dense_norm0_bwd_stats_f32(const float* G, int ldg, const float* Y0, int ld_y0, const float* scale0,
                                             const float* shift0, const float* sB, const float* sC, int C, long P,
                                             const float* mean, const float* istd, double* partials, int grid,
                                             eml_stream_t stream) {
  auto a16 = [](const void* q) { return (reinterpret_cast<size_t>(q) & 15) == 0; };
  if (!G || !Y0 || !scale0 || !shift0 || !sB || !sC || !mean || !istd || !partials || C < 4 || C > 32 || (C & 3) || P < 1 ||
      grid < 1 || ((ldg | ld_y0) & 3) || !a16(G) || !a16(Y0) || !a16(scale0) || !a16(shift0) || !a16(sB) || !a16(sC) || !a16(mean) ||
      !a16(istd))
    return eml::fail(EML_EINVAL, "eml_dense_norm0_bwd_stats_f32: bad arguments (C a multiple of 4 <= 32, 16-byte aligned operands)");
  hipLaunchKernelGGL(norm0_bwd_stats_kernel, dim3(grid), dim3(256), 0, (hipStream_t)stream, G, ldg, Y0, ld_y0, scale0, shift0, sB,
                     sC, C, (size_t)P, mean, istd, partials);
  return eml::check_launch("eml_dense_norm0_bwd_stats_f32");
}

extern "C" int eml_dense_conv0_bwd_weight_fused_f32(const float* x, const float* G, int ldg, const float* Y0, int C0,
                                                    const float* scale0, const float* shift0, const float* sB, const float* sC,
                                                    const float* cA, const float* cB, const float* cC, int B, int H, int W,
                                                    float* partial, float* dW0, int grid, eml_stream_t stream) {
  if (!x || !G || !Y0 || !scale0 || !shift0 || !sB || !sC || !cA || !cB || !cC || !partial || !dW0 || C0 < 1 || C0 > 32 || B < 1 ||
      grid < 1)
    return eml::fail(EML_EINVAL, "eml_dense_conv0_bwd_weight_fused_f32: bad arguments");
  hipLaunchKernelGGL(conv0_bwd_weight_kernel<true>, dim3(grid), dim3(256), 0, (hipStream_t)stream, x, G, ldg, nullptr, 0, Y0, C0, cA,
                     cB, cC, B, H, W, partial, scale0, shift0, sB, sC);
  int rc = eml::check_launch("eml_dense_conv0_bwd_weight_fused_f32");
  if (rc) return rc;
  hipLaunchKernelGGL(reduce_rows_kernel, dim3(27 * 32 / 64 + 1), dim3(256), 0, (hipStream_t)stream, partial, grid * 4,
                     (size_t)1024, 2, 0, C0, 0, dW0);
  return eml::check_launch("eml_dense_conv0_bwd_weight_fused_f32(reduce)");
}

extern "C" int eml_dense_conv0_bwd_data_f32(const float* G, int ldg, const float* X1, int ldx, const float* Y0, int C0,
                                            const float* scale0, const float* shift0, const float* sB, const float* sC,
                                            const float* cA, const float* cB, const float* cC, const float* W0, int B, int H,
                                            int W, float* dX, eml_stream_t stream) {
  auto a16 = [](const void* q) { return (reinterpret_cast<size_t>(q) & 15) == 0; };
  const bool fused = X1 == nullptr;
  if (!G || !Y0 || !cA || !cB || !cC || !W0 || !dX || (fused && (!scale0 || !shift0 || !sB || !sC)))
    return eml::fail(EML_EINVAL, "eml_dense_conv0_bwd_data_f32: null pointer");
  if (C0 != kC0dC || B < 1 || H < 1 || W < 1 || ldg < C0 || (ldg & 3) || (!fused && (ldx < C0 || (ldx & 3))))
    return eml::fail(EML_EINVAL, "eml_dense_conv0_bwd_data_f32: bad shape (C0 == 24, B, H, W >= 1, ldg / ldx >= 24 and multiples of 4)");
  if (!a16(G) || !a16(Y0) || (!fused && !a16(X1)) || !a16(cA) || !a16(cB) || !a16(cC) ||
      (fused && (!a16(scale0) || !a16(shift0) || !a16(sB) || !a16(sC))))
    return eml::fail(EML_EINVAL, "eml_dense_conv0_bwd_data_f32: G, X1, Y0 and the coefficient vectors must be 16-byte aligned");
  const size_t tiles = (size_t)B * ((H + kC0dTH - 1) / kC0dTH) * ((W + kC0dTW - 1) / kC0dTW);
  if (tiles > 0x7fffffff) return eml::fail(EML_EINVAL, "eml_dense_conv0_bwd_data_f32: more than 2^31 - 1 tiles of 8 x 32 pixels");
  const int grid = (int)tiles;
  if (fused)
    hipLaunchKernelGGL(conv0_bwd_data_kernel<true>, dim3(grid), dim3(256), 0, (hipStream_t)stream, G, ldg, nullptr, 0, Y0,
                       scale0, shift0, sB, sC, cA, cB, cC, W0, B, H, W, dX);
  else
    hipLaunchKernelGGL(conv0_bwd_data_kernel<false>, dim3(grid), dim3(256), 0, (hipStream_t)stream, G, ldg, X1, ldx, Y0,
                       nullptr, nullptr, nullptr, nullptr, cA, cB, cC, W0, B, H, W, dX);
  return eml::check_launch("eml_dense_conv0_bwd_data_f32");
}
```

include/emlight_hip_ext.h:

```cpp
#ifndef EMLIGHT_HIP_EXT_H
#define EMLIGHT_HIP_EXT_H

#include "emlight_hip.h"

#ifdef __cplusplus
extern "C" {
#endif

int eml_pano_warp_f32(const float* pano, int B, int H, int W, int h, int w, double theta_deg, double phi_deg, double move,
                      const double* params_dev, float* out, double* coords, eml_stream_t stream);

size_t eml_pano_warp_bwd_work_floats(int B, int H, int W, int h, int w, int want_dpano, int want_dparams);
int eml_pano_warp_bwd_f32(const float* grad_out, const float* pano, int B, int H, int W, int h, int w, double theta_deg,
                          double phi_deg, double move, const double* params_dev, float* dpano, double* dparams, float* work,
                          eml_stream_t stream);

size_t eml_sphere_render_bwd_work_floats(int B, int H, int W, int S);
int eml_sphere_render_bwd_f32(const float* grad_out, int B, int H, int W, int S, double view_azimuth_deg, int materials_mask,
                              double phong_m, const int* mirror_csr_ptr, const int* mirror_csr_src, const float* mirror_csr_w,
                              float* dpano, float* work, eml_stream_t stream);

int eml_sphere_mirror_taps_f32(int H, int W, int S, double view_azimuth_deg, int* idx, float* wgt, eml_stream_t stream);

int eml_gm_anchor_cost_f32(const void* depth, int depth_is_f64, int B, int N, float* anchors_out, float* M_out,
                           eml_stream_t stream);

int eml_sinkhorn_fwd_cost_f32(const float* x, const float* y, const float* M, const float* Mt,
                              const float* alpha, const float* beta, double blur, double scaling, int p,
                              double diameter, const float* range_lo_hi, float* eps_out, int* n_eps_out,
                              float* diameter_out, float* loss, float* gx, float* gy, float* work, int B, int N,
                              int D, int flags, double rho, float* lam_out, long cost_stride, eml_stream_t stream);

int eml_sphere_max_pool_fwd_f32(const float* x, const int* idx, const float* wgt, float* y, unsigned char* arg, int B,
                                int n_src, int n_dst, int C, eml_stream_t stream);

int eml_sphere_max_pool_bwd_f32(const float* gy, const unsigned char* arg, const int* csr_ptr, const int* csr_src,
                                const float* csr_w, float* gx, int B, int n_src, int n_dst, int C, eml_stream_t stream);

int eml_sphere_conv_small_dbias_f32(const float* dY, const float* Yact, float act_slope, float* partial, float* db, int B,
                                    int Po, int C, int O, eml_stream_t stream);

size_t eml_env_prefilter_work_floats(int B, int H, int W, int Ho, int L);
int eml_env_prefilter_f32(const float* pano, int B, int H, int W, int Ho, int L, const double* lobes, float* out, float* work,
                          eml_stream_t stream);

int eml_gbuffer_shade_f32(const float* pano, int H, const float* e_diffuse, int Hd, long d_stride, const float* e_phong, int Hg,
                          long g_stride, const float* normal, const float* coverage, const float* kd, const float* ks,
                          const float* km, int B, int h, int w, double fov_deg, double view_azimuth_deg, float* shaded,
                          const float* background, const float* exposure, double gamma, float* composite,
                          eml_stream_t stream);

size_t eml_env_prefilter_bwd_work_floats(int B, int H, int W, int Ho, int L);
int eml_env_prefilter_bwd_f32(const float* grad_out, int B, int H, int W, int Ho, int L, const double* lobes, float* dpano,
                              float* work, eml_stream_t stream);

size_t eml_gbuffer_shade_bwd_work_floats(int B, int H, int Hd, int Hg, int h, int w, int want_dpano, int want_d_e_diffuse,
                                         int want_d_e_phong);
int eml_gbuffer_shade_bwd_f32(const float* grad_out, const float* pano, int H, const float* e_diffuse, int Hd, long d_stride,
                              const float* e_phong, int Hg, long g_stride, const float* normal, const float* coverage,
                              const float* kd, const float* ks, const float* km, int B, int h, int w, double fov_deg,
                              double view_azimuth_deg, const float* shaded, const float* exposure, double gamma, float* dkd,
                              float* dks, float* dkm, float* d_e_diffuse, float* d_e_phong, float* dpano, float* dshaded,
                              float* work, eml_stream_t stream);

size_t eml_pano_warp_depth_work_floats(int B, int H, int W);
int eml_pano_warp_depth_f32(const float* pano, const float* depth, int B, int H, int W, int h, int w, double theta_deg,
                            double phi_deg, double move, const double* params_dev, int steps, int bisections, float* out_pano,
                            float* out_depth, double* hit, float* work, eml_stream_t stream);

int eml_gt_anchor_depth_f64(const float* depth, const int* csr_ptr, const int* csr_pix, int B, int H, int W, int N, double* out,
                            eml_stream_t stream);

size_t eml_ground_shadow_work_floats(int B, int H, int h, int w, int K);
int eml_ground_shadow_f32(const float* pano, int B, int H, int W, const float* plane, int plane_stride, const float* occluders,
                          int K, int h, int w, double fov_deg, double view_azimuth_deg, const float* image, float* ratio,
                          float* shadowed, float* work, eml_stream_t stream);

#ifdef __cplusplus
}
#endif

#endif
```

Measured before the change: 566.4 images/s.

## Merge dense-layer backward tail kernels into fewer combined launches

Adds merged tail kernels for the dense-block backward pass. The conv3x3 weight-gradient reduce is folded into the BN2 finalize, and the BN1 finalize of a layer pair is combined with the conv1x1 weight reduce. The dgamma-direct pass for both layers of a pair now runs in one paired launch. The goal is to cut the many small kernel launches and separate reduction passes per dense layer. The cost is more complex kernels and a doubled dgamma scratch buffer.

```diff
diff --git a/emlight_amd/RegressionNetwork/dense_engine.py b/emlight_amd/RegressionNetwork/dense_engine.py
--- a/emlight_amd/RegressionNetwork/dense_engine.py
+++ b/emlight_amd/RegressionNetwork/dense_engine.py
@@ -137,6 +137,7 @@
 
 class HipDenseEncoder:
     GRID_MAX = 1024
+    bwd_tail = "merged"
 
     @staticmethod
     def check_supported(model):
diff --git a/emlight_amd/RegressionNetwork/dense_engine_bwd.py b/emlight_amd/RegressionNetwork/dense_engine_bwd.py
--- a/emlight_amd/RegressionNetwork/dense_engine_bwd.py
+++ b/emlight_amd/RegressionNetwork/dense_engine_bwd.py
@@ -5,6 +5,9 @@
 
 from .. import _lib
 from .._knobs import knob_choice, knob_flag
+
+
+_TAIL_ENTRIES = ("eml_dense_conv3x3_bwd_tail_f32", "eml_dense_bn1_tail_f32", "eml_dense_bn_dgamma_direct_pair_f32")
 
 
 def _r16(v):
@@ -40,7 +43,7 @@
         self.condT = [torch.zeros(blk["trans"]["Kp"], **i32) for blk in ws.blocks]
         self.any_ill = torch.zeros(1, **i32)
         self.dg_grid = 128
-        self.dg_scratch = torch.empty(self.dg_grid * kp, dtype=torch.float64, device=dev)
+        self.dg_scratch = torch.empty(2 * self.dg_grid * kp, dtype=torch.float64, device=dev)
         self.side = None
         if enc.overlap_wgrad(dev):
             self.side = torch.cuda.Stream(device=dev)
@@ -103,6 +106,9 @@
     direct = knob_choice("EML_DGAMMA_DIRECT", "always", ("always", "never")) != "never"
     c3_fold = knob_flag("EML_C3_FOLD", True)
     c3_gf = knob_flag("EML_C3_GF", False)
+    if enc.bwd_tail not in ("merged", "separate"):
+        raise ValueError("HipDenseEncoder.bwd_tail must be 'merged' or 'separate', not %r" % (enc.bwd_tail,))
+    merged = enc.bwd_tail == "merged" and all(hasattr(L, n) for n in _TAIL_ENTRIES)
     bw.any_ill.zero_()
 
     def dgamma_direct(blk, X_ld, Pin, Hin, Win, pool, DY, ld_dy, Zr, ld_z, co, Cout, conv, Cin, scale1, shift1, cond, bn):
@@ -163,23 +169,31 @@
                  cond=bw.condT[bi])
         dgamma_direct(blk, ld, P, Hb, Wb, 1, dY, ld_dy, tr["T"], Ko, coefs[0], cout, T.conv, ctot, tr["scale"], tr["shift"],
                       bw.condT[bi], T.norm)
-        def conv2_backward(l, slot, n12=False, narrow_lo=None, top=False):
+        def c3_operand(l, n12, top):
+            return (p(bw.N12), 12, 0) if n12 else (p(top2[1]), 12, 0) if top else (p(Gbuf), ld, blk["layers"][l]["Cin"])
+
+        def c3_fused(l, n12, top):
+            g = c3_operand(l, n12, top)
+            return (bw.side is None and c3_fold
+                    and L.eml_dense_conv3x3_bwd_fused_supported(g[1], g[2], ld, blk["layers"][l]["Cin"]) == 1)
+
+        def conv2_backward(l, slot, n12=False, narrow_lo=None, top=False, tail=False):
             lay = blk["layers"][l]
             Lm = getattr(mod, "denselayer%d" % (l + 1))
             cin, kp, z, dz = lay["Cin"], lay["Kp"], blk["Z"][l], bw.DZ[slot]
-            gsrc = (p(bw.N12), 12, 0) if n12 else (p(top2[1]), 12, 0) if top else (p(Gbuf), ld, cin)
+            gsrc = c3_operand(l, n12, top)
             r = ring[0] = (ring[0] + 1) % bw.ring
             if bw.side is not None and bw.ev_done[r] is not None:
                 main.wait_event(bw.ev_done[r])
-            fold = (bw.side is None and c3_fold
-                    and L.eml_dense_conv3x3_bwd_fused_supported(gsrc[1], gsrc[2], ld, cin) == 1)
+            fold = c3_fused(l, n12, top)
             q = ws.drop_plan[bi][l] if ws.drop_plan is not None else 0.0
             drop = (ws.drop_key, gl0 + l, q) if q > 0 else ()
             if fold:
                 fn = "eml_dense_conv3x3_bwd_fused_drop_f32" if drop else "eml_dense_conv3x3_bwd_fused_f32"
                 _lib.check(getattr(L, fn)(*gsrc, p(Lm.conv2.weight), p(z), p(lay["zmean"]), p(lay["zistd"]), p(dz), B, Hb, Wb,
                                           p(part), G3d, p(blk["X"]), ld, cin, p(sB), p(sC), p(bw.gf12(r)) if c3_gf else None,
-                                          p(lay["scale2"]), p(lay["shift2"]), p(bw.partW), gr(Lm.conv2.weight), *drop, st), fn)
+                                          p(lay["scale2"]), p(lay["shift2"]), p(bw.partW),
+                                          None if tail else gr(Lm.conv2.weight), *drop, st), fn)
             else:
                 fn = "eml_dense_conv3x3_bwd_data_drop_f32" if drop else "eml_dense_conv3x3_bwd_data_f32"
                 _lib.check(getattr(L, fn)(*gsrc, p(Lm.conv2.weight), p(z), p(lay["zmean"]), p(lay["zistd"]), p(dz), B, Hb, Wb,
@@ -201,11 +215,17 @@
                 if bw.ev_done[r] is None:
                     bw.ev_done[r] = torch.cuda.Event()
                 bw.ev_done[r].record(bw.side)
-            finalize(G3d, 96, P, Lm.norm2, lay["zmean"], lay["zistd"], 48, 48, coef=slot)
             a, b, c = coefs[slot]
+            if tail:
+                _lib.check(L.eml_dense_conv3x3_bwd_tail_f32(
+                    p(bw.partW), G3d, gr(Lm.conv2.weight), p(part), float(P), p(Lm.norm2.weight), p(lay["zmean"]),
+                    p(lay["zistd"]), gr(Lm.norm2.weight), gr(Lm.norm2.bias), p(a), p(b), p(c), st),
+                    "eml_dense_conv3x3_bwd_tail_f32")
+            else:
+                finalize(G3d, 96, P, Lm.norm2, lay["zmean"], lay["zistd"], 48, 48, coef=slot)
             _lib.check(L.eml_dense_conv1x1_bwd_weight_f32(
                 p(blk["X"]), ld, P, Hb, Wb, 0, kp, cin, p(lay["scale1"]), p(lay["shift1"]), p(dz), 48, p(z), 48,
-                p(a), p(b), p(c), 48, p(bw.partW), gr(Lm.conv1.weight), Gw, p(dz),
+                p(a), p(b), p(c), 48, p(bw.partW), None if tail else gr(Lm.conv1.weight), Gw, p(dz),
                 *((p(Lm.conv1.weight), narrow_lo, *((p(top2[0]), 12) if top else (p(Gbuf), ld)), p(bw.N12),
                    p(bw.part2[slot])) if narrow_lo is not None
                   else (None, 0, None, 0, None, None)), st), "eml_dense_conv1x1_bwd_weight_f32")
@@ -240,23 +260,58 @@
             dgamma_direct(blk, ld, P, Hb, Wb, 0, bw.DZ[slot], 48, None, 0, None, 48, Lm.conv1, lay["Cin"], lay["scale1"],
                           lay["shift1"], bw.cond[bi][l], Lm.norm1)
 
+        def bn1_tail(first, l, Lm, slot, c_lo, c_hi, rows):
+            lay = blk["layers"][l]
+            A = (None, 0, 0, 0, None, None, None, None, None, None, None, 0)
+            if first is not None:
+                la_, Lma_, slot_a, a_hi = first
+                ya = blk["layers"][la_]
+                A = (p(bw.part2[slot_a]), Gd, ya["Kp"], ya["Cin"], p(Lma_.norm1.weight), p(Lma_.norm1.bias),
+                     p(Lma_.conv1.weight), gr(Lma_.conv1.weight), gr(Lma_.norm1.weight), gr(Lma_.norm1.bias),
+                     p(bw.cond[bi][la_]), a_hi)
+            _lib.check(L.eml_dense_bn1_tail_f32(
+                float(P), p(blk["mean"]), p(blk["istd"]), p(sB), p(sC), p(bw.any_ill), *A,
+                p(bw.partW), Gw, p(bw.part2[slot]), rows, lay["Kp"], lay["Cin"], p(Lm.norm1.weight), p(Lm.norm1.bias),
+                p(Lm.conv1.weight), gr(Lm.conv1.weight), gr(Lm.norm1.weight), gr(Lm.norm1.bias), p(bw.cond[bi][l]),
+                c_lo, c_hi, st), "eml_dense_bn1_tail_f32")
+
+        def bn1_direct_pair(la, Lma, lb, Lmb):
+            if not direct:
+                return
+            args = []
+            for l_, Lm_, slot in ((la, Lma, 0), (lb, Lmb, 1)):
+                y = blk["layers"][l_]
+                args += [p(bw.DZ[slot]), p(Lm_.conv1.weight), y["Cin"], p(y["scale1"]), p(y["shift1"]), p(bw.cond[bi][l_]),
+                         gr(Lm_.norm1.weight)]
+            _lib.check(L.eml_dense_bn_dgamma_direct_pair_f32(p(blk["X"]), ld, P, p(blk["mean"]), p(blk["istd"]), *args,
+                                                             p(bw.dg_scratch), bw.dg_grid, st),
+                       "eml_dense_bn_dgamma_direct_pair_f32")
+
         l = len(blk["layers"]) - 1
         have_top = False
         while l >= 0:
             if l >= 1:
                 la, lb = l, l - 1
                 cin_a, cin_b = blk["layers"][la]["Cin"], blk["layers"][lb]["Cin"]
-                Lma = conv2_backward(la, 0, narrow_lo=cin_b, top=have_top)
-                bn1_finalize(la, Lma, 0, cin_b, cin_a, rows=Gw)
-                Lmb = conv2_backward(lb, 1, n12=True)
+                tail = merged and c3_fused(la, False, have_top) and c3_fused(lb, True, False)
+                Lma = conv2_backward(la, 0, narrow_lo=cin_b, top=have_top, tail=tail)
+                if tail:
+                    bn1_tail(None, la, Lma, 0, cin_b, cin_a, Gw)
+                else:
+                    bn1_finalize(la, Lma, 0, cin_b, cin_a, rows=Gw)
+                Lmb = conv2_backward(lb, 1, n12=True, tail=tail)
                 to_top = (lb >= 2 and blk["layers"][la]["mask"] is not None and bw.side is None
                           and cin_b >= 24 and cin_b % 4 == 0)
                 dgrad([la, lb], [0, 1], 0, cin_b, top=to_top)
                 have_top = to_top
-                bn1_finalize(la, Lma, 0, 0, cin_b)
-                bn1_finalize(lb, Lmb, 1, 0, blk["layers"][lb]["Kp"])
-                bn1_direct(la, Lma, 0)
-                bn1_direct(lb, Lmb, 1)
+                if tail:
+                    bn1_tail((la, Lma, 0, cin_b), lb, Lmb, 1, 0, blk["layers"][lb]["Kp"], Gd)
+                    bn1_direct_pair(la, Lma, lb, Lmb)
+                else:
+                    bn1_finalize(la, Lma, 0, 0, cin_b)
+                    bn1_finalize(lb, Lmb, 1, 0, blk["layers"][lb]["Kp"])
+                    bn1_direct(la, Lma, 0)
+                    bn1_direct(lb, Lmb, 1)
                 l -= 2
             else:
                 Lm0 = conv2_backward(l, 0)
diff --git a/emlight_amd/_lib.py b/emlight_amd/_lib.py
--- a/emlight_amd/_lib.py
+++ b/emlight_amd/_lib.py
@@ -255,6 +255,15 @@
     "eml_ground_shadow_work_floats": (ctypes.c_size_t, [_int, _int, _int, _int, _int]),
     "eml_ground_shadow_f32": (_int, [_f32p, _int, _int, _int, _f32p, _int, _f32p, _int, _int, _int, ctypes.c_double,
                                      ctypes.c_double, _f32p, _f32p, _f32p, _f32p, _stream]),
+    "eml_dense_conv3x3_bwd_tail_f32": (_int, [_f32p, _int, _f32p, _f64p, ctypes.c_double, _f32p, _f32p, _f32p, _f32p, _f32p,
+                                              _f32p, _f32p, _f32p, _stream]),
+    "eml_dense_bn1_tail_f32": (_int, [ctypes.c_double, _f32p, _f32p, _f32p, _f32p, _i32p,
+                                      _f64p, _int, _int, _int, _f32p, _f32p, _f32p, _f32p, _f32p, _f32p, _i32p, _int,
+                                      _f32p, _int, _f64p, _int, _int, _int, _f32p, _f32p, _f32p, _f32p, _f32p, _f32p, _i32p,
+                                      _int, _int, _stream]),
+    "eml_dense_bn_dgamma_direct_pair_f32": (_int, [_f32p, _int, ctypes.c_long, _f32p, _f32p,
+                                                   _f32p, _f32p, _int, _f32p, _f32p, _i32p, _f32p,
+                                                   _f32p, _f32p, _int, _f32p, _f32p, _i32p, _f32p, _f64p, _int, _stream]),
 }
 
 _lock = threading.Lock()
diff --git a/emlight_amd/csrc/dense_bwd.hip b/emlight_amd/csrc/dense_bwd.hip
--- a/emlight_amd/csrc/dense_bwd.hip
+++ b/emlight_amd/csrc/dense_bwd.hip
@@ -770,26 +770,57 @@
 }
 
 
-__global__ __launch_bounds__(256) void bn_bwd_finalize_kernel(
-    const double* __restrict__ partials, int R, int pstride, double count, const float* __restrict__ gamma,
-    const float* __restrict__ mean, const float* __restrict__ istd, int C, int Cpad, int training,
-    float* __restrict__ dgamma, float* __restrict__ dbeta, float* __restrict__ cA, float* __restrict__ cB,
-    float* __restrict__ cC, float* __restrict__ sB, float* __restrict__ sC, int s_accumulate, int c_lo, int c_hi,
-    const float* __restrict__ beta, const float* __restrict__ Wc, const float* __restrict__ dWc, int w_rows,
-    int* __restrict__ cond , int* __restrict__ any_cond ) {
-  const int lane = threadIdx.x & 63, wave = threadIdx.x >> 6;
-  const int c = c_lo + blockIdx.x * 4 + wave;
-  if (c >= Cpad || c >= c_hi) return;
-  float a = 0.f, b = 0.f, d = 0.f;
+struct BnFinArgs {
+  const double* partials;
+  int R, pstride;
+  double count;
+  const float *gamma, *mean, *istd;
+  int C, Cpad, training;
+  float *dgamma, *dbeta, *cA, *cB, *cC, *sB, *sC;
+  int s_accumulate;
+  const float *beta, *Wc, *dWc;
+  int w_rows;
+  int *cond , *any_cond ;
+};
+
+struct BnFinSums {
+  double S1, S2, Q;
+};
+template <bool QREG>
+__device__ __forceinline__ BnFinSums bn_finalize_sums(const BnFinArgs& A, const int c, const int lane) {
+  const double* __restrict__ partials = A.partials;
+  const int R = A.R, pstride = A.pstride, C = A.C, w_rows = A.w_rows;
+  const float* __restrict__ Wc = A.Wc;
+  const float* __restrict__ dWc = A.dWc;
+  double S1 = 0.0, S2 = 0.0, Q = 0.0;
   if (c < C) {
-    double S1 = 0.0, S2 = 0.0;
+#pragma unroll 8
     for (int g = lane; g < R; g += 64) {
       S1 += partials[(size_t)g * pstride + 2 * c];
       S2 += partials[(size_t)g * pstride + 2 * c + 1];
     }
-    double Q = 0.0;
-    if (Wc)
-      for (int o = lane; o < w_rows; o += 64) Q += (double)Wc[(size_t)o * C + c] * (double)dWc[(size_t)o * C + c];
+    if constexpr (!QREG) {
+      if (Wc)
+        for (int o = lane; o < w_rows; o += 64) Q += (double)Wc[(size_t)o * C + c] * (double)dWc[(size_t)o * C + c];
+    }
+  }
+  return BnFinSums{S1, S2, Q};
+}
+
+template <bool QREG>
+__device__ __forceinline__ void bn_finalize_finish(const BnFinArgs& A, const int c, const int lane, const BnFinSums sums,
+                                                   const float dw) {
+  const int C = A.C, w_rows = A.w_rows;
+  const double count = A.count;
+  const float* __restrict__ gamma = A.gamma;
+  const float* __restrict__ beta = A.beta;
+  const float* __restrict__ Wc = A.Wc;
+  float a = 0.f, b = 0.f, d = 0.f;
+  if (c < C) {
+    double S1 = sums.S1, S2 = sums.S2, Q = sums.Q;
+    if constexpr (QREG) {
+      if (Wc && lane < w_rows) Q += (double)Wc[(size_t)lane * C + c] * (double)dw;
+    }
 #pragma unroll
     for (int o = 32; o > 0; o >>= 1) {
       S1 += __shfl_xor(S1, o, 64);
@@ -799,40 +830,55 @@
     if (Wc) {
       const double ga0 = gamma[c], bs = (double)beta[c] * S1, num = Q - bs;
       S2 = fabs(ga0) >= 1e-12 ? num / ga0 : 0.0;
-      if (cond && lane == 0) {
+      if (A.cond && lane == 0) {
         const int ill = fabs(ga0) < 1e-3 * fabs((double)beta[c]) || ga0 == 0.0;
-        cond[c] = ill;
-        if (ill && any_cond) *any_cond = 1;
+        A.cond[c] = ill;
+        if (ill && A.any_cond) *A.any_cond = 1;
       }
     }
     if (lane == 0) {
-      dgamma[c] = (float)S2;
-      dbeta[c] = (float)S1;
-    }
-    const double ga = gamma[c], is = istd[c], mu = mean[c];
+      A.dgamma[c] = (float)S2;
+      A.dbeta[c] = (float)S1;
+    }
+    const double ga = gamma[c], is = A.istd[c], mu = A.mean[c];
     a = (float)(ga * is);
-    if (training) {
+    if (A.training) {
       b = (float)(-ga * is * is * S2 / count);
       d = (float)(-ga * is * S1 / count + ga * is * is * S2 / count * mu);
     }
   }
   if (lane != 0) return;
-  if (cA) {
-    cA[c] = a;
-    cB[c] = b;
-    cC[c] = d;
-  }
-  if (sB) {
-    sB[c] = (s_accumulate ? sB[c] : 0.f) + b;
-    sC[c] = (s_accumulate ? sC[c] : 0.f) + d;
-  }
-}
-
-__global__ __launch_bounds__(256) void reduce_rows_kernel(const float* __restrict__ partial, int R, size_t row_stride,
-                                                          int mode, int dim0, int dim1, int n0,
-                                                          float* __restrict__ out) {
+  if (A.cA) {
+    A.cA[c] = a;
+    A.cB[c] = b;
+    A.cC[c] = d;
+  }
+  if (A.sB) {
+    A.sB[c] = (A.s_accumulate ? A.sB[c] : 0.f) + b;
+    A.sC[c] = (A.s_accumulate ? A.sC[c] : 0.f) + d;
+  }
+}
+
+template <bool QREG>
+__device__ __forceinline__ void bn_finalize_channel(const BnFinArgs& A, const int c, const int lane, const float dw) {
+  bn_finalize_finish<QREG>(A, c, lane, bn_finalize_sums<QREG>(A, c, lane), dw);
+}
+
+__device__ __forceinline__ void bn_finalize_block(const BnFinArgs& A, const int c_lo, const int c_hi, const int block) {
+  const int lane = threadIdx.x & 63, wave = threadIdx.x >> 6;
+  const int c = c_lo + block * 4 + wave;
+  if (c >= A.Cpad || c >= c_hi) return;
+  bn_finalize_channel<false>(A, c, lane, 0.f);
+}
+
+__global__ __launch_bounds__(256) void bn_bwd_finalize_kernel(const BnFinArgs A, int c_lo, int c_hi) {
+  bn_finalize_block(A, c_lo, c_hi, blockIdx.x);
+}
+
+__device__ __forceinline__ void reduce_rows_block(const float* __restrict__ partial, int R, size_t row_stride, int mode,
+                                                  int dim0, int dim1, int n0, float* __restrict__ out, const int block) {
   __shared__ double red[4][64];
-  const int tid = threadIdx.x, e = blockIdx.x * 64 + (tid & 63), slice = tid >> 6;
+  const int tid = threadIdx.x, e = block * 64 + (tid & 63), slice = tid >> 6;
   size_t src = 0, dst = 0;
   bool valid = false;
   if (mode == 0) {
@@ -858,12 +904,58 @@
   }
   double s = 0.0;
   if (valid) {
-#pragma unroll 8
+#pragma unroll 16
     for (int r = slice; r < R; r += 4) s += (double)partial[(size_t)r * row_stride + src];
   }
   red[slice][tid & 63] = s;
   __syncthreads();
   if (slice == 0 && valid) out[dst] = (float)((red[0][tid] + red[1][tid]) + (red[2][tid] + red[3][tid]));
+}
+
+__global__ __launch_bounds__(256) void reduce_rows_kernel(const float* __restrict__ partial, int R, size_t row_stride,
+                                                          int mode, int dim0, int dim1, int n0,
+                                                          float* __restrict__ out) {
+  reduce_rows_block(partial, R, row_stride, mode, dim0, dim1, n0, out, blockIdx.x);
+}
+
+
+constexpr int kC3TailReduceBlocks = 21 * 256 / 64, kC3TailBlocks = kC3TailReduceBlocks + 48 / 4;
+__global__ __launch_bounds__(256) void conv3x3_bwd_tail_kernel(const float* __restrict__ partialW, int R,
+                                                               float* __restrict__ dW2, const BnFinArgs A) {
+  if (blockIdx.x < kC3TailReduceBlocks)
+    reduce_rows_block(partialW, R, (size_t)21 * 256, 3, 0, 0, 0, dW2, blockIdx.x);
+  else
+    bn_finalize_block(A, 0, 48, blockIdx.x - kC3TailReduceBlocks);
+}
+
+__global__ __launch_bounds__(256) void bn1_tail_kernel(const BnFinArgs A, int a_hi, const BnFinArgs B, int b_lo, int b_hi,
+                                                       const float* __restrict__ partialW, int Rw,
+                                                       float* __restrict__ dW) {
+  __shared__ double red[4][64];
+  const int tid = threadIdx.x, o = tid & 63, slice = tid >> 6, c = blockIdx.x;
+  const int Cin = B.C;
+  const bool valid = c < Cin && o < 48;
+  const bool fin_a = slice == 0 && A.partials && c < a_hi && c < A.Cpad;
+  const bool fin_b = slice == 0 && c >= b_lo && c < b_hi && c < B.Cpad;
+  BnFinSums sa{0.0, 0.0, 0.0}, sb{0.0, 0.0, 0.0};
+  if (fin_a) sa = bn_finalize_sums<false>(A, c, o);
+  if (fin_b) sb = bn_finalize_sums<true>(B, c, o);
+  double s = 0.0;
+  if (valid) {
+    const size_t row_stride = (size_t)B.Cpad * 48, src = (size_t)c * 48 + o;
+#pragma unroll 16
+    for (int r = slice; r < Rw; r += 4) s += (double)partialW[(size_t)r * row_stride + src];
+  }
+  red[slice][o] = s;
+  __syncthreads();
+  if (slice != 0) return;
+  float v = 0.f;
+  if (valid) {
+    v = (float)((red[0][tid] + red[1][tid]) + (red[2][tid] + red[3][tid]));
+    dW[(size_t)o * Cin + c] = v;
+  }
+  if (fin_a) bn_finalize_finish<false>(A, c, tid, sa, 0.f);
+  if (fin_b) bn_finalize_finish<true>(B, c, tid, sb, v);
 }
 
 struct NarrowArgs {
@@ -2316,12 +2408,12 @@
 
 }
 
-__global__ __launch_bounds__(256) void bn_dgamma_direct_partial_kernel(
+__device__ __forceinline__ void bn_dgamma_direct_partial_block(
     const float* __restrict__ X, int ldx, long P, int Hin, int Win, int pool, const float* __restrict__ DY, int ld_dy,
     const float* __restrict__ Zr, int ld_z, const float* __restrict__ cA, const float* __restrict__ cB,
     const float* __restrict__ cC, int Cout, const float* __restrict__ W, int Cin, const float* __restrict__ scale1,
     const float* __restrict__ shift1, const float* __restrict__ mean, const float* __restrict__ istd,
-    const int* __restrict__ cond, double* __restrict__ partial) {
+    const int* __restrict__ cond, double* __restrict__ partial, const int block, const int nblocks) {
   __shared__ int list[384];
   __shared__ int cnt;
   __shared__ float wcol[192], co[3][192];
@@ -2339,7 +2431,7 @@
     co[1][o] = Zr ? cB[o] : 0.f;
     co[2][o] = Zr ? cC[o] : 0.f;
   }
-  const long per = (P + gridDim.x - 1) / gridDim.x, p_lo = (long)blockIdx.x * per, p_hi = min(P, p_lo + per);
+  const long per = (P + nblocks - 1) / nblocks, p_lo = (long)block * per, p_hi = min(P, p_lo + per);
   const int Ho = Hin >> 1, Wo = Win >> 1;
   for (int li = 0; li < n; ++li) {
     const int c = list[li];
@@ -2370,18 +2462,54 @@
     for (int o = 32; o > 0; o >>= 1) acc += shfl_xor_d(acc, o);
     if ((tid & 63) == 0) red[tid >> 6] = acc;
     __syncthreads();
-    if (tid == 0) partial[(size_t)blockIdx.x * Cin + c] = (red[0] + red[1]) + (red[2] + red[3]);
-  }
-}
-
-__global__ __launch_bounds__(256) void bn_dgamma_direct_reduce_kernel(const double* __restrict__ partial, int R, int Cin,
-                                                                      const int* __restrict__ cond,
-                                                                      float* __restrict__ dgamma) {
-  const int c = blockIdx.x * 256 + threadIdx.x;
+    if (tid == 0) partial[(size_t)block * Cin + c] = (red[0] + red[1]) + (red[2] + red[3]);
+  }
+}
+
+__global__ __launch_bounds__(256) void bn_dgamma_direct_partial_kernel(
+    const float* __restrict__ X, int ldx, long P, int Hin, int Win, int pool, const float* __restrict__ DY, int ld_dy,
+    const float* __restrict__ Zr, int ld_z, const float* __restrict__ cA, const float* __restrict__ cB,
+    const float* __restrict__ cC, int Cout, const float* __restrict__ W, int Cin, const float* __restrict__ scale1,
+    const float* __restrict__ shift1, const float* __restrict__ mean, const float* __restrict__ istd,
+    const int* __restrict__ cond, double* __restrict__ partial) {
+  bn_dgamma_direct_partial_block(X, ldx, P, Hin, Win, pool, DY, ld_dy, Zr, ld_z, cA, cB, cC, Cout, W, Cin, scale1, shift1, mean,
+                                 istd, cond, partial, blockIdx.x, gridDim.x);
+}
+
+__device__ __forceinline__ void bn_dgamma_direct_reduce_block(const double* __restrict__ partial, int R, int Cin,
+                                                              const int* __restrict__ cond, float* __restrict__ dgamma,
+                                                              const int block) {
+  const int c = block * 256 + threadIdx.x;
   if (c >= Cin || !cond[c]) return;
   double s = 0.0;
   for (int g = 0; g < R; ++g) s += partial[(size_t)g * Cin + c];
   dgamma[c] = (float)s;
+}
+
+__global__ __launch_bounds__(256) void bn_dgamma_direct_reduce_kernel(const double* __restrict__ partial, int R, int Cin,
+                                                                      const int* __restrict__ cond,
+                                                                      float* __restrict__ dgamma) {
+  bn_dgamma_direct_reduce_block(partial, R, Cin, cond, dgamma, blockIdx.x);
+}
+
+struct DirectLayer {
+  const float *DY, *W, *scale1, *shift1;
+  const int* cond;
+  double* partial;
+  float* dgamma;
+  int Cin;
+};
+__global__ __launch_bounds__(256) void bn_dgamma_direct_partial_pair_kernel(
+    const float* __restrict__ X, int ldx, long P, int Hin, int Win, int pool, int ld_dy, int Cout,
+    const float* __restrict__ mean, const float* __restrict__ istd, const DirectLayer L0, const DirectLayer L1) {
+  const DirectLayer& Y = blockIdx.y ? L1 : L0;
+  bn_dgamma_direct_partial_block(X, ldx, P, Hin, Win, pool, Y.DY, ld_dy, nullptr, 0, nullptr, nullptr, nullptr, Cout, Y.W, Y.Cin,
+                                 Y.scale1, Y.shift1, mean, istd, Y.cond, Y.partial, blockIdx.x, gridDim.x);
+}
+
+__global__ __launch_bounds__(256) void bn_dgamma_direct_reduce_pair_kernel(int R, const DirectLayer L0, const DirectLayer L1) {
+  const DirectLayer& Y = blockIdx.y ? L1 : L0;
+  bn_dgamma_direct_reduce_block(Y.partial, R, Y.Cin, Y.cond, Y.dgamma, blockIdx.x);
 }
 
 template <bool DROP>
@@ -2478,7 +2606,7 @@
                                     const float* scale2, const float* shift2, float* partialW, float* dW2, eml::DropKey dk,
                                     eml_stream_t stream) {
   if (!G || !W2 || !Z || !zmean || !zistd || !DZ || !partials || !X || !sB || !sC || !scale2 || !shift2 || !partialW ||
-      !dW2 || B < 1 || H < 1 || W < 1 || grid < 1 || cx < 0)
+      B < 1 || H < 1 || W < 1 || grid < 1 || cx < 0)
     return eml::fail(EML_EINVAL, "%s: bad arguments", name);
   const auto al16 = [](const void* q) { return (reinterpret_cast<uintptr_t>(q) & 15) == 0; };
   if (!eml_dense_conv3x3_bwd_fused_supported(ldg, c0, ldx, cx) || !al16(G) || !al16(X) || !al16(GF) || !al16(Z) || !al16(scale2) ||
@@ -2495,7 +2623,7 @@
   if (a16) { if (GF) launch(std::true_type{}, std::true_type{}); else launch(std::true_type{}, std::false_type{}); }
   else     { if (GF) launch(std::false_type{}, std::true_type{}); else launch(std::false_type{}, std::false_type{}); }
   int rc = eml::check_launch(name);
-  if (rc) return rc;
+  if (rc || !dW2) return rc;
   hipLaunchKernelGGL(reduce_rows_kernel, dim3(21 * 256 / 64), dim3(256), 0, (hipStream_t)stream, partialW, grid,
                      (size_t)21 * 256, 3, 0, 0, 0, dW2);
   return eml::check_launch(DROP ? "eml_dense_conv3x3_bwd_fused_drop_f32(reduce)" : "eml_dense_conv3x3_bwd_fused_f32(reduce)");
@@ -2565,9 +2693,9 @@
   if (W && (!dW || !beta || w_rows < 1))
     return eml::fail(EML_EINVAL, "eml_dense_bn_bwd_finalize_f32: W given without dW / beta / w_rows");
   if (c_hi > Cpad) c_hi = Cpad;
-  hipLaunchKernelGGL(bn_bwd_finalize_kernel, dim3((c_hi - c_lo + 3) / 4), dim3(256), 0, (hipStream_t)stream, partials,
-                     R, pstride, count, gamma, mean, istd, C, Cpad, training, dgamma, dbeta, cA, cB, cC, sB, sC,
-                     s_accumulate, c_lo, c_hi, beta, W, dW, w_rows, W ? cond : nullptr, W ? any_cond : nullptr);
+  const BnFinArgs A{partials, R, pstride, count, gamma, mean, istd, C, Cpad, training, dgamma, dbeta, cA, cB, cC, sB, sC,
+                    s_accumulate, beta, W, dW, w_rows, W ? cond : nullptr, W ? any_cond : nullptr};
+  hipLaunchKernelGGL(bn_bwd_finalize_kernel, dim3((c_hi - c_lo + 3) / 4), dim3(256), 0, (hipStream_t)stream, A, c_lo, c_hi);
   return eml::check_launch("eml_dense_bn_bwd_finalize_f32");
 }
 
@@ -2589,6 +2717,66 @@
   return eml::check_launch("eml_dense_bn_dgamma_direct_f32(reduce)");
 }
 
+extern "C" int eml_dense_bn_dgamma_direct_pair_f32(const float* X, int ldx, long P, const float* mean, const float* istd,
+                                                   const float* DY0, const float* W0, int Cin0, const float* scale0,
+                                                   const float* shift0, const int* cond0, float* dgamma0,
+                                                   const float* DY1, const float* W1, int Cin1, const float* scale1,
+                                                   const float* shift1, const int* cond1, float* dgamma1,
+                                                   double* scratch, int grid, eml_stream_t stream) {
+  if (!X || !mean || !istd || !DY0 || !W0 || !scale0 || !shift0 || !cond0 || !dgamma0 || !DY1 || !W1 || !scale1 || !shift1 ||
+      !cond1 || !dgamma1 || !scratch || P < 1 || grid < 1 || Cin0 < 1 || Cin0 > 384 || Cin1 < 1 || Cin1 > 384 || Cin0 > ldx ||
+      Cin1 > ldx)
+    return eml::fail(EML_EINVAL, "eml_dense_bn_dgamma_direct_pair_f32: bad arguments (1 <= Cin <= 384, Cin <= ldx)");
+  const DirectLayer L0{DY0, W0, scale0, shift0, cond0, scratch, dgamma0, Cin0};
+  const DirectLayer L1{DY1, W1, scale1, shift1, cond1, scratch + (size_t)grid * Cin0, dgamma1, Cin1};
+  hipLaunchKernelGGL(bn_dgamma_direct_partial_pair_kernel, dim3(grid, 2), dim3(256), 0, (hipStream_t)stream, X, ldx, P, 0, 0,
+                     0, 48, 48, mean, istd, L0, L1);
+  int rc = eml::check_launch("eml_dense_bn_dgamma_direct_pair_f32(partial)");
+  if (rc) return rc;
+  const int cmax = Cin0 > Cin1 ? Cin0 : Cin1;
+  hipLaunchKernelGGL(bn_dgamma_direct_reduce_pair_kernel, dim3((cmax + 255) / 256, 2), dim3(256), 0, (hipStream_t)stream,
+                     grid, L0, L1);
+  return eml::check_launch("eml_dense_bn_dgamma_direct_pair_f32(reduce)");
+}
+
+extern "C" int eml_dense_conv3x3_bwd_tail_f32(const float* partialW, int grid, float* dW2, const double* partials,
+                                              double count, const float* gamma, const float* mean, const float* istd,
+                                              float* dgamma, float* dbeta, float* cA, float* cB, float* cC,
+                                              eml_stream_t stream) {
+  if (!partialW || !dW2 || !partials || !gamma || !mean || !istd || !dgamma || !dbeta || !cA || !cB || !cC || grid < 1)
+    return eml::fail(EML_EINVAL, "eml_dense_conv3x3_bwd_tail_f32: bad arguments");
+  const BnFinArgs A{partials, grid, 96, count, gamma, mean, istd, 48, 48, 1, dgamma, dbeta, cA, cB, cC, nullptr, nullptr,
+                    0, nullptr, nullptr, nullptr, 0, nullptr, nullptr};
+  hipLaunchKernelGGL(conv3x3_bwd_tail_kernel, dim3(kC3TailBlocks), dim3(256), 0, (hipStream_t)stream, partialW, grid, dW2, A);
+  return eml::check_launch("eml_dense_conv3x3_bwd_tail_f32");
+}
+
+extern "C" int eml_dense_bn1_tail_f32(double count, const float* mean, const float* istd, float* sB, float* sC, int* any_cond,
+                                      const double* partsA, int RA, int KpA, int CinA, const float* gammaA,
+                                      const float* betaA, const float* WA, const float* dWA, float* dgammaA, float* dbetaA,
+                                      int* condA, int a_hi,
+                                      const float* partialW, int Rw, const double* partsB, int RB, int KpB, int CinB,
+                                      const float* gammaB, const float* betaB, const float* WB, float* dWB, float* dgammaB,
+                                      float* dbetaB, int* condB, int b_lo, int b_hi, eml_stream_t stream) {
+  if (!mean || !istd || !sB || !sC || !partialW || !partsB || !gammaB || !betaB || !WB || !dWB || !dgammaB || !dbetaB ||
+      Rw < 1 || RB < 1 || CinB < 1 || KpB < CinB || b_lo < 0 || b_hi <= b_lo)
+    return eml::fail(EML_EINVAL, "eml_dense_bn1_tail_f32: bad arguments");
+  if (partsA && (!gammaA || !betaA || !WA || !dWA || !dgammaA || !dbetaA || RA < 1 || CinA < 1 || KpA < CinA || a_hi < 1))
+    return eml::fail(EML_EINVAL, "eml_dense_bn1_tail_f32: first layer given without its arguments");
+  if (b_hi > KpB) b_hi = KpB;
+  if (!partsA) a_hi = 0;
+  else if (a_hi > KpA) a_hi = KpA;
+  const BnFinArgs A{partsA, RA, 2 * KpA, count, gammaA, mean, istd, CinA, KpA, 1, dgammaA, dbetaA, nullptr, nullptr, nullptr,
+                    sB, sC, 1, betaA, WA, dWA, 48, condA, condA ? any_cond : nullptr};
+  const BnFinArgs Bl{partsB, RB, 2 * KpB, count, gammaB, mean, istd, CinB, KpB, 1, dgammaB, dbetaB, nullptr, nullptr, nullptr,
+                     sB, sC, 1, betaB, WB, nullptr, 48, condB, condB ? any_cond : nullptr};
+  int nblocks = CinB > b_hi ? CinB : b_hi;
+  if (a_hi > nblocks) nblocks = a_hi;
+  hipLaunchKernelGGL(bn1_tail_kernel, dim3(nblocks), dim3(256), 0, (hipStream_t)stream, A, a_hi, Bl, b_lo, b_hi, partialW, Rw,
+                     dWB);
+  return eml::check_launch("eml_dense_bn1_tail_f32");
+}
+
 extern "C" int eml_dense_conv1x1_bwd_weight_f32(const float* X, int ldx, long P, int Hin, int Win, int pool, int Kp,
                                                 int Cin, const float* scale1, const float* shift1, const float* DY,
                                                 int ld_dy, const float* Zr, int ld_z, const float* cA, const float* cB,
@@ -2601,7 +2789,9 @@
               (ldg != 12 && k_lo + 12 > ldg)))
     return eml::fail(EML_EINVAL, "eml_dense_conv1x1_bwd_weight_f32: fused narrow pass needs a dense layer, W1, G, partials_n "
                                  "and an even k_lo with k_lo + 12 <= Cin (k_lo=%d, Cin=%d)", k_lo, Cin);
-  if (!X || !scale1 || !shift1 || !DY || !Zr || !cA || !cB || !cC || !partial || !dW || P < 1 || grid < 1 || Kp < 32 ||
+  if (!dW && (Cout != 48 || pool))
+    return eml::fail(EML_EINVAL, "eml_dense_conv1x1_bwd_weight_f32: dW == NULL is for dense layers (Cout == 48, no pool)");
+  if (!X || !scale1 || !shift1 || !DY || !Zr || !cA || !cB || !cC || !partial || P < 1 || grid < 1 || Kp < 32 ||
       (Kp & 15) || Cin > Kp || Cout < 1)
     return eml::fail(EML_EINVAL, "eml_dense_conv1x1_bwd_weight_f32: bad arguments");
   const int nchunks = (Cout + 47) / 48;
@@ -2624,7 +2814,7 @@
                          (int)P, Hin, Win, Kp, scale1, shift1, DY + n0, ld_dy, Zr + n0, ld_z, cA + n0, cB + n0, cC + n0,
                          nv, n_load, partial, dz_out, na);
     int rc = eml::check_launch("eml_dense_conv1x1_bwd_weight_f32");
-    if (rc) return rc;
+    if (rc || !dW) return rc;
     hipLaunchKernelGGL(reduce_rows_kernel, dim3((Cin * 48 + 63) / 64), dim3(256), 0, (hipStream_t)stream, partial,
                        grid, (size_t)Kp * 48, 0, Cin, nv, n0, dW);
     rc = eml::check_launch("eml_dense_conv1x1_bwd_weight_f32(reduce)");
diff --git a/include/emlight_hip_ext.h b/include/emlight_hip_ext.h
--- a/include/emlight_hip_ext.h
+++ b/include/emlight_hip_ext.h
@@ -76,6 +76,21 @@
                           int K, int h, int w, double fov_deg, double view_azimuth_deg, const float* image, float* ratio,
                           float* shadowed, float* work, eml_stream_t stream);
 
+int eml_dense_conv3x3_bwd_tail_f32(const float* partialW, int grid, float* dW2, const double* partials, double count,
+                                   const float* gamma, const float* mean, const float* istd, float* dgamma, float* dbeta,
+                                   float* cA, float* cB, float* cC, eml_stream_t stream);
+int eml_dense_bn1_tail_f32(double count, const float* mean, const float* istd, float* sB, float* sC, int* any_cond,
+                           const double* partsA, int RA, int KpA, int CinA, const float* gammaA, const float* betaA,
+                           const float* WA, const float* dWA, float* dgammaA, float* dbetaA, int* condA, int a_hi,
+                           const float* partialW, int Rw, const double* partsB, int RB, int KpB, int CinB,
+                           const float* gammaB, const float* betaB, const float* WB, float* dWB, float* dgammaB,
+                           float* dbetaB, int* condB, int b_lo, int b_hi, eml_stream_t stream);
+int eml_dense_bn_dgamma_direct_pair_f32(const float* X, int ldx, long P, const float* mean, const float* istd,
+                                        const float* DY0, const float* W0, int Cin0, const float* scale0,
+                                        const float* shift0, const int* cond0, float* dgamma0, const float* DY1,
+                                        const float* W1, int Cin1, const float* scale1, const float* shift1,
+                                        const int* cond1, float* dgamma1, double* scratch, int grid, eml_stream_t stream);
+
 #ifdef __cplusplus
 }
 #endif
```

Measured after the change: 569.0 images/s (median of 6 runs). No clear change (+0.5%).
